# libmir/mir-optim

Measured on AMD Instinct MI355X. Metric: LM iterations/sec, higher is better.
Workload: dtype f64

## Files before the change

include/mir_optim_amd.h:

```cpp
#ifndef MIR_OPTIM_AMD_H
#define MIR_OPTIM_AMD_H

#include <stddef.h>
#include <stdint.h>

#ifdef __cplusplus
extern "C" {
#endif


typedef enum mir_least_squares_status {
    mir_ls_maxIterations = -1,
    mir_ls_furtherImprovement = 0,
    mir_ls_xConverged = 1,
    mir_ls_gConverged = 2,
    mir_ls_fConverged = 3,
    mir_ls_badBounds = -32,
    mir_ls_badGuess = -31,
    mir_ls_badMinStepQuality = -30,
    mir_ls_badGoodStepQuality = -29,
    mir_ls_badStepQuality = -28,
    mir_ls_badLambdaParams = -27,
    mir_ls_numericError = -26
} mir_least_squares_status;

typedef enum mir_box_qp_status {
    mir_box_qp_solved = 0,
    mir_box_qp_numericError = 1,
    mir_box_qp_maxIterations = 2
} mir_box_qp_status;

typedef struct mir_box_qp_settings_d { double relTolerance, absTolerance; uint32_t maxIterations; } mir_box_qp_settings_d;
typedef struct mir_box_qp_settings_s { float relTolerance, absTolerance; uint32_t maxIterations; } mir_box_qp_settings_s;

typedef struct mir_least_squares_settings_d {
    uint32_t maxIterations;
    uint32_t maxAge;
    double jacobianEpsilon;
    double absTolerance;
    double relTolerance;
    double gradTolerance;
    double maxGoodResidual;
    double maxStep;
    double maxLambda;
    double minLambda;
    double minStepQuality;
    double goodStepQuality;
    double lambdaIncrease;
    double lambdaDecrease;
    mir_box_qp_settings_d qpSettings;
} mir_least_squares_settings_d;

typedef struct mir_least_squares_settings_s {
    uint32_t maxIterations, maxAge;
    float jacobianEpsilon, absTolerance, relTolerance, gradTolerance, maxGoodResidual, maxStep,
          maxLambda, minLambda, minStepQuality, goodStepQuality, lambdaIncrease, lambdaDecrease;
    mir_box_qp_settings_s qpSettings;
} mir_least_squares_settings_s;

typedef struct mir_least_squares_result_d {
    int32_t status;
    uint32_t iterations, fCalls, gCalls;
    double residual;
    double lambda;
} mir_least_squares_result_d;
typedef struct mir_least_squares_result_s {
    int32_t status;
    uint32_t iterations, fCalls, gCalls;
    float residual, lambda;
} mir_least_squares_result_s;

typedef struct mir_slice_d { size_t length; double* ptr; } mir_slice_d;
typedef struct mir_slice_s { size_t length; float* ptr; } mir_slice_s;
typedef struct mir_slice_i { size_t length; int32_t* ptr; } mir_slice_i;

typedef void (*mir_least_squares_function_d)(void* context, size_t m, size_t n, const double* x, double* y);
typedef void (*mir_least_squares_jacobian_d)(void* context, size_t m, size_t n, const double* x, double* J);
typedef void (*mir_least_squares_function_s)(void* context, size_t m, size_t n, const float* x, float* y);
typedef void (*mir_least_squares_jacobian_s)(void* context, size_t m, size_t n, const float* x, float* J);

typedef struct mir_least_squares_task { void* context; void* function; } mir_least_squares_task;
typedef void (*mir_least_squares_task_function)(mir_least_squares_task task, uint32_t totalThreads,
                                                uint32_t threadId, uint32_t i);
typedef void (*mir_least_squares_thread_manager)(void* context, uint32_t count,
                                                 mir_least_squares_task taskContext,
                                                 mir_least_squares_task_function task);

size_t mir_least_squares_work_length(size_t m, size_t n);
size_t mir_least_squares_iwork_length(size_t m, size_t n);
size_t mir_box_qp_work_length(size_t n);
size_t mir_box_qp_iwork_length(size_t n);
size_t mir_box_qp_iwork_length_ilp64(size_t n);
size_t mir_least_squares_iwork_length_ilp64(size_t m, size_t n);
const char* mir_least_squares_status_string(mir_least_squares_status st);
void mir_least_squares_init_d(mir_least_squares_settings_d* settings);
void mir_least_squares_init_s(mir_least_squares_settings_s* settings);
void mir_least_squares_reset_d(mir_least_squares_settings_d* settings);
void mir_least_squares_reset_s(mir_least_squares_settings_s* settings);

mir_least_squares_result_d mir_optimize_least_squares_d(
    const mir_least_squares_settings_d* settings, size_t m, size_t n,
    double* x, const double* l, const double* u,
    mir_slice_d work, mir_slice_i iwork,
    void* fContext, mir_least_squares_function_d f,
    void* gContext, mir_least_squares_jacobian_d g,
    void* tmContext, mir_least_squares_thread_manager tm);

mir_least_squares_result_s mir_optimize_least_squares_s(
    const mir_least_squares_settings_s* settings, size_t m, size_t n,
    float* x, const float* l, const float* u,
    mir_slice_s work, mir_slice_i iwork,
    void* fContext, mir_least_squares_function_s f,
    void* gContext, mir_least_squares_jacobian_s g,
    void* tmContext, mir_least_squares_thread_manager tm);


typedef struct mir_lsq_comm mir_lsq_comm;
typedef struct mir_lsq_workspace mir_lsq_workspace;

typedef void (*mir_lsq_batched_function_d)(void* context, size_t m, size_t n, size_t p, const double* X, double* Y);
typedef void (*mir_lsq_batched_function_s)(void* context, size_t m, size_t n, size_t p, const float* X, float* Y);
enum {
    MIR_LSQ_DEVICE_CALLBACKS = 1u,
    MIR_LSQ_TIME_KERNELS = 2u
};

enum {
    MIR_LSQ_VARIANT_BROYDEN_REWRITE = 1u << 0,
    MIR_LSQ_VARIANT_FD_SEPARATE_FILL = 1u << 1,
    MIR_LSQ_VARIANT_NO_SPECULATION = 1u << 4,
    MIR_LSQ_VARIANT_NO_NULL_SKIP = 1u << 5,
    MIR_LSQ_VARIANT_SOLVE_BOUNDED = 1u << 6,
    MIR_LSQ_VARIANT_SOLVE_GENERIC = 1u << 10,
    MIR_LSQ_VARIANT_SOLVE_ONE_WORKGROUP = 1u << 11,
    MIR_LSQ_VARIANT_FD_HOST_COLUMNS = 1u << 13,
    MIR_LSQ_VARIANT_NO_PIPELINE = 1u << 22,
    MIR_LSQ_VARIANT_DEBUG_HELPERS_ABSENT = 1u << 12,
    MIR_LSQ_VARIANT_DEBUG_SOLVE = 1u << 7,
    MIR_LSQ_VARIANT_HOST_PROFILE = 1u << 8,
    MIR_LSQ_VARIANT_LR_CAP_SHIFT = 16
};

typedef struct mir_lsq_stats {
    uint64_t passes, accepted, rejected, step_guard_rejects;
    uint64_t jacobian_full, jacobian_broyden;
    uint64_t jtj_launches;
    uint64_t jtj_broyden_launches;
    double jtj_ms;
    double jtj_broyden_ms;
    double solve_ms;
    uint64_t solve_launches;
    double fd_ms;
    double total_ms;
    uint64_t qp_active_set_passes;
    uint64_t broyden_lr_columns;
    double jtj_fd_ms;
    uint64_t jtj_fd_launches;
    uint64_t elided_evaluations;
    uint64_t allreduce_calls[3];
    uint64_t allreduce_elems[3];
    uint64_t broyden_flushes;
    uint64_t jtj_resyncs;
    double fd_callback_ms;
    uint64_t fd_callback_calls, fd_callback_points;
    double trial_callback_ms;
    uint64_t trial_callback_calls, trial_callback_points;
    uint64_t library_launches;
    uint64_t round_launches[3];
    uint64_t rounds[3];
    double fd_host_wall_ms, fd_host_f_ms;
    uint64_t fd_host_columns;
    double host_f_ms;
    uint64_t host_f_calls;
    uint64_t fused_rounds;
    uint64_t fused_passes;
    uint64_t coop_timeouts;
} mir_lsq_stats;

typedef struct mir_lsq_trace_record {
    int32_t event;
    uint32_t iterations;
    double lambda, residual, trial_residual, dx_dot;
} mir_lsq_trace_record;
typedef struct mir_lsq_trace {
    mir_lsq_trace_record* records;
    uint64_t capacity;
    uint64_t count;
} mir_lsq_trace;

typedef struct mir_lsq_gpu_options {
    uint32_t struct_size;
    uint32_t flags;
    void* stream;
    mir_lsq_comm* comm;
    mir_lsq_workspace* workspace;
    void* fbContext;
    void* fb;
    uint32_t fd_batch;
    uint32_t variant;
    mir_lsq_stats* stats;
    mir_lsq_trace* trace;
    void* fbRowMajor;
    void* fbRowMajorDiff;
    uint32_t stats_size;
    uint32_t reserved0;
} mir_lsq_gpu_options;

mir_least_squares_result_d mir_optimize_least_squares_gpu_d(
    const mir_least_squares_settings_d* settings, size_t m, size_t n,
    double* x, const double* l, const double* u, const mir_lsq_gpu_options* options,
    void* fContext, mir_least_squares_function_d f,
    void* gContext, mir_least_squares_jacobian_d g,
    void* tmContext, mir_least_squares_thread_manager tm);
mir_least_squares_result_s mir_optimize_least_squares_gpu_s(
    const mir_least_squares_settings_s* settings, size_t m, size_t n,
    float* x, const float* l, const float* u, const mir_lsq_gpu_options* options,
    void* fContext, mir_least_squares_function_s f,
    void* gContext, mir_least_squares_jacobian_s g,
    void* tmContext, mir_least_squares_thread_manager tm);

int mir_solve_box_qp_gpu_d(const mir_box_qp_settings_d* settings, size_t n, const double* P,
                           const double* q, const double* l, const double* u, double* x,
                           int unconstrainedSolution, int* iterations);
int mir_solve_box_qp_gpu_s(const mir_box_qp_settings_s* settings, size_t n, const float* P,
                           const float* q, const float* l, const float* u, float* x,
                           int unconstrainedSolution, int* iterations);

#define MIR_LSQ_BOX_QP_UNCONSTRAINED_SOLUTION 1u
int mir_lsq_batched_box_qp_s(const mir_box_qp_settings_s* settings, size_t count, size_t n, const float* P, const float* q,
                             const float* l, const float* u, size_t bound_stride, float* x, int* status, int* iterations,
                             unsigned flags, void* stream);
int mir_lsq_batched_box_qp_d(const mir_box_qp_settings_d* settings, size_t count, size_t n, const double* P, const double* q,
                             const double* l, const double* u, size_t bound_stride, double* x, int* status, int* iterations,
                             unsigned flags, void* stream);

int mir_lsq_batched_box_qp16_s(const mir_box_qp_settings_s* settings, size_t count, size_t n, const float* P, const float* q,
                               const float* l, const float* u, size_t bound_stride, float* x, int* status, int* iterations,
                               unsigned flags, void* stream);
int mir_lsq_batched_box_qp16_d(const mir_box_qp_settings_d* settings, size_t count, size_t n, const double* P, const double* q,
                               const double* l, const double* u, size_t bound_stride, double* x, int* status, int* iterations,
                               unsigned flags, void* stream);

enum { MIR_LSQ_MODEL_EXP_DECAY = 0, MIR_LSQ_MODEL_EXP3_AFFINE = 1,
       MIR_LSQ_MODEL_EXP_DECAY_PAD8 = 2 };
enum { MIR_LSQ_BATCHED_ANALYTIC_JACOBIAN = 2 };
enum { MIR_LSQ_BATCHED_NO_LADDER = 1 };
enum { MIR_LSQ_BATCHED_DEVICE_BOUNDS = 4 };
typedef struct mir_lsq_batched_options {
    uint32_t struct_size;
    uint32_t variant;
    void* stream;
    float* basis;
    size_t basis_bytes;
    uint64_t* timing;
} mir_lsq_batched_options;

int mir_optimize_least_squares_batched_s(const mir_least_squares_settings_s* settings, size_t count, size_t m, int model,
                                         float* x, const float* lower, const float* upper,
                                         const float* t, size_t t_stride, const float* data,
                                         mir_least_squares_result_s* results, const mir_lsq_batched_options* options);

enum { MIR_LSQ_BATCHED_NEEDS_GENERAL = -100 };
int mir_lsq_batched_kernel_s(const mir_least_squares_settings_s* settings, size_t count, size_t m, int model,
                             float* x, const float* lower, const float* upper,
                             const float* t, size_t t_stride, const float* data,
                             mir_least_squares_result_s* results, const mir_lsq_batched_options* options);

int mir_optimize_least_squares_batched_d(const mir_least_squares_settings_d* settings, size_t count, size_t m, int model,
                                         double* x, const double* lower, const double* upper,
                                         const double* t, size_t t_stride, const double* data,
                                         mir_least_squares_result_d* results, const mir_lsq_batched_options* options);
int mir_lsq_batched_kernel_d(const mir_least_squares_settings_d* settings, size_t count, size_t m, int model,
                             double* x, const double* lower, const double* upper,
                             const double* t, size_t t_stride, const double* data,
                             mir_least_squares_result_d* results, const mir_lsq_batched_options* options);

enum { MIR_LSQ_BATCHED_ABSOLUTE_SIGMA = 1u };
typedef struct mir_lsq_batched_extras {
    uint32_t struct_size;
    uint32_t flags;
    const void* weights;
    size_t weight_stride;
    void* covariance;
} mir_lsq_batched_extras;
int mir_optimize_least_squares_batched_ex_s(const mir_least_squares_settings_s* settings, size_t count, size_t m, int model,
                                            float* x, const float* lower, const float* upper,
                                            const float* t, size_t t_stride, const float* data,
                                            mir_least_squares_result_s* results, const mir_lsq_batched_options* options,
                                            const mir_lsq_batched_extras* extras);
int mir_optimize_least_squares_batched_ex_d(const mir_least_squares_settings_d* settings, size_t count, size_t m, int model,
                                            double* x, const double* lower, const double* upper,
                                            const double* t, size_t t_stride, const double* data,
                                            mir_least_squares_result_d* results, const mir_lsq_batched_options* options,
                                            const mir_lsq_batched_extras* extras);
int mir_lsq_batched_kernel_ex_s(const mir_least_squares_settings_s* settings, size_t count, size_t m, int model,
                                float* x, const float* lower, const float* upper,
                                const float* t, size_t t_stride, const float* data,
                                mir_least_squares_result_s* results, const mir_lsq_batched_options* options,
                                const mir_lsq_batched_extras* extras);
int mir_lsq_batched_kernel_ex_d(const mir_least_squares_settings_d* settings, size_t count, size_t m, int model,
                                double* x, const double* lower, const double* upper,
                                const double* t, size_t t_stride, const double* data,
                                mir_least_squares_result_d* results, const mir_lsq_batched_options* options,
                                const mir_lsq_batched_extras* extras);
int mir_lsq_batched_covariance_s(const mir_least_squares_settings_s* settings, size_t count, size_t m, int model,
                                 const float* x, const float* lower, const float* upper,
                                 const float* t, size_t t_stride, const float* data,
                                 const mir_least_squares_result_s* results, const mir_lsq_batched_options* options,
                                 const mir_lsq_batched_extras* extras);
int mir_lsq_batched_covariance_d(const mir_least_squares_settings_d* settings, size_t count, size_t m, int model,
                                 const double* x, const double* lower, const double* upper,
                                 const double* t, size_t t_stride, const double* data,
                                 const mir_least_squares_result_d* results, const mir_lsq_batched_options* options,
                                 const mir_lsq_batched_extras* extras);

enum { MIR_LSQ_MODEL16_EXP_HARM16 = 16, MIR_LSQ_MODEL16_GAUSS3_AFFINE = 17 };
int mir_optimize_least_squares_batched16_d(const mir_least_squares_settings_d* settings, size_t count, size_t m, int model,
                                           double* x, const double* lower, const double* upper,
                                           const double* t, size_t t_stride, const double* data,
                                           mir_least_squares_result_d* results, const mir_lsq_batched_options* options,
                                           const mir_lsq_batched_extras* extras);
int mir_lsq_batched16_kernel_d(const mir_least_squares_settings_d* settings, size_t count, size_t m, int model,
                               double* x, const double* lower, const double* upper,
                               const double* t, size_t t_stride, const double* data,
                               mir_least_squares_result_d* results, const mir_lsq_batched_options* options,
                               const mir_lsq_batched_extras* extras);
int mir_optimize_least_squares_batched16_ex_d(const mir_least_squares_settings_d* settings, size_t count, size_t m, int model,
                                              double* x, const double* lower, const double* upper,
                                              const double* t, size_t t_stride, const double* data,
                                              mir_least_squares_result_d* results, const mir_lsq_batched_options* options,
                                              const mir_lsq_batched_extras* extras);
int mir_lsq_batched16_kernel_ex_d(const mir_least_squares_settings_d* settings, size_t count, size_t m, int model,
                                  double* x, const double* lower, const double* upper,
                                  const double* t, size_t t_stride, const double* data,
                                  mir_least_squares_result_d* results, const mir_lsq_batched_options* options,
                                  const mir_lsq_batched_extras* extras);
int mir_lsq_batched16_covariance_d(const mir_least_squares_settings_d* settings, size_t count, size_t m, int model,
                                   const double* x, const double* lower, const double* upper,
                                   const double* t, size_t t_stride, const double* data,
                                   const mir_least_squares_result_d* results, const mir_lsq_batched_options* options,
                                   const mir_lsq_batched_extras* extras);
int mir_lsq_batched16_jtj_d(size_t count, size_t m, size_t n, const double* J, const double* y, double* JJ, double* Jy, void* stream);

enum { MIR_LSQ_RESIDENT_NO_NULL_SKIP = 1u,
       MIR_LSQ_RESIDENT_UNBOUNDED = 2u,
       MIR_LSQ_RESIDENT_NO_LOOKAHEAD = 4u,
       MIR_LSQ_RESIDENT_DEBUG_DROP_WORKGROUP = 16u,
       MIR_LSQ_RESIDENT_ANALYTIC_JACOBIAN = 32u,
       MIR_LSQ_RESIDENT_NO_STAMPS = 8u           };
typedef struct mir_lsq_resident_stats {
    uint64_t rounds, passes, accepted, rejected, step_guard_rejects, jacobian_full, jacobian_broyden, qp_active_set_passes,
        elided_evaluations;
    uint64_t t_total, t_stage, t_worker, t_group, t_total_wait, t_solver, t_solve_body, t_cmd_wait;
    uint64_t t_w_eval, t_w_fd, t_w_prod;
    uint64_t t_w_mma;
    uint64_t lookahead_rejections;
    uint64_t t_look;
    uint64_t t_unpack, t_publish;
    uint32_t abort_code, grid, rows, groups;
} mir_lsq_resident_stats;
typedef struct mir_lsq_resident_options {
    uint32_t struct_size;
    uint32_t variant;
    void* stream;
    void* workspace;
    size_t workspace_bytes;
    mir_lsq_trace_record* trace_records;
    uint32_t trace_capacity;
    uint32_t max_workgroups;
    uint32_t* trace_count;
    mir_lsq_resident_stats* stats;
} mir_lsq_resident_options;

int mir_lsq_batched_posvx_s(size_t count, size_t n, const float* P, const float* rhs, float* x, int* info, void* stream);
int mir_lsq_batched_posvx_d(size_t count, size_t n, const double* P, const double* rhs, double* x, int* info, void* stream);
int mir_lsq_batched_posvx16_s(size_t count, size_t n, const float* P, const float* rhs, float* x, int* info, void* stream);
int mir_lsq_batched_posvx16_d(size_t count, size_t n, const double* P, const double* rhs, double* x, int* info, void* stream);

int mir_lsq_jtj_d(size_t m, size_t n, double* J, const double* y, const double* y_old, const double* dx,
                  int broyden, double* JJ, double* Jy, void* stream, float* kernel_ms);
int mir_lsq_jtj_s(size_t m, size_t n, float* J, const float* y, const float* y_old, const float* dx,
                  int broyden, float* JJ, float* Jy, void* stream, float* kernel_ms);
int mir_lsq_fd_jtj_d(size_t m, size_t n, const double* Yrm, const double* twh, const double* y, double* J,
                     double* JJ, double* Jy, void* stream, float* kernel_ms);
int mir_lsq_fd_diff_jtj_d(size_t m, size_t n, const double* Drm, const double* twh, const double* y, double* J,
                          double* JJ, double* Jy, void* stream, float* kernel_ms);
int mir_lsq_jtj_plan(size_t elem_size, size_t m, size_t n, int num_cu, int op, int aligned16, size_t out[10]);

enum { MIR_LSQ_COVARIANCE_ABSOLUTE_SIGMA = 1u };
int mir_lsq_covariance_gpu_d(const mir_least_squares_settings_d* settings, size_t m, size_t n,
    const double* x, const double* l, const double* u, const mir_lsq_gpu_options* options,
    void* fContext, mir_least_squares_function_d f, void* gContext, mir_least_squares_jacobian_d g,
    void* tmContext, mir_least_squares_thread_manager tm,
    uint32_t flags, double* cov, double* residual_out, int* info);
int mir_lsq_covariance_gpu_s(const mir_least_squares_settings_s* settings, size_t m, size_t n,
    const float* x, const float* l, const float* u, const mir_lsq_gpu_options* options,
    void* fContext, mir_least_squares_function_s f, void* gContext, mir_least_squares_jacobian_s g,
    void* tmContext, mir_least_squares_thread_manager tm,
    uint32_t flags, float* cov, float* residual_out, int* info);
int mir_lsq_spd_inverse_d(size_t n, const double* P, const unsigned char* fixed, double* X, int* info, void* stream);
int mir_lsq_spd_inverse_s(size_t n, const float*  P, const unsigned char* fixed, float*  X, int* info, void* stream);
size_t mir_lsq_spd_inverse_work_bytes(size_t n, size_t elem_size);
int mir_lsq_spd_inverse_work_d(size_t n, const double* P, const unsigned char* fixed, double* X, int* info, void* work,
                               size_t work_bytes, void* stream);
int mir_lsq_spd_inverse_work_s(size_t n, const float* P, const unsigned char* fixed, float* X, int* info, void* work,
                               size_t work_bytes, void* stream);

mir_lsq_workspace* mir_lsq_workspace_create(size_t m, size_t n, size_t elem_size);
void mir_lsq_workspace_destroy(mir_lsq_workspace* ws);

int mir_lsq_rccl_unique_id(void* out_128_bytes);
mir_lsq_comm* mir_lsq_comm_create_rccl(int nranks, int rank, const void* unique_id_128_bytes);
typedef void (*mir_lsq_allreduce_fn)(void* ctx, double* device_buf, size_t count, void* stream);
mir_lsq_comm* mir_lsq_comm_create_callback(int nranks, int rank, mir_lsq_allreduce_fn fn, void* ctx);
int mir_lsq_comm_create_local_group(int nranks, mir_lsq_comm** out_comms);
void mir_lsq_comm_destroy(mir_lsq_comm* comm);
int mir_lsq_comm_record(mir_lsq_comm* comm, double* host_buf, size_t capacity);
size_t mir_lsq_comm_recorded(const mir_lsq_comm* comm);
mir_lsq_comm* mir_lsq_comm_create_replay(int nranks, int rank, const double* totals_host, size_t len, mir_lsq_comm* inner);
int mir_lsq_comm_replay_rewind(mir_lsq_comm* comm);
int mir_lsq_comm_replay_set_delay(mir_lsq_comm* comm, unsigned microseconds);
int mir_lsq_comm_ranks(const mir_lsq_comm* comm);
int mir_lsq_comm_describe(const mir_lsq_comm* comm, char* buf, size_t len);
int mir_lsq_comm_allreduce_d(mir_lsq_comm* comm, double* buf, size_t count, void* stream);
int mir_lsq_comm_allreduce_s(mir_lsq_comm* comm, float* buf, size_t count, void* stream);

int mir_lsq_device_count(void);
void* mir_lsq_device_malloc(size_t bytes);
void mir_lsq_device_free(void* p);
int mir_lsq_memcpy_h2d(void* dst_device, const void* src_host, size_t bytes, void* stream);
int mir_lsq_memcpy_d2h(void* dst_host, const void* src_device, size_t bytes, void* stream);
int mir_lsq_memcpy_d2d(void* dst_device, const void* src_device, size_t bytes, void* stream);

int mir_lsq_selftest_reductions(int rounds, int mismatches[4]);
void* mir_lsq_stream_create(void);
void mir_lsq_stream_destroy(void* stream);
int mir_lsq_stream_synchronize(void* stream);
const char* mir_lsq_version(void);

enum { MIR_FIT_SPLINE_OK = 0, MIR_FIT_SPLINE_TOO_FEW_POINTS = 1, MIR_FIT_SPLINE_BAD_ARGUMENT = 2 };

int mir_fit_spline_d(const mir_least_squares_settings_d* settings, size_t npoints, const double* points, size_t nx,
                     const double* x, const double* l, const double* u, double lambda, double (*dist)(double, double),
                     double* splineY, double* splineD, mir_least_squares_result_d* result);
int mir_fit_spline_s(const mir_least_squares_settings_s* settings, size_t npoints, const float* points, size_t nx,
                     const float* x, const float* l, const float* u, float lambda, float (*dist)(float, float),
                     float* splineY, float* splineD, mir_least_squares_result_s* result);
void mir_fit_spline_residuals_d(size_t npoints, const double* points, size_t nx, const double* x, double lambda,
                                const double* splineY, size_t m, double* y);
void mir_spline_c2_derivatives_d(size_t n, const double* x, const double* y, double* d);
void mir_spline_c2_derivatives_s(size_t n, const float* x, const float* y, float* d);
void mir_spline_eval_d(size_t n, const double* x, const double* y, const double* d, double t, double* out3);
void mir_spline_eval_s(size_t n, const float* x, const float* y, const float* d, float t, float* out3);

#ifdef __cplusplus
}
#endif
#endif
```

mir_optim_amd/api.py:

```python
import ctypes as C
import enum
import os

import numpy as np

from . import build as _build

__all__ = [
    "LeastSquaresStatus", "BoxQPStatus", "LeastSquaresSettings", "LeastSquaresResult", "BoxQPSettings",
    "LeastSquaresException", "optimize", "optimizeLeastSquares", "solveBoxQP", "leastSquaresStatusString",
    "mir_least_squares_work_length", "mir_least_squares_iwork_length", "mir_box_qp_work_length",
    "mir_box_qp_iwork_length", "GpuOptions", "Stats", "lib", "workloads_lib", "device_count",
    "DeviceBuffer", "Stream", "jtj", "fd_jtj", "DEVICE_CALLBACKS", "TIME_KERNELS", "optimizeLeastSquaresBatched", "batchedPosvx", "BATCHED_NO_LADDER", "BATCHED_DEVICE_BOUNDS",
    "solveBoxQPBatched", "BOX_QP_UNCONSTRAINED_SOLUTION",
    "MODEL_EXP_DECAY", "MODEL_EXP3_AFFINE", "MODEL_EXP_DECAY_PAD8", "MODEL16_EXP_HARM16", "MODEL16_GAUSS3_AFFINE", "batched16JtJ", "optimizeLeastSquaresBatched16", "ResultS", "Trace", "TraceRecord", "Spline", "FitSplineResult", "fitSpline",
    "fit_spline_residuals", "variant_lr_cap",
    "VARIANT_BROYDEN_REWRITE", "VARIANT_FD_SEPARATE_FILL", "VARIANT_NO_SPECULATION", "VARIANT_NO_NULL_SKIP",
    "VARIANT_SOLVE_BOUNDED", "VARIANT_DEBUG_SOLVE", "VARIANT_HOST_PROFILE", "VARIANT_SOLVE_GENERIC", "VARIANT_SOLVE_ONE_WORKGROUP", "VARIANT_DEBUG_HELPERS_ABSENT", "VARIANT_FD_HOST_COLUMNS",
    "VARIANT_NO_PIPELINE", "BatchedOptions", "BatchedExtras", "BATCHED_ABSOLUTE_SIGMA",
    "covariance", "spdInverse", "COVARIANCE_ABSOLUTE_SIGMA",
]

MODEL_EXP_DECAY = 0
MODEL_EXP3_AFFINE = 1
MODEL_EXP_DECAY_PAD8 = 2
MODEL16_EXP_HARM16 = 16
MODEL16_GAUSS3_AFFINE = 17
_MODELS16 = (MODEL16_EXP_HARM16, MODEL16_GAUSS3_AFFINE)

DEVICE_CALLBACKS = 1
TIME_KERNELS = 2

VARIANT_BROYDEN_REWRITE = 1 << 0
VARIANT_FD_SEPARATE_FILL = 1 << 1
VARIANT_NO_SPECULATION = 1 << 4
VARIANT_NO_NULL_SKIP = 1 << 5
VARIANT_SOLVE_BOUNDED = 1 << 6
VARIANT_DEBUG_SOLVE = 1 << 7
VARIANT_HOST_PROFILE = 1 << 8
VARIANT_SOLVE_GENERIC = 1 << 10
VARIANT_SOLVE_ONE_WORKGROUP = 1 << 11
VARIANT_DEBUG_HELPERS_ABSENT = 1 << 12
VARIANT_FD_HOST_COLUMNS = 1 << 13
VARIANT_NO_PIPELINE = 1 << 22


def variant_lr_cap(k):
    return (int(k) & 31) << 16


class LeastSquaresStatus(enum.IntEnum):
    maxIterations = -1
    furtherImprovement = 0
    xConverged = 1
    gConverged = 2
    fConverged = 3
    badBounds = -32
    badGuess = -31
    badMinStepQuality = -30
    badGoodStepQuality = -29
    badStepQuality = -28
    badLambdaParams = -27
    numericError = -26


class BoxQPStatus(enum.IntEnum):
    solved = 0
    numericError = 1
    maxIterations = 2


class LeastSquaresException(Exception):

    def __init__(self, status, result=None):
        self.status = LeastSquaresStatus(status)
        self.result = result
        super().__init__("mir-optim Least Squares: " + leastSquaresStatusString(status))


class _QPd(C.Structure):
    _fields_ = [("relTolerance", C.c_double), ("absTolerance", C.c_double), ("maxIterations", C.c_uint32)]


class _QPs(C.Structure):
    _fields_ = [("relTolerance", C.c_float), ("absTolerance", C.c_float), ("maxIterations", C.c_uint32)]


_FIELDS = ["jacobianEpsilon", "absTolerance", "relTolerance", "gradTolerance", "maxGoodResidual", "maxStep",
           "maxLambda", "minLambda", "minStepQuality", "goodStepQuality", "lambdaIncrease", "lambdaDecrease"]


class _Sd(C.Structure):
    _fields_ = ([("maxIterations", C.c_uint32), ("maxAge", C.c_uint32)] + [(k, C.c_double) for k in _FIELDS]
                + [("qpSettings", _QPd)])


class _Ss(C.Structure):
    _fields_ = ([("maxIterations", C.c_uint32), ("maxAge", C.c_uint32)] + [(k, C.c_float) for k in _FIELDS]
                + [("qpSettings", _QPs)])


class _Rd(C.Structure):
    _fields_ = [("status", C.c_int32), ("iterations", C.c_uint32), ("fCalls", C.c_uint32), ("gCalls", C.c_uint32),
                ("residual", C.c_double), ("lambda_", C.c_double)]


class _Rs(C.Structure):
    _fields_ = [("status", C.c_int32), ("iterations", C.c_uint32), ("fCalls", C.c_uint32), ("gCalls", C.c_uint32),
                ("residual", C.c_float), ("lambda_", C.c_float)]


ResultS = _Rs


class _SliceD(C.Structure):
    _fields_ = [("length", C.c_size_t), ("ptr", C.c_void_p)]


class _Task(C.Structure):
    _fields_ = [("context", C.c_void_p), ("function", C.c_void_p)]


class Stats(C.Structure):
    _fields_ = [("passes", C.c_uint64), ("accepted", C.c_uint64), ("rejected", C.c_uint64),
                ("step_guard_rejects", C.c_uint64), ("jacobian_full", C.c_uint64), ("jacobian_broyden", C.c_uint64),
                ("jtj_launches", C.c_uint64), ("jtj_broyden_launches", C.c_uint64), ("jtj_ms", C.c_double),
                ("jtj_broyden_ms", C.c_double), ("solve_ms", C.c_double), ("solve_launches", C.c_uint64),
                ("fd_ms", C.c_double), ("total_ms", C.c_double), ("qp_active_set_passes", C.c_uint64),
                ("broyden_lr_columns", C.c_uint64),
                ("jtj_fd_ms", C.c_double), ("jtj_fd_launches", C.c_uint64),
                ("elided_evaluations", C.c_uint64),
                ("allreduce_calls", C.c_uint64 * 3), ("allreduce_elems", C.c_uint64 * 3),
                ("broyden_flushes", C.c_uint64), ("jtj_resyncs", C.c_uint64),
                ("fd_callback_ms", C.c_double), ("fd_callback_calls", C.c_uint64), ("fd_callback_points", C.c_uint64),
                ("trial_callback_ms", C.c_double), ("trial_callback_calls", C.c_uint64),
                ("trial_callback_points", C.c_uint64),
                ("library_launches", C.c_uint64), ("round_launches", C.c_uint64 * 3), ("rounds", C.c_uint64 * 3),
                ("fd_host_wall_ms", C.c_double), ("fd_host_f_ms", C.c_double), ("fd_host_columns", C.c_uint64),
                ("host_f_ms", C.c_double), ("host_f_calls", C.c_uint64),
                ("fused_rounds", C.c_uint64), ("fused_passes", C.c_uint64), ("coop_timeouts", C.c_uint64)]

    def as_dict(self):
        return {k: (list(getattr(self, k)) if isinstance(getattr(self, k), C.Array) else getattr(self, k)) for k, _ in self._fields_}


class TraceRecord(C.Structure):
    _fields_ = [("event", C.c_int32), ("iterations", C.c_uint32), ("lambda_", C.c_double), ("residual", C.c_double),
                ("trial_residual", C.c_double), ("dx_dot", C.c_double)]


class _TraceHeader(C.Structure):
    _fields_ = [("records", C.POINTER(TraceRecord)), ("capacity", C.c_uint64), ("count", C.c_uint64)]


class Trace:

    EVENTS = {0: "jacobian_full", 1: "jacobian_broyden", 2: "rejected", 3: "accepted", 4: "step_guard"}

    def __init__(self, capacity=4096):
        self._buf = (TraceRecord * capacity)()
        self.header = _TraceHeader(C.cast(self._buf, C.POINTER(TraceRecord)), capacity, 0)

    @property
    def count(self):
        return int(self.header.count)

    def records(self):
        k = min(self.count, int(self.header.capacity))
        return [(r.event, r.iterations, r.lambda_, r.residual, r.trial_residual, r.dx_dot) for r in self._buf[:k]]


class GpuOptions(C.Structure):
    _fields_ = [("struct_size", C.c_uint32), ("flags", C.c_uint32), ("stream", C.c_void_p), ("comm", C.c_void_p),
                ("workspace", C.c_void_p), ("fbContext", C.c_void_p), ("fb", C.c_void_p), ("fd_batch", C.c_uint32),
                ("variant", C.c_uint32), ("stats", C.POINTER(Stats)), ("trace", C.POINTER(_TraceHeader)),
                ("fbRowMajor", C.c_void_p), ("fbRowMajorDiff", C.c_void_p), ("stats_size", C.c_uint32),
                ("reserved0", C.c_uint32)]

    def __init__(self, **kw):
        super().__init__(**kw)
        self.struct_size = C.sizeof(GpuOptions)
        self.stats_size = C.sizeof(Stats)


class BatchedOptions(C.Structure):
    _fields_ = [("struct_size", C.c_uint32), ("variant", C.c_uint32), ("stream", C.c_void_p), ("basis", C.c_void_p),
                ("basis_bytes", C.c_size_t), ("timing", C.c_void_p)]

    def __init__(self, **kw):
        super().__init__(**kw)
        self.struct_size = C.sizeof(BatchedOptions)


class BatchedExtras(C.Structure):
    _fields_ = [("struct_size", C.c_uint32), ("flags", C.c_uint32), ("weights", C.c_void_p), ("weight_stride", C.c_size_t),
                ("covariance", C.c_void_p)]

    def __init__(self, **kw):
        super().__init__(**kw)
        self.struct_size = C.sizeof(BatchedExtras)


TASK_FN = C.CFUNCTYPE(None, _Task, C.c_uint32, C.c_uint32, C.c_uint32)
TM_FN = C.CFUNCTYPE(None, C.c_void_p, C.c_uint32, _Task, TASK_FN)
ALLREDUCE_FN = C.CFUNCTYPE(None, C.c_void_p, C.c_void_p, C.c_size_t, C.c_void_p)


def _ftype(dtype):
    ct = C.c_double if dtype == np.float64 else C.c_float
    return C.CFUNCTYPE(None, C.c_void_p, C.c_size_t, C.c_size_t, C.POINTER(ct), C.POINTER(ct))


_lib = None
_wl = None


def _load(path):
    if not os.path.exists(path):
        raise ImportError(f"{path} is missing: build it with `python -m mir_optim_amd.build` "
                          "(hipcc --offload-arch=gfx950). mir_optim_amd has no CPU fallback.")
    return C.CDLL(path, mode=C.RTLD_GLOBAL)


def lib():
    global _lib
    if _lib is None:
        L = _load(_build.SOLVER_LIB)
        sz = C.c_size_t
        for name in ("mir_least_squares_work_length", "mir_least_squares_iwork_length"):
            getattr(L, name).restype = sz
            getattr(L, name).argtypes = [sz, sz]
        for name in ("mir_box_qp_work_length", "mir_box_qp_iwork_length"):
            getattr(L, name).restype = sz
            getattr(L, name).argtypes = [sz]
        L.mir_box_qp_iwork_length_ilp64.restype = sz
        L.mir_box_qp_iwork_length_ilp64.argtypes = [sz]
        L.mir_least_squares_iwork_length_ilp64.restype = sz
        L.mir_least_squares_iwork_length_ilp64.argtypes = [sz, sz]
        L.mir_least_squares_status_string.restype = C.c_char_p
        L.mir_least_squares_status_string.argtypes = [C.c_int]
        for suf, S, R in (("d", _Sd, _Rd), ("s", _Ss, _Rs)):
            getattr(L, "mir_least_squares_init_" + suf).argtypes = [C.POINTER(S)]
            getattr(L, "mir_least_squares_reset_" + suf).argtypes = [C.POINTER(S)]
            fn = getattr(L, "mir_optimize_least_squares_" + suf)
            fn.restype = R
            fn.argtypes = [C.POINTER(S), sz, sz, C.c_void_p, C.c_void_p, C.c_void_p, _SliceD, _SliceD,
                           C.c_void_p, C.c_void_p, C.c_void_p, C.c_void_p, C.c_void_p, C.c_void_p]
            fn = getattr(L, "mir_optimize_least_squares_gpu_" + suf)
            fn.restype = R
            fn.argtypes = [C.POINTER(S), sz, sz, C.c_void_p, C.c_void_p, C.c_void_p, C.POINTER(GpuOptions),
                           C.c_void_p, C.c_void_p, C.c_void_p, C.c_void_p, C.c_void_p, C.c_void_p]
            fn = getattr(L, "mir_solve_box_qp_gpu_" + suf)
            fn.restype = C.c_int
            fn.argtypes = [C.c_void_p, sz, C.c_void_p, C.c_void_p, C.c_void_p, C.c_void_p, C.c_void_p, C.c_int,
                           C.POINTER(C.c_int)]
            fn = getattr(L, "mir_lsq_jtj_" + suf)
            fn.restype = C.c_int
            fn.argtypes = [sz, sz, C.c_void_p, C.c_void_p, C.c_void_p, C.c_void_p, C.c_int, C.c_void_p, C.c_void_p,
                           C.c_void_p, C.POINTER(C.c_float)]
            fn = getattr(L, "mir_lsq_covariance_gpu_" + suf)
            fn.restype = C.c_int
            fn.argtypes = [C.POINTER(S), sz, sz, C.c_void_p, C.c_void_p, C.c_void_p, C.POINTER(GpuOptions),
                           C.c_void_p, C.c_void_p, C.c_void_p, C.c_void_p, C.c_void_p, C.c_void_p,
                           C.c_uint32, C.c_void_p, C.c_void_p, C.POINTER(C.c_int)]
            fn = getattr(L, "mir_lsq_spd_inverse_" + suf)
            fn.restype = C.c_int
            fn.argtypes = [sz, C.c_void_p, C.c_void_p, C.c_void_p, C.c_void_p, C.c_void_p]
            fn = getattr(L, "mir_lsq_spd_inverse_work_" + suf)
            fn.restype = C.c_int
            fn.argtypes = [sz, C.c_void_p, C.c_void_p, C.c_void_p, C.c_void_p, C.c_void_p, sz, C.c_void_p]
        L.mir_lsq_spd_inverse_work_bytes.restype = sz
        L.mir_lsq_spd_inverse_work_bytes.argtypes = [sz, sz]
        L.mir_lsq_comm_create_local_group.restype = C.c_int
        L.mir_lsq_comm_create_local_group.argtypes = [C.c_int, C.POINTER(C.c_void_p)]
        L.mir_lsq_fd_diff_jtj_d.restype = C.c_int
        L.mir_lsq_fd_diff_jtj_d.argtypes = [sz, sz, C.c_void_p, C.c_void_p, C.c_void_p, C.c_void_p, C.c_void_p, C.c_void_p,
                                            C.c_void_p, C.POINTER(C.c_float)]
        L.mir_lsq_fd_jtj_d.restype = C.c_int
        L.mir_lsq_fd_jtj_d.argtypes = [sz, sz, C.c_void_p, C.c_void_p, C.c_void_p, C.c_void_p, C.c_void_p, C.c_void_p,
                                       C.c_void_p, C.c_void_p]
        L.mir_optimize_least_squares_batched_s.restype = C.c_int
        L.mir_optimize_least_squares_batched_s.argtypes = [C.POINTER(_Ss), sz, sz, C.c_int, C.c_void_p, C.c_void_p, C.c_void_p,
                                                           C.c_void_p, sz, C.c_void_p, C.c_void_p, C.POINTER(BatchedOptions)]
        L.mir_lsq_batched_kernel_s.restype = C.c_int
        L.mir_lsq_batched_kernel_s.argtypes = [C.POINTER(_Ss), sz, sz, C.c_int, C.c_void_p, C.c_void_p, C.c_void_p,
                                               C.c_void_p, sz, C.c_void_p, C.c_void_p, C.POINTER(BatchedOptions)]
        L.mir_lsq_jtj_plan.restype = C.c_int
        L.mir_lsq_jtj_plan.argtypes = [sz, sz, sz, C.c_int, C.c_int, C.c_int, C.POINTER(sz * 10)]
        L.mir_lsq_selftest_reductions.restype = C.c_int
        L.mir_lsq_selftest_reductions.argtypes = [C.c_int, C.POINTER(C.c_int * 4)]
        L.mir_lsq_batched_posvx_s.restype = C.c_int
        L.mir_lsq_batched_posvx_s.argtypes = [sz, sz, C.c_void_p, C.c_void_p, C.c_void_p, C.c_void_p, C.c_void_p]
        L.mir_optimize_least_squares_batched_d.restype = C.c_int
        L.mir_optimize_least_squares_batched_d.argtypes = [C.POINTER(_Sd), sz, sz, C.c_int, C.c_void_p, C.c_void_p, C.c_void_p,
                                                           C.c_void_p, sz, C.c_void_p, C.c_void_p, C.POINTER(BatchedOptions)]
        L.mir_lsq_batched_kernel_d.restype = C.c_int
        L.mir_lsq_batched_kernel_d.argtypes = [C.POINTER(_Sd), sz, sz, C.c_int, C.c_void_p, C.c_void_p, C.c_void_p,
                                               C.c_void_p, sz, C.c_void_p, C.c_void_p, C.POINTER(BatchedOptions)]
        L.mir_lsq_batched_posvx_d.restype = C.c_int
        L.mir_lsq_batched_posvx_d.argtypes = [sz, sz, C.c_void_p, C.c_void_p, C.c_void_p, C.c_void_p, C.c_void_p]
        for suf, S in (("s", _Ss), ("d", _Sd)):
            for name in ("mir_optimize_least_squares_batched_ex_", "mir_lsq_batched_kernel_ex_", "mir_lsq_batched_covariance_"):
                fn = getattr(L, name + suf)
                fn.restype = C.c_int
                fn.argtypes = [C.POINTER(S), sz, sz, C.c_int, C.c_void_p, C.c_void_p, C.c_void_p, C.c_void_p, sz, C.c_void_p,
                               C.c_void_p, C.POINTER(BatchedOptions), C.POINTER(BatchedExtras)]
        for name in ("mir_optimize_least_squares_batched16_d", "mir_lsq_batched16_kernel_d", "mir_optimize_least_squares_batched16_ex_d",
                     "mir_lsq_batched16_kernel_ex_d", "mir_lsq_batched16_covariance_d"):
            fn = getattr(L, name)
            fn.restype = C.c_int
            fn.argtypes = [C.POINTER(_Sd), sz, sz, C.c_int, C.c_void_p, C.c_void_p, C.c_void_p, C.c_void_p, sz, C.c_void_p,
                           C.c_void_p, C.POINTER(BatchedOptions), C.POINTER(BatchedExtras)]
        L.mir_lsq_batched16_jtj_d.restype = C.c_int
        L.mir_lsq_batched16_jtj_d.argtypes = [sz, sz, sz, C.c_void_p, C.c_void_p, C.c_void_p, C.c_void_p, C.c_void_p]
        for name in ("box_qp_s", "box_qp_d", "box_qp16_s", "box_qp16_d"):
            fn = getattr(L, "mir_lsq_batched_" + name)
            fn.restype = C.c_int
            fn.argtypes = [C.c_void_p, sz, sz, C.c_void_p, C.c_void_p, C.c_void_p, C.c_void_p, sz, C.c_void_p, C.c_void_p,
                           C.c_void_p, C.c_uint, C.c_void_p]
        for suf in ("s", "d"):
            fn = getattr(L, "mir_lsq_batched_posvx16_" + suf)
            fn.restype = C.c_int
            fn.argtypes = [sz, sz, C.c_void_p, C.c_void_p, C.c_void_p, C.c_void_p, C.c_void_p]
        L.mir_lsq_comm_describe.restype = C.c_int
        L.mir_lsq_comm_describe.argtypes = [C.c_void_p, C.c_char_p, C.c_size_t]
        L.mir_lsq_workspace_create.restype = C.c_void_p
        L.mir_lsq_workspace_create.argtypes = [sz, sz, sz]
        L.mir_lsq_workspace_destroy.argtypes = [C.c_void_p]
        L.mir_lsq_rccl_unique_id.restype = C.c_int
        L.mir_lsq_rccl_unique_id.argtypes = [C.c_void_p]
        L.mir_lsq_comm_create_rccl.restype = C.c_void_p
        L.mir_lsq_comm_create_rccl.argtypes = [C.c_int, C.c_int, C.c_void_p]
        L.mir_lsq_comm_create_callback.restype = C.c_void_p
        L.mir_lsq_comm_create_callback.argtypes = [C.c_int, C.c_int, ALLREDUCE_FN, C.c_void_p]
        L.mir_lsq_comm_destroy.argtypes = [C.c_void_p]
        L.mir_lsq_comm_record.restype = C.c_int
        L.mir_lsq_comm_record.argtypes = [C.c_void_p, C.c_void_p, sz]
        L.mir_lsq_comm_recorded.restype = sz
        L.mir_lsq_comm_recorded.argtypes = [C.c_void_p]
        L.mir_lsq_comm_create_replay.restype = C.c_void_p
        L.mir_lsq_comm_create_replay.argtypes = [C.c_int, C.c_int, C.c_void_p, sz, C.c_void_p]
        L.mir_lsq_comm_replay_rewind.restype = C.c_int
        L.mir_lsq_comm_replay_rewind.argtypes = [C.c_void_p]
        L.mir_lsq_comm_replay_set_delay.restype = C.c_int
        L.mir_lsq_comm_replay_set_delay.argtypes = [C.c_void_p, C.c_uint]
        L.mir_lsq_comm_ranks.restype = C.c_int
        L.mir_lsq_comm_ranks.argtypes = [C.c_void_p]
        for name in ("mir_lsq_comm_allreduce_d", "mir_lsq_comm_allreduce_s"):
            getattr(L, name).restype = C.c_int
            getattr(L, name).argtypes = [C.c_void_p, C.c_void_p, sz, C.c_void_p]
        L.mir_lsq_device_count.restype = C.c_int
        L.mir_lsq_device_malloc.restype = C.c_void_p
        L.mir_lsq_device_malloc.argtypes = [sz]
        L.mir_lsq_device_free.argtypes = [C.c_void_p]
        for name in ("mir_lsq_memcpy_h2d", "mir_lsq_memcpy_d2h", "mir_lsq_memcpy_d2d"):
            getattr(L, name).restype = C.c_int
            getattr(L, name).argtypes = [C.c_void_p, C.c_void_p, sz, C.c_void_p]
        L.mir_lsq_stream_create.restype = C.c_void_p
        L.mir_lsq_stream_destroy.argtypes = [C.c_void_p]
        L.mir_lsq_stream_synchronize.restype = C.c_int
        L.mir_lsq_stream_synchronize.argtypes = [C.c_void_p]
        L.mir_lsq_version.restype = C.c_char_p
        for suf, S, R, ct in (("d", _Sd, _Rd, C.c_double), ("s", _Ss, _Rs, C.c_float)):
            fn = getattr(L, "mir_fit_spline_" + suf)
            fn.restype = C.c_int
            fn.argtypes = [C.POINTER(S), sz, C.c_void_p, sz, C.c_void_p, C.c_void_p, C.c_void_p, ct, C.c_void_p,
                           C.c_void_p, C.c_void_p, C.POINTER(R)]
            getattr(L, "mir_spline_c2_derivatives_" + suf).argtypes = [sz, C.c_void_p, C.c_void_p, C.c_void_p]
            getattr(L, "mir_spline_eval_" + suf).argtypes = [sz, C.c_void_p, C.c_void_p, C.c_void_p, ct, C.c_void_p]
        L.mir_fit_spline_residuals_d.argtypes = [sz, C.c_void_p, sz, C.c_void_p, C.c_double, C.c_void_p, sz, C.c_void_p]
        _lib = L
    return _lib


def workloads_lib():
    global _wl
    if _wl is None:
        W = _load(_build.WORKLOADS_LIB)
        W.wl_uniform.argtypes = [C.c_uint64, C.c_uint64, C.c_size_t, C.c_void_p]
        W.wl_tanh_linear_generate.argtypes = [C.c_size_t, C.c_size_t, C.c_size_t, C.c_double, C.c_void_p, C.c_void_p,
                                              C.c_void_p, C.c_void_p]
        _wl = W
    return _wl


def device_count():
    return lib().mir_lsq_device_count()


def leastSquaresStatusString(st):
    return lib().mir_least_squares_status_string(int(st)).decode()


def mir_least_squares_work_length(m, n):
    return lib().mir_least_squares_work_length(m, n)


def mir_least_squares_iwork_length(m, n):
    return lib().mir_least_squares_iwork_length(m, n)


def mir_box_qp_work_length(n):
    return lib().mir_box_qp_work_length(n)


def mir_box_qp_iwork_length(n):
    return lib().mir_box_qp_iwork_length(n)


def LeastSquaresSettings(dtype=np.float64):
    s = _Sd() if dtype == np.float64 else _Ss()
    (lib().mir_least_squares_init_d if dtype == np.float64 else lib().mir_least_squares_init_s)(C.byref(s))
    return s


def BoxQPSettings(dtype=np.float64):
    return LeastSquaresSettings(dtype).qpSettings


class LeastSquaresResult:

    def __init__(self, raw):
        self.status = LeastSquaresStatus(raw.status)
        self.iterations = raw.iterations
        self.fCalls = raw.fCalls
        self.gCalls = raw.gCalls
        self.residual = raw.residual
        self.lambda_ = raw.lambda_

    def __repr__(self):
        return (f"LeastSquaresResult(status={self.status.name}, iterations={self.iterations}, fCalls={self.fCalls}, "
                f"gCalls={self.gCalls}, residual={self.residual!r}, lambda={self.lambda_!r})")


class Stream:
    def __init__(self):
        self.handle = lib().mir_lsq_stream_create()
        if not self.handle:
            raise RuntimeError("hipStreamCreate failed (no GPU?)")

    def synchronize(self):
        if lib().mir_lsq_stream_synchronize(self.handle) != 0:
            raise RuntimeError("stream synchronize failed")

    def close(self):
        if self.handle:
            lib().mir_lsq_stream_destroy(self.handle)
            self.handle = None

    def __del__(self):
        try:
            self.close()
        except Exception:
            pass


class DeviceBuffer:

    def __init__(self, array=None, nbytes=None, dtype=None, shape=None):
        if array is not None:
            array = np.ascontiguousarray(array)
            nbytes, dtype, shape = array.nbytes, array.dtype, array.shape
        self.nbytes, self.dtype, self.shape = int(nbytes), np.dtype(dtype), tuple(shape)
        self.ptr = lib().mir_lsq_device_malloc(max(self.nbytes, 8))
        if not self.ptr:
            raise MemoryError(f"hipMalloc({self.nbytes}) failed (no GPU?)")
        if array is not None:
            self.upload(array)

    def upload(self, array):
        array = np.ascontiguousarray(array, dtype=self.dtype)
        assert array.nbytes == self.nbytes
        if lib().mir_lsq_memcpy_h2d(self.ptr, array.ctypes.data, self.nbytes, None) != 0:
            raise RuntimeError("H2D copy failed")

    def upload_at(self, byte_offset, array):
        array = np.ascontiguousarray(array, dtype=self.dtype)
        assert 0 <= byte_offset and byte_offset + array.nbytes <= self.nbytes
        if lib().mir_lsq_memcpy_h2d(self.ptr + byte_offset, array.ctypes.data, array.nbytes, None) != 0:
            raise RuntimeError("H2D copy failed")

    def download(self):
        out = np.empty(self.shape, dtype=self.dtype)
        if lib().mir_lsq_memcpy_d2h(out.ctypes.data, self.ptr, self.nbytes, None) != 0:
            raise RuntimeError("D2H copy failed")
        return out

    def free(self):
        if self.ptr:
            lib().mir_lsq_device_free(self.ptr)
            self.ptr = None

    def __del__(self):
        try:
            self.free()
        except Exception:
            pass


def _as_fnptr(cb, ftype, wrap, keep):
    if cb is None:
        return C.c_void_p(None)
    if callable(cb):
        c = ftype(wrap(cb))
        keep.append(c)
        return C.cast(c, C.c_void_p)
    return C.c_void_p(int(cb))


def _wrap_callbacks(f, g, tm, dtype):
    ft = _ftype(dtype)
    keep = []
    errors = []

    def wrap_f(fn):
        def cb(_ctx, m_, n_, xp, yp):
            yv = np.ctypeslib.as_array(yp, shape=(m_,))
            try:
                xv = np.ctypeslib.as_array(xp, shape=(n_,))
                yv[:] = 0
                fn(xv, yv)
            except BaseException as e:
                errors.append(e)
                yv[:] = np.nan
        return cb

    def wrap_g(fn):
        def cb(_ctx, m_, n_, xp, Jp):
            Jv = np.ctypeslib.as_array(Jp, shape=(m_ * n_,)).reshape(m_, n_)
            try:
                xv = np.ctypeslib.as_array(xp, shape=(n_,))
                Jv[:] = 0
                fn(xv, Jv)
            except BaseException as e:
                errors.append(e)
                Jv[:] = np.nan
        return cb

    fptr = _as_fnptr(f, ft, wrap_f, keep)
    gptr = _as_fnptr(g, ft, wrap_g, keep)
    tmptr = C.c_void_p(None)
    if tm is not None:
        def tm_cb(_ctx, count, task, taskfn):
            try:
                tm(count, lambda total, tid, i: taskfn(task, total, tid, i))
            except BaseException as e:
                errors.append(e)
        tmc = TM_FN(tm_cb)
        keep.append(tmc)
        tmptr = C.cast(tmc, C.c_void_p)
    return fptr, gptr, tmptr, keep, errors


def optimizeLeastSquares(f, m, x, l=None, u=None, g=None, tm=None, settings=None, dtype=np.float64,
                         fContext=None, gContext=None, options=None, gpu_entry=None):
    L = lib()
    dbl = dtype == np.float64
    x = np.ascontiguousarray(x, dtype=dtype)
    n = x.size
    lo = np.full(n, -np.inf, dtype=dtype) if l is None else np.ascontiguousarray(l, dtype=dtype)
    up = np.full(n, np.inf, dtype=dtype) if u is None else np.ascontiguousarray(u, dtype=dtype)
    if settings is None:
        settings = LeastSquaresSettings(dtype)
    fptr, gptr, tmptr, keep, errors = _wrap_callbacks(f, g, tm, dtype)
    use_gpu_entry = gpu_entry if gpu_entry is not None else (options is not None)
    suf = "d" if dbl else "s"
    if use_gpu_entry:
        fn = getattr(L, "mir_optimize_least_squares_gpu_" + suf)
        raw = fn(C.byref(settings), m, n, x.ctypes.data, lo.ctypes.data, up.ctypes.data,
                 C.byref(options) if options is not None else None, fContext, fptr, gContext, gptr, None, tmptr)
    else:
        wl = L.mir_least_squares_work_length(m, n)
        iwl = L.mir_least_squares_iwork_length(m, n)
        iwork = np.zeros(iwl + 4, dtype=np.int32)
        work_slice = _SliceD(wl, None)
        iwork_slice = _SliceD(iwl, iwork.ctypes.data)
        fn = getattr(L, "mir_optimize_least_squares_" + suf)
        raw = fn(C.byref(settings), m, n, x.ctypes.data, lo.ctypes.data, up.ctypes.data, work_slice, iwork_slice,
                 fContext, fptr, gContext, gptr, None, tmptr)
    del keep
    if errors:
        raise errors[0]
    return LeastSquaresResult(raw), x


def optimize(f, m, x, l=None, u=None, g=None, tm=None, settings=None, dtype=np.float64, taskPool=None, **kw):
    if taskPool is not None and tm is None:
        import threading
        workers = max(1, getattr(taskPool, "_max_workers", 1))
        ids = {}
        lock = threading.Lock()

        def tm(count, task):
            def run(i):
                with lock:
                    tid = ids.setdefault(threading.get_ident(), len(ids))
                task(workers, tid % workers, i)
            list(taskPool.map(run, range(count)))
    res, xo = optimizeLeastSquares(f, m, x, l, u, g, tm, settings, dtype, **kw)
    if res.status < 0:
        raise LeastSquaresException(res.status, res)
    return res, xo


def _batched_suffix(dtype):
    if np.dtype(dtype) == np.float32:
        return "s"
    if np.dtype(dtype) == np.float64:
        return "d"
    raise ValueError(f"the batched entries exist in float32 and float64, not {np.dtype(dtype)}")


def optimizeLeastSquaresBatched(model, x, t, data, l=None, u=None, settings=None, variant=0, dtype=np.float32, weights=None,
                                covariance=False, absolute_sigma=False):
    if int(model) in _MODELS16:
        return _optimize_batched16(model, x, t, data, l, u, settings, variant, dtype, weights, covariance, absolute_sigma)
    suf = _batched_suffix(dtype)
    dtype = np.float32 if suf == "s" else np.float64
    L = lib()
    x = np.array(x, dtype=dtype, order="C")
    count, n = x.shape
    data = np.ascontiguousarray(data, dtype=dtype)
    m = data.shape[1]
    t = np.ascontiguousarray(t, dtype=dtype)
    t_stride = 0 if t.ndim == 1 else m
    lo = np.full(n, -np.inf, dtype=dtype) if l is None else np.ascontiguousarray(l, dtype=dtype)
    up = np.full(n, np.inf, dtype=dtype) if u is None else np.ascontiguousarray(u, dtype=dtype)
    if settings is None:
        settings = LeastSquaresSettings(dtype)
    raw = ((_Rs if suf == "s" else _Rd) * count)()
    if weights is None and not covariance and not absolute_sigma:
        fn = getattr(L, "mir_optimize_least_squares_batched_" + suf)
        rc = fn(C.byref(settings), count, m, int(model), x.ctypes.data, lo.ctypes.data, up.ctypes.data, t.ctypes.data, t_stride,
                data.ctypes.data, raw, C.byref(BatchedOptions(variant=variant)))
        if rc != 0:
            raise RuntimeError(f"mir_optimize_least_squares_batched_{suf} failed: {rc}")
        return [LeastSquaresResult(r) for r in raw], x
    ex = BatchedExtras(flags=BATCHED_ABSOLUTE_SIGMA if absolute_sigma else 0)
    if weights is not None:
        weights = np.ascontiguousarray(weights, dtype=dtype)
        if weights.shape not in ((m,), (count, m)):
            raise ValueError(f"weights: {m} values or {count} x {m}, not {weights.shape}")
        ex.weights = weights.ctypes.data
        ex.weight_stride = 0 if weights.ndim == 1 else m
    cov = np.empty((count, n, n), dtype=dtype) if covariance else None
    if covariance:
        ex.covariance = cov.ctypes.data
    fn = getattr(L, "mir_optimize_least_squares_batched_ex_" + suf)
    rc = fn(C.byref(settings), count, m, int(model), x.ctypes.data, lo.ctypes.data, up.ctypes.data, t.ctypes.data, t_stride,
            data.ctypes.data, raw, C.byref(BatchedOptions(variant=variant)), C.byref(ex))
    if rc != 0:
        raise RuntimeError(f"mir_optimize_least_squares_batched_ex_{suf} failed: {rc}")
    res = [LeastSquaresResult(r) for r in raw]
    return (res, x, cov) if covariance else (res, x)


def _optimize_batched16(model, x, t, data, l, u, settings, variant, dtype, weights, covariance, absolute_sigma):
    if np.dtype(dtype) != np.float64:
        raise ValueError(f"the MODEL16_* models are fitted in float64 only, not {np.dtype(dtype)}: pass dtype=np.float64")
    if weights is not None or covariance or absolute_sigma:
        raise ValueError("the MODEL16_* models take neither weights nor covariance here: call optimizeLeastSquaresBatched16")
    L = lib()
    x = np.array(x, dtype=np.float64, order="C")
    count, n = x.shape
    data = np.ascontiguousarray(data, dtype=np.float64)
    m = data.shape[1]
    t = np.ascontiguousarray(t, dtype=np.float64)
    t_stride = 0 if t.ndim == 1 else m
    lo = np.full(n, -np.inf) if l is None else np.ascontiguousarray(l, dtype=np.float64)
    up = np.full(n, np.inf) if u is None else np.ascontiguousarray(u, dtype=np.float64)
    if settings is None:
        settings = LeastSquaresSettings(np.float64)
    raw = (_Rd * count)()
    rc = L.mir_optimize_least_squares_batched16_d(C.byref(settings), count, m, int(model), x.ctypes.data, lo.ctypes.data,
                                                  up.ctypes.data, t.ctypes.data, t_stride, data.ctypes.data, raw,
                                                  C.byref(BatchedOptions(variant=variant)), None)
    if rc != 0:
        raise RuntimeError(f"mir_optimize_least_squares_batched16_d failed: {rc}")
    return [LeastSquaresResult(r) for r in raw], x


def optimizeLeastSquaresBatched16(model, x, t, data, l=None, u=None, settings=None, variant=0, weights=None, covariance=False,
                                  absolute_sigma=False):
    if int(model) not in _MODELS16:
        raise ValueError(f"optimizeLeastSquaresBatched16 takes a MODEL16_* id, not {model}")
    for name, a in (("x", x), ("t", t), ("data", data), ("weights", weights)):
        dt = getattr(a, "dtype", None)
        if dt is not None and np.issubdtype(dt, np.floating) and dt != np.float64:
            raise ValueError(f"the MODEL16_* models are fitted in float64 only: {name} is {dt}")
    if weights is None and not covariance and not absolute_sigma:
        return _optimize_batched16(model, x, t, data, l, u, settings, variant, np.float64, None, False, False)
    L = lib()
    x = np.array(x, dtype=np.float64, order="C")
    data = np.ascontiguousarray(data, dtype=np.float64)
    t = np.ascontiguousarray(t, dtype=np.float64)
    if x.ndim != 2 or data.ndim != 2 or data.shape[0] != x.shape[0]:
        raise ValueError(f"x: count x n and data: count x m, not {x.shape} and {data.shape}")
    count, n = x.shape
    m = data.shape[1]
    if t.shape not in ((m,), (count, m)):
        raise ValueError(f"t: {m} values or {count} x {m}, not {t.shape}")
    t_stride = 0 if t.ndim == 1 else m
    lo = np.full(n, -np.inf) if l is None else np.ascontiguousarray(l, dtype=np.float64)
    up = np.full(n, np.inf) if u is None else np.ascontiguousarray(u, dtype=np.float64)
    if lo.shape != (n,) or up.shape != (n,):
        raise ValueError(f"l and u: {n} values each, not {lo.shape} and {up.shape}")
    if settings is None:
        settings = LeastSquaresSettings(np.float64)
    ex = BatchedExtras(flags=BATCHED_ABSOLUTE_SIGMA if absolute_sigma else 0)
    if weights is not None:
        weights = np.ascontiguousarray(weights, dtype=np.float64)
        if weights.shape not in ((m,), (count, m)):
            raise ValueError(f"weights: {m} values or {count} x {m}, not {weights.shape}")
        ex.weights = weights.ctypes.data
        ex.weight_stride = 0 if weights.ndim == 1 else m
    cov = np.empty((count, n, n), dtype=np.float64) if covariance else None
    if covariance:
        ex.covariance = cov.ctypes.data
    raw = (_Rd * count)()
    rc = L.mir_optimize_least_squares_batched16_ex_d(C.byref(settings), count, m, int(model), x.ctypes.data, lo.ctypes.data,
                                                     up.ctypes.data, t.ctypes.data, t_stride, data.ctypes.data, raw,
                                                     C.byref(BatchedOptions(variant=variant)), C.byref(ex))
    if rc != 0:
        raise RuntimeError(f"mir_optimize_least_squares_batched16_ex_d failed: {rc}")
    res = [LeastSquaresResult(r) for r in raw]
    return (res, x, cov) if covariance else (res, x)


def batched16JtJ(J, y):
    L = lib()
    J = np.ascontiguousarray(J, dtype=np.float64)
    y = np.ascontiguousarray(y, dtype=np.float64)
    count, m, n = J.shape
    dJ, dy = DeviceBuffer(J), DeviceBuffer(y)
    dJJ = DeviceBuffer(nbytes=count * 256 * 8, dtype=np.float64, shape=(count, 16, 16))
    dJy = DeviceBuffer(nbytes=count * 16 * 8, dtype=np.float64, shape=(count, 16))
    st = Stream()
    rc = L.mir_lsq_batched16_jtj_d(count, m, n, dJ.ptr, dy.ptr, dJJ.ptr, dJy.ptr, st.handle)
    if rc != 0:
        raise RuntimeError(f"mir_lsq_batched16_jtj_d failed: {rc}")
    st.synchronize()
    JJ, Jy = dJJ.download().copy(), dJy.download().copy()
    for b in (dJ, dy, dJJ, dJy):
        b.free()
    return JJ, Jy


BATCHED_NO_LADDER = 1
BATCHED_DEVICE_BOUNDS = 4
BATCHED_ABSOLUTE_SIGMA = 1


def batchedPosvx(P, rhs, dtype=np.float32):
    suf = _batched_suffix(dtype)
    dtype = np.float32 if suf == "s" else np.float64
    L = lib()
    P = np.asarray(P, dtype=dtype)
    count, n = P.shape[0], P.shape[1]
    w, name = (8, "mir_lsq_batched_posvx_" + suf) if n <= 8 else (16, "mir_lsq_batched_posvx16_" + suf)
    Pp = np.zeros((count, w, w), dtype=dtype); Pp[:, :n, :n] = P
    bp = np.zeros((count, w), dtype=dtype); bp[:, :n] = rhs
    dP, db = DeviceBuffer(Pp), DeviceBuffer(bp)
    dx = DeviceBuffer(nbytes=count * w * np.dtype(dtype).itemsize, dtype=dtype, shape=(count, w))
    di = DeviceBuffer(nbytes=count * 4, dtype=np.int32, shape=(count,))
    st = Stream()
    rc = getattr(L, name)(count, n, dP.ptr, db.ptr, dx.ptr, di.ptr, st.handle)
    if rc != 0:
        raise RuntimeError(f"{name} failed: {rc}")
    st.synchronize()
    x, info = dx.download()[:, :n].copy(), di.download().copy()
    for b in (dP, db, dx, di):
        b.free()
    return x, info


COVARIANCE_ABSOLUTE_SIGMA = 1


def covariance(f, m, x, l=None, u=None, g=None, tm=None, settings=None, dtype=np.float64, absolute_sigma=False,
               fContext=None, gContext=None, options=None):
    L = lib()
    x = np.array(x, dtype=dtype, order="C")
    n = x.size
    lo = np.full(n, -np.inf, dtype=dtype) if l is None else np.ascontiguousarray(l, dtype=dtype)
    up = np.full(n, np.inf, dtype=dtype) if u is None else np.ascontiguousarray(u, dtype=dtype)
    if settings is None:
        settings = LeastSquaresSettings(dtype)
    fptr, gptr, tmptr, keep, errors = _wrap_callbacks(f, g, tm, dtype)
    cov = np.empty((n, n), dtype=dtype)
    res = np.zeros(1, dtype=dtype)
    info = C.c_int(0)
    fn = getattr(L, "mir_lsq_covariance_gpu_" + ("d" if dtype == np.float64 else "s"))
    rc = fn(C.byref(settings), m, n, x.ctypes.data, lo.ctypes.data, up.ctypes.data,
            C.byref(options) if options is not None else None, fContext, fptr, gContext, gptr, None, tmptr,
            COVARIANCE_ABSOLUTE_SIGMA if absolute_sigma else 0, cov.ctypes.data, res.ctypes.data, C.byref(info))
    del keep
    if errors:
        raise errors[0]
    if rc == -1:
        raise ValueError("mir_lsq_covariance_gpu: NULL argument")
    if rc != 0:
        raise LeastSquaresException(rc)
    with np.errstate(invalid="ignore"):
        stderr = np.sqrt(np.diag(cov))
    return cov, stderr, res[0], info.value


def spdInverse(P, fixed=None, dtype=np.float64):
    suf = _batched_suffix(dtype)
    dtype = np.float32 if suf == "s" else np.float64
    L = lib()
    P = np.ascontiguousarray(P, dtype=dtype)
    n = P.shape[0]
    dP = DeviceBuffer(P)
    dX = DeviceBuffer(nbytes=n * n * P.itemsize, dtype=dtype, shape=(n, n))
    di = DeviceBuffer(nbytes=4, dtype=np.int32, shape=(1,))
    df = None
    if fixed is not None:
        fx = np.ascontiguousarray(np.asarray(fixed) != 0, dtype=np.uint8)
        if fx.shape != (n,):
            raise ValueError(f"fixed: {n} flags, not {fx.shape}")
        df = DeviceBuffer(fx)
    rc = getattr(L, "mir_lsq_spd_inverse_" + suf)(n, dP.ptr, df.ptr if df is not None else None, dX.ptr, di.ptr, None)
    if rc != 0:
        raise RuntimeError(f"mir_lsq_spd_inverse_{suf} failed: {rc}")
    X, info = dX.download(), int(di.download()[0])
    for b in (dP, dX, di, df):
        if b is not None:
            b.free()
    return X, info


def solveBoxQP(P, q, l, u, x=None, settings=None, dtype=np.float64, unconstrainedSolution=False):
    L = lib()
    P = np.ascontiguousarray(P, dtype=dtype)
    n = P.shape[0]
    q = np.ascontiguousarray(q, dtype=dtype)
    l = np.ascontiguousarray(l, dtype=dtype)
    u = np.ascontiguousarray(u, dtype=dtype)
    xo = np.zeros(n, dtype=dtype) if x is None else np.ascontiguousarray(x, dtype=dtype).copy()
    if settings is None:
        settings = BoxQPSettings(dtype)
    it = C.c_int(0)
    fn = L.mir_solve_box_qp_gpu_d if dtype == np.float64 else L.mir_solve_box_qp_gpu_s
    st = fn(C.byref(settings), n, P.ctypes.data, q.ctypes.data, l.ctypes.data, u.ctypes.data, xo.ctypes.data,
            1 if unconstrainedSolution else 0, C.byref(it))
    return BoxQPStatus(st), xo, it.value


BOX_QP_UNCONSTRAINED_SOLUTION = 1


def _box_qp_batched_pack(P, q, l, u, x, dtype, unconstrainedSolution):
    return _box_qp_batched_pack_w(P, q, l, u, x, dtype, unconstrainedSolution, 8, 1)


def _box_qp_batched_pack16(P, q, l, u, x, dtype, unconstrainedSolution):
    return _box_qp_batched_pack_w(P, q, l, u, x, dtype, unconstrainedSolution, 16, 9)


def _box_qp_batched_pack_w(P, q, l, u, x, dtype, unconstrainedSolution, W, nmin):
    suf = _batched_suffix(dtype)
    dtype = np.float32 if suf == "s" else np.float64
    P = np.asarray(P, dtype=dtype)
    if P.ndim != 3 or P.shape[1] != P.shape[2]:
        raise ValueError(f"P: count x n x n, not {P.shape}")
    count, n = P.shape[0], P.shape[1]
    if not nmin <= n <= W:
        raise ValueError(f"solveBoxQPBatched: n = {n} is outside {nmin} .. {W}")
    q = np.asarray(q, dtype=dtype)
    if q.shape != (count, n):
        raise ValueError(f"q: {count} x {n}, not {q.shape}")
    l, u = np.asarray(l, dtype=dtype), np.asarray(u, dtype=dtype)
    if l.shape != u.shape or l.shape not in ((n,), (count, n)):
        raise ValueError(f"l, u: both {n} values or both {count} x {n}, not {l.shape} and {u.shape}")
    shared = l.ndim == 1
    Pp = np.zeros((count, W, W), dtype=dtype); Pp[:, :n, :n] = P
    qp = np.zeros((count, W), dtype=dtype); qp[:, :n] = q
    lp = np.zeros((W,) if shared else (count, W), dtype=dtype); lp[..., :n] = l
    up = np.zeros((W,) if shared else (count, W), dtype=dtype); up[..., :n] = u
    xp = np.zeros((count, W), dtype=dtype)
    if x is not None:
        x = np.asarray(x, dtype=dtype)
        if x.shape != (count, n):
            raise ValueError(f"x: {count} x {n}, not {x.shape}")
        xp[:, :n] = x
    elif unconstrainedSolution:
        raise ValueError("unconstrainedSolution=True needs x, the unconstrained minimisers")
    return count, n, Pp, qp, lp, up, (0 if shared else W), xp


def solveBoxQPBatched(P, q, l, u, x=None, settings=None, dtype=np.float64, unconstrainedSolution=False):
    n_in = np.shape(P)[1] if np.ndim(P) == 3 else 0
    if n_in > 16:
        raise ValueError(f"solveBoxQPBatched: n = {n_in} is above 16, the limit of the batched kernels")
    wide = n_in > 8
    pack = _box_qp_batched_pack16 if wide else _box_qp_batched_pack
    count, n, Pp, qp, lp, up, bound_stride, xp = pack(P, q, l, u, x, dtype, unconstrainedSolution)
    dtype = Pp.dtype.type
    suf = "s" if dtype == np.float32 else "d"
    if settings is None:
        settings = BoxQPSettings(dtype)
    if count == 0:
        return np.zeros(0, dtype=np.int32), np.zeros((0, n), dtype=dtype), np.zeros(0, dtype=np.int32)
    L = lib()
    bufs = [DeviceBuffer(a) for a in (Pp, qp, lp, up, xp)]
    dst = DeviceBuffer(nbytes=count * 4, dtype=np.int32, shape=(count,))
    dit = DeviceBuffer(nbytes=count * 4, dtype=np.int32, shape=(count,))
    st = Stream()
    name = ("mir_lsq_batched_box_qp16_" if wide else "mir_lsq_batched_box_qp_") + suf
    rc = getattr(L, name)(C.addressof(settings), count, n, bufs[0].ptr, bufs[1].ptr, bufs[2].ptr, bufs[3].ptr, bound_stride,
                          bufs[4].ptr, dst.ptr, dit.ptr, BOX_QP_UNCONSTRAINED_SOLUTION if unconstrainedSolution else 0, st.handle)
    if rc != 0:
        raise RuntimeError(f"{name} failed: {rc}")
    st.synchronize()
    out = dst.download().copy(), bufs[4].download()[:, :n].copy(), dit.download().copy()
    for b in bufs + [dst, dit]:
        b.free()
    return out


def jtj(J, y, y_old=None, dx=None, dtype=np.float64):
    L = lib()
    J = np.ascontiguousarray(J, dtype=dtype)
    m, n = J.shape
    dJ = DeviceBuffer(J)
    dy = DeviceBuffer(np.ascontiguousarray(y, dtype=dtype))
    broyden = dx is not None
    dyo = DeviceBuffer(np.ascontiguousarray(y_old if broyden else y, dtype=dtype))
    ddx = DeviceBuffer(np.ascontiguousarray(dx if broyden else np.zeros(n), dtype=dtype))
    dJJ = DeviceBuffer(nbytes=n * n * J.itemsize, dtype=dtype, shape=(n, n))
    dJy = DeviceBuffer(nbytes=n * J.itemsize, dtype=dtype, shape=(n,))
    ms = C.c_float(0)
    fn = L.mir_lsq_jtj_d if dtype == np.float64 else L.mir_lsq_jtj_s
    rc = fn(m, n, dJ.ptr, dy.ptr, dyo.ptr, ddx.ptr, 1 if broyden else 0, dJJ.ptr, dJy.ptr, None, C.byref(ms))
    if rc != 0:
        raise RuntimeError(f"mir_lsq_jtj failed: {rc}")
    out = dJJ.download(), dJy.download(), dJ.download(), ms.value
    for b in (dJ, dy, dyo, ddx, dJJ, dJy):
        b.free()
    return out


JTJ_OPS = ("plain", "rewrite", "fd", "fd_diff")
JTJ_FAMILIES = ("none", "stream", "fdp", "pc32", "ring8", "fdp8", "wide")


def jtj_plan(elem_size, m, n, num_cu, op, aligned=True):
    out = (C.c_size_t * 10)()
    rc = lib().mir_lsq_jtj_plan(elem_size, m, n, num_cu, JTJ_OPS.index(op), int(bool(aligned)), C.byref(out))
    if rc != 0:
        raise ValueError(f"mir_lsq_jtj_plan: {rc}")
    d = dict(zip(("family", "ncb", "flat", "grid", "jobs", "lds", "slabs", "slab_len", "reduce_ncb", "workspace_slab_elems"), map(int, out)))
    d["family"] = JTJ_FAMILIES[d["family"]]
    return d


def fd_jtj(Yrm, twh, y, diff=False):
    L = lib()
    Yrm = np.ascontiguousarray(Yrm, dtype=np.float64)
    m, n2 = Yrm.shape
    n = n2 if diff else n2 // 2
    dY = DeviceBuffer(Yrm)
    dt = DeviceBuffer(np.ascontiguousarray(twh, dtype=np.float64))
    dy = DeviceBuffer(np.ascontiguousarray(y, dtype=np.float64))
    dJ = DeviceBuffer(nbytes=m * n * 8, dtype=np.float64, shape=(m, n))
    dJJ = DeviceBuffer(nbytes=n * n * 8, dtype=np.float64, shape=(n, n))
    dJy = DeviceBuffer(nbytes=n * 8, dtype=np.float64, shape=(n,))
    ms = C.c_float(0)
    rc = (L.mir_lsq_fd_diff_jtj_d if diff else L.mir_lsq_fd_jtj_d)(m, n, dY.ptr, dt.ptr, dy.ptr, dJ.ptr, dJJ.ptr, dJy.ptr, None, C.byref(ms))
    if rc != 0:
        raise RuntimeError(f"mir_lsq_fd_jtj_d failed: {rc}")
    out = dJ.download(), dJJ.download(), dJy.download(), ms.value
    for b in (dY, dt, dy, dJ, dJJ, dJy):
        b.free()
    return out



class Spline:

    def __init__(self, x, values, dtype=np.float64):
        self.dtype = dtype
        self.x = np.ascontiguousarray(x, dtype=dtype)
        self.values = np.ascontiguousarray(values, dtype=dtype)
        self.derivatives = np.zeros_like(self.values)
        suf = "d" if dtype == np.float64 else "s"
        getattr(lib(), "mir_spline_c2_derivatives_" + suf)(self.x.size, self.x.ctypes.data, self.values.ctypes.data,
                                                         self.derivatives.ctypes.data)
        self._eval = getattr(lib(), "mir_spline_eval_" + suf)

    def withTwoDerivatives(self, t):
        out = np.zeros(3, dtype=self.dtype)
        self._eval(self.x.size, self.x.ctypes.data, self.values.ctypes.data, self.derivatives.ctypes.data, t, out.ctypes.data)
        return out

    def __call__(self, t):
        if np.ndim(t) == 0:
            return self.withTwoDerivatives(float(t))[0]
        return np.array([self.withTwoDerivatives(float(v))[0] for v in np.asarray(t).ravel()]).reshape(np.shape(t))


class FitSplineResult:

    def __init__(self, leastSquaresResult, spline):
        self.leastSquaresResult = leastSquaresResult
        self.spline = spline


def fit_spline_residuals(points, x, lambda_, splineY):
    points = np.ascontiguousarray(points, dtype=np.float64)
    x = np.ascontiguousarray(x, dtype=np.float64)
    v = np.ascontiguousarray(splineY, dtype=np.float64)
    m = points.shape[0] + (1 if lambda_ == 0 else 0)
    y = np.zeros(m)
    lib().mir_fit_spline_residuals_d(points.shape[0], points.ctypes.data, x.size, x.ctypes.data, lambda_, v.ctypes.data, m,
                                     y.ctypes.data)
    return y


def fitSpline(settings, points, x, l, u, lambda_=0.0, dtype=np.float64):
    L = lib()
    points = np.ascontiguousarray(points, dtype=dtype)
    x = np.ascontiguousarray(x, dtype=dtype)
    lo = np.ascontiguousarray(l, dtype=dtype)
    up = np.ascontiguousarray(u, dtype=dtype)
    if not lambda_ >= 0:
        raise ValueError("fitSpline: lambda has to be non-negative")
    y = np.zeros(x.size, dtype=dtype)
    d = np.zeros(x.size, dtype=dtype)
    dbl = dtype == np.float64
    raw = (_Rd if dbl else _Rs)()
    fn = L.mir_fit_spline_d if dbl else L.mir_fit_spline_s
    rc = fn(C.byref(settings) if settings is not None else None, points.shape[0], points.ctypes.data, x.size,
            x.ctypes.data, lo.ctypes.data, up.ctypes.data, lambda_, None, y.ctypes.data, d.ctypes.data, C.byref(raw))
    if rc == 1:
        raise Exception("fitSpline: points.length has to be greater or equal x.length when lambda is 0.0")
    if rc != 0:
        raise ValueError("fitSpline: bad argument")
    res = LeastSquaresResult(raw)
    if res.status < 0:
        raise LeastSquaresException(int(res.status), res)
    return FitSplineResult(res, Spline(x, y, dtype))
```

mir_optim_amd/csrc/broyden_launch.h:

```cpp
#pragma once

#include "common.h"
#include "solve_types.h"

namespace mirlsq {

template <typename T>
struct LrArgs {
    const T* J;
    T* U;
    const T* D;
    const T* dx;
    const T* dx_dot;
    const T* y;
    const T* y_old;
    T* partials;
    size_t m;
    int n;
    int k;
    const ChainRec<T>* spec_rec;
    T absTolerance, relTolerance;
};

constexpr int kLrMaxBlocks = 1024;
inline int lr_blocks(size_t m, int num_cu)
{
    const size_t G = (m + 3) / 4;
    size_t want = (G + 4 * 8 - 1) / (4 * 8);
    size_t cap = (size_t)num_cu * 4;
    if (cap > (size_t)kLrMaxBlocks) cap = kLrMaxBlocks;
    if (want > cap) want = cap;
    return (int)(want ? want : 1);
}

template <typename T> hipError_t lr_sweep(const LrArgs<T>& a, int nblk, hipStream_t s);
template <typename T> hipError_t lr_reduce(const T* partials, int nblk, int n, T* out, hipStream_t s);
template <typename T> hipError_t lr_finish(const T* lr, T* D, const T* dx, int k, int n, T* JJ, T* Jy, LmState<T>* st, hipStream_t s);
template <typename T> hipError_t lr_sumsq(const T* v, size_t m, int count, size_t vstride, T* partials, int pstride, int nblk, hipStream_t s);
template <typename T> hipError_t lr_sumsq_final(const T* partials, int pstride, int nblk, int count, T* out, hipStream_t s);
template <typename T> hipError_t lr_flush(T* J, const T* U, const T* D, int k, size_t m, int n, int num_cu, hipStream_t s);

}
```

mir_optim_amd/csrc/broyden_lr.h:

```cpp
#pragma once

#include "broyden_launch.h"
#include "common.h"
#include "solve_types.h"

namespace mirlsq {


template <typename T> struct LrPair;
template <> struct LrPair<double> { using type = double2; };
template <> struct LrPair<float> { using type = float2; };



template <typename T>
__device__ __forceinline__ bool lr_spec_go(const ChainRec<T>& r, T absTolerance, T relTolerance)
{
    const T dxn = dsqrt(r.new_dx_dot);
    return r.qp_status == 0 && !(r.flags & (kFlagDxNaN | kFlagXNaN | kFlagStepTooLong | kFlagNullStep | kFlagGradSmall))
        && (dxn > absTolerance && r.trial_xnorm > dxn * relTolerance);
}

template <typename T>
__device__ __forceinline__ T lr_wave_sumsq(const T* __restrict__ y, size_t m, size_t gb, size_t ge, int q)
{
    T yy = 0;
    for (size_t g0 = gb; g0 < ge; g0 += 8) {
        T v[8];
#pragma unroll
        for (int e = 0; e < 8; ++e) {
            const size_t row = 4 * (g0 + e) + q;
            v[e] = (g0 + e < ge && row < m) ? y[row] : T(0);
        }
#pragma unroll
        for (int e = 0; e < 8; ++e)
            if (g0 + e < ge) yy = dfma(v[e], v[e], yy);
    }
    yy += wave_shfl_xor(yy, 16);
    yy += wave_shfl_xor(yy, 32);
    return yy;
}

template <typename T, int NCP, bool VEC>
__global__ __launch_bounds__(256, (NCP <= 4 ? 4 : 1)) void k_broyden_lr(const LrArgs<T> a)
{
    using P2 = typename LrPair<T>::type;
    __shared__ T red[4][lr_len(kLrMaxN)];
    __shared__ T coef[kLrMax];
    const int lane = threadIdx.x & 63, wave = threadIdx.x >> 6;
    const int q = lane >> 4, p = lane & 15;
    const int n = a.n, k = a.k;
    const size_t m = a.m;
    const size_t G = (m + 3) / 4;
    const size_t nw = (size_t)gridDim.x * 4, wid = (size_t)blockIdx.x * 4 + wave;
    const size_t per = (G + nw - 1) / nw;
    const size_t gb = wid * per;
    const size_t ge = gb + per < G ? gb + per : G;
    if (a.spec_rec && !lr_spec_go(a.spec_rec[0], a.absTolerance, a.relTolerance)) {
        const T yy = lr_wave_sumsq(a.y, m, gb, ge, q);
        if (q == 0 && p == 0) red[wave][0] = yy;
        __syncthreads();
        const int len = lr_len(n);
        T* out = a.partials + (size_t)blockIdx.x * len;
        for (int e = threadIdx.x; e < len; e += blockDim.x) out[e] = e == lr_yy(n) ? (red[0][0] + red[1][0]) + (red[2][0] + red[3][0]) : T(0);
        return;
    }

    for (int l = wave; l < k; l += 4) {
        T s = 0;
        for (int j = lane; j < n; j += kWave) s += a.D[(size_t)l * n + j] * a.dx[j];
        s = wave_sum(s);
        if (lane == 0) coef[l] = s;
    }
    T d0[NCP], d1[NCP];
    int coff[NCP];
    bool ok0[NCP], ok1[NCP];
#pragma unroll
    for (int c = 0; c < NCP; ++c) {
        const int col = 32 * c + 2 * p;
        ok0[c] = col < n;
        ok1[c] = col + 1 < n;
        coff[c] = ok0[c] ? col : 0;
        const T t0 = a.dx[ok0[c] ? col : 0], t1 = a.dx[ok1[c] ? col + 1 : 0];
        d0[c] = ok0[c] ? t0 : T(0);
        d1[c] = ok1[c] ? t1 : T(0);
    }
    __syncthreads();
    const bool own = p < k;
    const T cp = own ? coef[p] : T(0);
    const T* __restrict__ Up = a.U + (size_t)(own ? p : 0) * m;
    T* __restrict__ Uk = a.U + (size_t)k * m;
    const T nd = -(T(1) / *a.dx_dot);

    T va0[NCP], va1[NCP], ga0[NCP], ga1[NCP];
#pragma unroll
    for (int c = 0; c < NCP; ++c) { va0[c] = 0; va1[c] = 0; ga0[c] = 0; ga1[c] = 0; }
    T wl = 0, hl = 0, uu = 0, uy = 0, yy = 0;

    constexpr int UNR = NCP == 1 ? 4 : (NCP == 2 ? 2 : 1);
    for (size_t g0 = gb; g0 < ge; g0 += UNR) {
        T v0[UNR][NCP], v1[UNR][NCP], ynv[UNR], yov[UNR], ulv[UNR];
#pragma unroll
        for (int e = 0; e < UNR; ++e) {
            const size_t g = g0 + e < ge ? g0 + e : ge - 1;
            const size_t row = 4 * g + q;
            const size_t rr = row < m ? row : m - 1;
            const T* __restrict__ rp = a.J + rr * (size_t)n;
#pragma unroll
            for (int c = 0; c < NCP; ++c) {
                if constexpr (VEC) {
                    typedef T lr_v2 __attribute__((ext_vector_type(2)));
                    const lr_v2 t = __builtin_nontemporal_load(reinterpret_cast<const lr_v2*>(rp + coff[c]));
                    v0[e][c] = t.x;
                    v1[e][c] = t.y;
                } else {
                    v0[e][c] = rp[coff[c]];
                    v1[e][c] = rp[ok1[c] ? coff[c] + 1 : 0];
                }
            }
            ynv[e] = a.y[rr];
            yov[e] = a.y_old[rr];
            ulv[e] = own ? Up[rr] : T(0);
        }
#pragma unroll
        for (int e = 0; e < UNR; ++e) {
            if (g0 + e < ge) {
                const size_t row = 4 * (g0 + e) + q;
                const bool rok = row < m;
                T yn = ynv[e];
                const T yo = yov[e], ul = ulv[e];
                T s = ul * cp;
#pragma unroll
                for (int c = 0; c < NCP; ++c) s += v0[e][c] * d0[c] + v1[e][c] * d1[c];
                s = sum16(s);
                T u = nd * ((yo - yn) + s);
                if (!rok) { u = 0; yn = 0; }
                if (rok && p == 0) Uk[row] = u;
#pragma unroll
                for (int c = 0; c < NCP; ++c) {
                    va0[c] += v0[e][c] * u;
                    va1[c] += v1[e][c] * u;
                    ga0[c] += v0[e][c] * yn;
                    ga1[c] += v1[e][c] * yn;
                }
                wl += ul * u;
                hl += ul * yn;
                uu += u * u;
                uy += u * yn;
                yy = dfma(yn, yn, yy);
            }
        }
    }

    auto qsum = [](T v) { v += wave_shfl_xor(v, 16); v += wave_shfl_xor(v, 32); return v; };
#pragma unroll
    for (int c = 0; c < NCP; ++c) { va0[c] = qsum(va0[c]); va1[c] = qsum(va1[c]); ga0[c] = qsum(ga0[c]); ga1[c] = qsum(ga1[c]); }
    wl = qsum(wl); hl = qsum(hl); uu = qsum(uu); uy = qsum(uy); yy = qsum(yy);
    if (q == 0) {
#pragma unroll
        for (int c = 0; c < NCP; ++c) {
            if (ok0[c]) { red[wave][coff[c]] = va0[c]; red[wave][n + coff[c]] = ga0[c]; }
            if (ok1[c]) { red[wave][coff[c] + 1] = va1[c]; red[wave][n + coff[c] + 1] = ga1[c]; }
        }
        red[wave][2 * n + p] = wl;
        red[wave][2 * n + kLrMax + p] = hl;
        if (p == 0) { red[wave][2 * n + 2 * kLrMax] = uu; red[wave][2 * n + 2 * kLrMax + 1] = uy; red[wave][lr_yy(n)] = yy; }
    }
    __syncthreads();
    const int len = lr_len(n);
    T* out = a.partials + (size_t)blockIdx.x * len;
    for (int e = threadIdx.x; e < len; e += blockDim.x) out[e] = (red[0][e] + red[1][e]) + (red[2][e] + red[3][e]);
}

template <typename T>
__global__ __launch_bounds__(32 * kReduceRanges) void k_lr_reduce(const T* __restrict__ partials, int nparts, int len, T* __restrict__ out)
{
    __shared__ T part[kReduceRanges][33];
    const int es = threadIdx.x & 31, sp = threadIdx.x >> 5;
    const int e = blockIdx.x * 32 + es;
    T s = 0;
    if (e < len) {
        const int per = (nparts + kReduceRanges - 1) / kReduceRanges;
        const int b0 = sp * per, b1 = (b0 + per < nparts) ? b0 + per : nparts;
#pragma unroll 8
        for (int b = b0; b < b1; ++b) s += partials[(size_t)b * len + e];
    }
    part[sp][es] = s;
    __syncthreads();
    if (sp == 0 && e < len) {
        T tot = part[0][es];
#pragma unroll
        for (int r = 1; r < kReduceRanges; ++r) tot += part[r][es];
        out[e] = tot;
    }
}

template <typename T>
__device__ inline T lr_reduce_scalar(const T* __restrict__ partials, int nparts, T* part )
{
    if ((int)threadIdx.x < kReduceRanges) {
        const int per = (nparts + kReduceRanges - 1) / kReduceRanges;
        const int b0 = (int)threadIdx.x * per, b1 = (b0 + per < nparts) ? b0 + per : nparts;
        T s = 0;
#pragma unroll 8
        for (int b = b0; b < b1; ++b) s += partials[b];
        part[threadIdx.x] = s;
    }
    __syncthreads();
    T tot = part[0];
#pragma unroll
    for (int r = 1; r < kReduceRanges; ++r) tot += part[r];
    __syncthreads();
    return tot;
}

template <typename T>
__global__ __launch_bounds__(256) void k_lr_sumsq(const T* __restrict__ v0, size_t m, size_t vstride, T* __restrict__ partials0, int pstride)
{
    __shared__ T red[4];
    const int lane = threadIdx.x & 63, wave = threadIdx.x >> 6;
    const T* __restrict__ v = v0 + (size_t)blockIdx.y * vstride;
    const size_t G = (m + 3) / 4;
    const size_t nw = (size_t)gridDim.x * 4, wid = (size_t)blockIdx.x * 4 + wave;
    const size_t per = (G + nw - 1) / nw;
    const size_t gb = wid * per;
    const size_t ge = gb + per < G ? gb + per : G;
    const T yy = lr_wave_sumsq(v, m, gb, ge, lane >> 4);
    if (lane == 0) red[wave] = yy;
    __syncthreads();
    if (threadIdx.x == 0) partials0[(size_t)blockIdx.y * pstride + blockIdx.x] = (red[0] + red[1]) + (red[2] + red[3]);
}
template <typename T>
__global__ __launch_bounds__(256) void k_lr_sumsq_final(const T* __restrict__ partials0, int pstride, int nparts, T* __restrict__ out)
{
    __shared__ T part[kReduceRanges];
    const T tot = lr_reduce_scalar(partials0 + (size_t)blockIdx.x * pstride, nparts, part);
    if (threadIdx.x == 0) out[blockIdx.x] = tot;
}

template <typename T>
__global__ __launch_bounds__(256) void k_lr_finish(const T* __restrict__ lr, T* __restrict__ D, const T* __restrict__ dx,
                                                   int k, int n, T* __restrict__ JJ, T* __restrict__ Jy, LmState<T>* st)
{
    __shared__ T v[kLrMaxN];
    __shared__ T red[4];
    const T* __restrict__ w = lr + 2 * n;
    const T* __restrict__ h = w + kLrMax;
    const T uu = lr[2 * n + 2 * kLrMax], uy = lr[2 * n + 2 * kLrMax + 1];
    const int i = blockIdx.x;
    if (i < n) {
        for (int j = threadIdx.x; j < n; j += blockDim.x) {
            T s = lr[j];
            for (int l = 0; l < k; ++l) s = dfma(D[(size_t)l * n + j], w[l], s);
            v[j] = s;
        }
        __syncthreads();
        for (int j = threadIdx.x; j < n; j += blockDim.x) {
            const int r = i >= j ? i : j, c = i >= j ? j : i;
            JJ[(size_t)i * n + j] += lr_jj_term(v[r], v[c], dx[r], dx[c], uu);
        }
        return;
    }
    T mx = 0;
    for (int j = threadIdx.x; j < n; j += blockDim.x) {
        T s = lr[n + j];
        for (int l = 0; l < k; ++l) s = dfma(D[(size_t)l * n + j], h[l], s);
        s = dfma(dx[j], uy, s);
        Jy[j] = s;
        const T av = dabs(s);
        if (av > mx) mx = av;
        D[(size_t)k * n + j] = dx[j];
    }
    mx = wave_max(mx);
    if ((threadIdx.x & 63) == 0) red[threadIdx.x >> 6] = mx;
    __syncthreads();
    if (threadIdx.x == 0) {
        T r = red[0];
        for (int wv = 1; wv < (int)(blockDim.x >> 6); ++wv) r = red[wv] > r ? red[wv] : r;
        st->jy_inf = r;
    }
}

template <typename T, int NCP, bool VEC>
__global__ __launch_bounds__(256) void k_lr_flush(T* J, const T* __restrict__ U, const T* __restrict__ D,
                                                  int k, size_t m, int n)
{
    using P2 = typename LrPair<T>::type;
    extern __shared__ unsigned char lr_smem[];
    T* Ds = reinterpret_cast<T*>(lr_smem);
    for (int e = threadIdx.x; e < k * n; e += blockDim.x) Ds[e] = D[e];
    __syncthreads();
    const int lane = threadIdx.x & 63;
    const int q = lane >> 4, p = lane & 15;
    int coff[NCP];
    bool ok0[NCP], ok1[NCP];
#pragma unroll
    for (int c = 0; c < NCP; ++c) {
        const int col = 32 * c + 2 * p;
        ok0[c] = col < n;
        ok1[c] = col + 1 < n;
        coff[c] = ok0[c] ? col : 0;
    }
    const size_t G = (m + 3) / 4;
    const size_t wave_id = ((size_t)blockIdx.x * blockDim.x + threadIdx.x) >> 6;
    const size_t nwaves = ((size_t)gridDim.x * blockDim.x) >> 6;
    for (size_t g = wave_id; g < G; g += nwaves) {
        const size_t row = 4 * g + q;
        const bool rok = row < m;
        const size_t rr = rok ? row : m - 1;
        T* rp = J + rr * (size_t)n;
        const T* sp = rp;
        T v0[NCP], v1[NCP];
#pragma unroll
        for (int c = 0; c < NCP; ++c) {
            if constexpr (VEC) {
                typedef T lr_v2 __attribute__((ext_vector_type(2)));
                const lr_v2 t = __builtin_nontemporal_load(reinterpret_cast<const lr_v2*>(sp + coff[c]));
                v0[c] = t.x;
                v1[c] = t.y;
            } else {
                v0[c] = sp[coff[c]];
                v1[c] = sp[ok1[c] ? coff[c] + 1 : 0];
            }
        }
        for (int l = 0; l < k; ++l) {
            const T ul = U[(size_t)l * m + rr];
#pragma unroll
            for (int c = 0; c < NCP; ++c) {
                v0[c] += ul * Ds[l * n + coff[c]];
                v1[c] += ul * Ds[l * n + (ok1[c] ? coff[c] + 1 : 0)];
            }
        }
        if (rok) {
#pragma unroll
            for (int c = 0; c < NCP; ++c) {
                if constexpr (VEC) {
                    if (ok0[c]) {
                        typedef T lr_v2 __attribute__((ext_vector_type(2)));
                        lr_v2 t; t.x = v0[c]; t.y = v1[c];
                        __builtin_nontemporal_store(t, reinterpret_cast<lr_v2*>(rp + coff[c]));
                    }
                } else {
                    if (ok0[c]) rp[coff[c]] = v0[c];
                    if (ok1[c]) rp[coff[c] + 1] = v1[c];
                }
            }
        }
    }
}

}
```

mir_optim_amd/csrc/launch_broyden.hip:

```cpp
#include <hip/hip_runtime.h>

#include "broyden_launch.h"
#include "launch_util.h"
#include "broyden_lr.h"

namespace mirlsq {

namespace {
template <typename T, int NCP>
hipError_t lr_sweep_ncp(const LrArgs<T>& a, int nblk, bool vec, hipStream_t s)
{
    if (vec) MIRLSQ_LAUNCH((k_broyden_lr<T, NCP, true>), dim3(nblk), dim3(256), 0, s, a);
    else MIRLSQ_LAUNCH((k_broyden_lr<T, NCP, false>), dim3(nblk), dim3(256), 0, s, a);
    return hipGetLastError();
}
}
template <typename T>
hipError_t lr_sweep(const LrArgs<T>& a, int nblk, hipStream_t s)
{
    if (a.n > kLrMaxN || a.k < 0 || a.k >= kLrMax) return hipErrorInvalidValue;
    const bool vec = (a.n % 2 == 0) && (reinterpret_cast<uintptr_t>(a.J) % (2 * sizeof(T)) == 0);
    const int ncp = (a.n + 31) / 32;
    if (ncp <= 1) return lr_sweep_ncp<T, 1>(a, nblk, vec, s);
    if (ncp <= 2) return lr_sweep_ncp<T, 2>(a, nblk, vec, s);
    if (ncp <= 4) return lr_sweep_ncp<T, 4>(a, nblk, vec, s);
    if (ncp <= 8) return lr_sweep_ncp<T, 8>(a, nblk, vec, s);
    return lr_sweep_ncp<T, 16>(a, nblk, vec, s);
}

namespace {
template <typename T, int NCP>
hipError_t lr_flush_ncp(T* J, const T* U, const T* D, int k, size_t m, int n, int nblk, bool vec, hipStream_t s)
{
    const size_t lds = (size_t)k * n * sizeof(T);
    if (vec) MIRLSQ_LAUNCH((k_lr_flush<T, NCP, true>), dim3(nblk), dim3(256), lds, s, J, U, D, k, m, n);
    else MIRLSQ_LAUNCH((k_lr_flush<T, NCP, false>), dim3(nblk), dim3(256), lds, s, J, U, D, k, m, n);
    return hipGetLastError();
}
}
template <typename T>
hipError_t lr_flush(T* J, const T* U, const T* D, int k, size_t m, int n, int num_cu, hipStream_t s)
{
    if (k <= 0) return hipSuccess;
    if (n > kLrMaxN || k > kLrMax) return hipErrorInvalidValue;
    const size_t G = (m + 3) / 4;
    size_t blocks = (G + 3) / 4;
    if (blocks > (size_t)num_cu * 8) blocks = (size_t)num_cu * 8;
    if (blocks < 1) blocks = 1;
    const bool vec = (n % 2 == 0) && (reinterpret_cast<uintptr_t>(J) % (2 * sizeof(T)) == 0);
    const int ncp = (n + 31) / 32;
    if (ncp <= 1) return lr_flush_ncp<T, 1>(J, U, D, k, m, n, (int)blocks, vec, s);
    if (ncp <= 2) return lr_flush_ncp<T, 2>(J, U, D, k, m, n, (int)blocks, vec, s);
    if (ncp <= 4) return lr_flush_ncp<T, 4>(J, U, D, k, m, n, (int)blocks, vec, s);
    if (ncp <= 8) return lr_flush_ncp<T, 8>(J, U, D, k, m, n, (int)blocks, vec, s);
    return lr_flush_ncp<T, 16>(J, U, D, k, m, n, (int)blocks, vec, s);
}

template <typename T>
hipError_t lr_reduce(const T* partials, int nblk, int n, T* out, hipStream_t s)
{
    const int len = lr_len(n);
    MIRLSQ_LAUNCH(k_lr_reduce<T>, dim3((len + 31) / 32), dim3(32 * kReduceRanges), 0, s, partials, nblk, len, out);
    return hipGetLastError();
}

template <typename T>
hipError_t lr_finish(const T* lr, T* D, const T* dx, int k, int n, T* JJ, T* Jy, LmState<T>* st, hipStream_t s)
{
    MIRLSQ_LAUNCH(k_lr_finish<T>, dim3(n + 1), dim3(256), 0, s, lr, D, dx, k, n, JJ, Jy, st);
    return hipGetLastError();
}

template <typename T>
hipError_t lr_sumsq(const T* v, size_t m, int count, size_t vstride, T* partials, int pstride, int nblk, hipStream_t s)
{
    if (count < 1 || nblk < 1 || nblk > pstride) return hipErrorInvalidValue;
    MIRLSQ_LAUNCH(k_lr_sumsq<T>, dim3(nblk, count), dim3(256), 0, s, v, m, vstride, partials, pstride);
    return hipGetLastError();
}
template <typename T>
hipError_t lr_sumsq_final(const T* partials, int pstride, int nblk, int count, T* out, hipStream_t s)
{
    MIRLSQ_LAUNCH(k_lr_sumsq_final<T>, dim3(count), dim3(256), 0, s, partials, pstride, nblk, out);
    return hipGetLastError();
}

#define MIRLSQ_INSTANTIATE(T)                                                                                             \
    template hipError_t lr_sweep<T>(const LrArgs<T>&, int, hipStream_t);                                                  \
    template hipError_t lr_reduce<T>(const T*, int, int, T*, hipStream_t);                                                \
    template hipError_t lr_finish<T>(const T*, T*, const T*, int, int, T*, T*, LmState<T>*, hipStream_t);                 \
    template hipError_t lr_sumsq<T>(const T*, size_t, int, size_t, T*, int, int, hipStream_t);                            \
    template hipError_t lr_sumsq_final<T>(const T*, int, int, int, T*, hipStream_t);                                      \
    template hipError_t lr_flush<T>(T*, const T*, const T*, int, size_t, int, int, hipStream_t);
MIRLSQ_INSTANTIATE(double)
MIRLSQ_INSTANTIATE(float)
#undef MIRLSQ_INSTANTIATE

}

MIRLSQ_DEFINE_PRELOAD(broyden)
```

mir_optim_amd/csrc/solver_jacobian.hip:

```cpp
#include "driver.h"
#include "launch_util.h"
#include "misc_kernels.h"

namespace mirlsq {

template <typename T>
bool Solver<T>::broyden_lowrank(const T* y_dev, const T* yold_dev)
{
    T* U = static_cast<T*>(ws->ulr);
    if (lr_k >= lr_cap) {
        const uint64_t launches_before = launches_now();
        struct Excl { Solver* s; uint64_t l0; ~Excl() { s->launches_excluded += s->launches_now() - l0; } } excl{this, launches_before};
        if (!ok(lr_flush<T>(B.J, U, B.lrD, lr_k, m, (int)n, ws->num_cu, stream), "broyden flush")) return false;
        lr_k = 0;
        if (stats) stats->broyden_flushes++;
        if (!plain_products(yold_dev)) return false;
        if (stats) stats->jtj_resyncs++;
    }
    LrArgs<T> a{};
    a.J = B.J; a.U = U; a.D = B.lrD; a.dx = B.dx_acc; a.dx_dot = &B.st->dx_dot; a.y = y_dev; a.y_old = yold_dev;
    a.partials = B.lrpart; a.m = m; a.n = (int)n; a.k = lr_k;
    const int nblk = lr_blocks(m, ws->num_cu), len = lr_len((int)n);
    ev_begin(1);
    if (!ok(lr_sweep<T>(a, nblk, stream), "broyden sweep")) return false;
    ev_end();
    if (!ok(lr_reduce<T>(B.lrpart, nblk, (int)n, B.lrvec, stream), "broyden reduce")) return false;
    if (comm && !allreduce(B.lrvec, (size_t)len, 1)) return false;
    if (!ok(lr_finish<T>(B.lrvec, B.lrD, B.dx_acc, lr_k, (int)n, B.JJ, B.Jy, B.st, stream), "broyden finish")) return false;
    if (stats) stats->broyden_lr_columns += (uint64_t)lr_k;
    ++lr_k;
    return true;
}

template <typename T>
bool Solver<T>::plain_products(const T* y_vec)
{
    JtjArgs<T> a{};
    a.J = B.J; a.Jout = B.J; a.y = y_vec; a.y_old = y_vec; a.dx = B.dx_acc; a.dx_dot = &B.st->dx_dot;
    a.slabs = B.slabs; a.m = m; a.n = (int)n;
    const bool direct = unpack_in_reduce(JtjOp::plain);
    ev_begin(0);
    if (!ok(jtj_run<T>(plan, JtjOp::plain, a, B.packed, stream, direct ? unpack_target() : JtjUnpack<T>{}), "jtj kernel")) return false;
    ev_end();
    return finish_products(direct);
}

template <typename T>
bool Solver<T>::finish_products(bool direct)
{
    if (direct) return ok(hipGetLastError(), "jtj reduce");
    if (comm && !allreduce(B.packed, (size_t)n * (n + 1) / 2 + n, 0)) return false;
    return ok(jtj_unpack<T>(B.packed, (int)n, B.JJ, B.Jy, B.st, stream), "unpack");
}

template <typename T>
bool Solver<T>::jacobian_products(bool broyden, const T* y_dev, const T* yold_dev)
{
    if (broyden && lowrank) return broyden_lowrank(y_dev, yold_dev);
    if (!broyden) lr_k = 0;
    JtjArgs<T> a{};
    a.J = B.J; a.Jout = B.J; a.y = y_dev; a.y_old = yold_dev; a.dx = B.dx_acc; a.dx_dot = &B.st->dx_dot;
    a.slabs = B.slabs; a.m = m; a.n = (int)n;
    if (!broyden && fd_fused) {
        const JtjOp op = fd_fused == 2 ? JtjOp::fd_diff : JtjOp::fd;
        fd_fused = 0;
        a.J = static_cast<const T*>(ws->ypanel); a.twh = B.twh;
        const bool direct = unpack_in_reduce(op);
        ev_begin(3);
        if (!ok(jtj_run<T>(plan, op, a, B.packed, stream, direct ? unpack_target() : JtjUnpack<T>{}), "fd + jtj kernel")) return false;
        ev_end();
        return finish_products(direct);
    }
    const JtjOp op = broyden ? JtjOp::rewrite : JtjOp::plain;
    const bool direct = unpack_in_reduce(op);
    ev_begin(broyden ? 1 : 0);
    if (!ok(jtj_run<T>(plan, op, a, B.packed, stream, direct ? unpack_target() : JtjUnpack<T>{}), "jtj kernel")) return false;
    ev_end();
    return finish_products(direct);
}

template <typename T>
bool Solver<T>::fd_device()
{
    MIRLSQ_LAUNCH(k_fd_points<T>, dim3(n), dim3(64), 0, stream, B.x, B.lower, B.upper, sd.jacobianEpsilon, (int)n, B.X, B.twh);
    for (uint32_t j = 0; j < n; ++j) {
        const T save = xh[j];
        T xmh = save - S->jacobianEpsilon, xph = save + S->jacobianEpsilon;
        xmh = std::fmax(xmh, lh[j]);
        xph = std::fmin(xph, uh[j]);
        twh_h[j] = xph - xmh;
    }
    size_t pb = n;
    size_t cap = (size_t)64 << 30;
    if (ws->ypanel_bytes < 2 * pb * m * sizeof(T)) {
        size_t free_b = 0, total_b = 0;
        if (hipMemGetInfo(&free_b, &total_b) == hipSuccess) {
            const size_t have = ws->ypanel_bytes + free_b;
            if (have / 2 < cap) cap = have / 2;
        }
        if (cap < ((size_t)1 << 30)) cap = (size_t)1 << 30;
    }
    if (2 * pb * m * sizeof(T) > cap) {
        pb = cap / (2 * m * sizeof(T));
        if (pb >= 64) pb -= pb % 64;
    }
    if (pb < 1) pb = 1;
    if (fb && fd_batch && fd_batch / 2 < pb) pb = fd_batch / 2 ? fd_batch / 2 : 1;
    const bool no_fuse = (variant & MIR_LSQ_VARIANT_FD_SEPARATE_FILL) != 0;
    const bool use_diff = fbd && plan.fd_diff.kernel != JtjKernel::none && pb == n && !no_fuse;
    const size_t need = (use_diff ? 1 : 2) * pb * m * sizeof(T);
    if (ws->ypanel_bytes < need) {
        if (ws->ypanel) (void)hipFree(ws->ypanel);
        ws->ypanel = nullptr; ws->ypanel_bytes = 0;
        if (!ok(hipMalloc(&ws->ypanel, need), "hipMalloc(FD panel)")) return false;
        ws->ypanel_bytes = need;
    }
    T* Y = static_cast<T*>(ws->ypanel);
    if (use_diff) {
        ev_begin(4);
        fbd(fbctx, m, n, 2 * (size_t)n, B.X, Y);
        ev_end();
        if (stats) { stats->fd_callback_points += 2 * (uint64_t)n; stats->fd_callback_calls++; }
        fd_fused = 2;
        ret.fCalls += n;
        return ok(hipGetLastError(), "fd batched callback");
    }
    if (fbr && plan.fd.kernel != JtjKernel::none && pb == n && !no_fuse) {
        ev_begin(4);
        fbr(fbctx, m, n, 2 * (size_t)n, B.X, Y);
        ev_end();
        if (stats) { stats->fd_callback_points += 2 * (uint64_t)n; stats->fd_callback_calls++; }
        fd_fused = 1;
        ret.fCalls += n;
        return ok(hipGetLastError(), "fd batched callback");
    }
    for (size_t j0 = 0; j0 < n; j0 += pb) {
        const size_t pc = (j0 + pb <= n) ? pb : n - j0;
        ev_begin(4);
        if (fb) {
            fb(fbctx, m, n, 2 * pc, B.X + 2 * j0 * n, Y);
            if (stats) stats->fd_callback_points += 2 * (uint64_t)pc;
        } else {
            for (size_t c = 0; c < pc; ++c) {
                if (twh_h[j0 + c] == 0) continue;
                f(fctx, m, n, B.X + (2 * (j0 + c)) * n, Y + (2 * c) * m);
                f(fctx, m, n, B.X + (2 * (j0 + c) + 1) * n, Y + (2 * c + 1) * m);
                if (stats) stats->fd_callback_points += 2;
            }
        }
        ev_end();
        if (stats) stats->fd_callback_calls++;
        dim3 grid((unsigned)((m + 63) / 64), (unsigned)((pc + 31) / 32));
        MIRLSQ_LAUNCH(k_fd_fill<T>, grid, dim3(256), 0, stream, Y, m, B.twh, B.J, m, (int)n, (int)j0, (int)pc);
    }
    ret.fCalls += n;
    return ok(hipGetLastError(), "fd fill");
}

template <typename T>
void Solver<T>::fd_task_trampoline(mir_least_squares_task task, uint32_t totalThreads, uint32_t threadId, uint32_t j)
{
    static_cast<Solver<T>*>(task.context)->fd_task(totalThreads, threadId, j);
}
template <typename T>
void Solver<T>::fd_task(uint32_t totalThreads, uint32_t threadId, uint32_t j)
{
    const uint32_t idx = totalThreads >= n ? j : threadId;
    if (idx >= n || j >= n) { fd_failed = true; return; }
    ++fd_tasks_run;
    if (hipSetDevice(device) != hipSuccess) { fd_failed = true; return; }
    Slot* s;
    {
        std::lock_guard<std::mutex> lk(fd_mutex);
        s = &slots[idx];
        if (!s->p) {
            s->p = static_cast<T*>(std::malloc(n * sizeof(T)));
            if (!s->p) { fd_failed = true; return; }
        }
        if (!fd_panel_mode && !s->yp) {
            if (hipHostMalloc((void**)&s->yp, m * sizeof(T), hipHostMallocDefault) != hipSuccess
                || hipHostMalloc((void**)&s->ym, m * sizeof(T), hipHostMallocDefault) != hipSuccess) {
                fd_failed = true;
                return;
            }
        }
        if (slot_count[idx]++ == 0) std::memcpy(s->p, xh, n * sizeof(T));
    }
    T* p = s->p;
    const T save = p[j];
    T xmh = save - S->jacobianEpsilon, xph = save + S->jacobianEpsilon;
    xmh = std::fmax(xmh, lh[j]);
    xph = std::fmin(xph, uh[j]);
    const T twh = xph - xmh;
    if (fd_panel_mode) {
        if (twh != 0) {
            T* hp = static_cast<T*>(ws->pinned_panel) + (size_t)(2 * j) * m;
            const auto t0 = std::chrono::steady_clock::now();
            p[j] = xph;
            f(fctx, m, n, p, hp);
            p[j] = xmh;
            f(fctx, m, n, p, hp + m);
            p[j] = save;
            fd_f_ns += (uint64_t)std::chrono::duration_cast<std::chrono::nanoseconds>(std::chrono::steady_clock::now() - t0).count();
            const int k = (int)(idx % mir_lsq_workspace::kCopyStreams);
            fd_streams_used |= 1u << k;
            if (hipMemcpyAsync(static_cast<T*>(ws->ypanel) + (size_t)(2 * j) * m, hp, 2 * m * sizeof(T), hipMemcpyHostToDevice,
                               ws->copy_stream[k]) != hipSuccess)
                fd_failed = true;
        }
        return;
    }
    if (twh != 0) {
        p[j] = xph;
        f(fctx, m, n, p, s->yp);
        p[j] = xmh;
        f(fctx, m, n, p, s->ym);
        p[j] = save;
    }
    std::lock_guard<std::mutex> lk(fd_mutex);
    if (twh != 0) {
        if (hipMemcpyAsync(mB, s->yp, m * sizeof(T), hipMemcpyHostToDevice, stream) != hipSuccess
            || hipMemcpyAsync(fr, s->ym, m * sizeof(T), hipMemcpyHostToDevice, stream) != hipSuccess) {
            fd_failed = true;
            return;
        }
    }
    hipLaunchKernelGGL(k_fd_fill_col<T>, dim3((unsigned)((m + 255) / 256)), dim3(256), 0, stream, mB, fr, twh, B.J, m, (int)n, (int)j);
    worker_launches.fetch_add(1, std::memory_order_relaxed);
    if (hipStreamSynchronize(stream) != hipSuccess) fd_failed = true;
}
template <typename T>
bool Solver<T>::fd_host_prepare_panel()
{
    if (variant & MIR_LSQ_VARIANT_FD_HOST_COLUMNS) return false;
    const size_t need = 2 * (size_t)n * m * sizeof(T);
    if (need > ((size_t)16 << 30)) return false;
    if (ws->ypanel_bytes < need) {
        size_t free_b = 0, total_b = 0;
        if (hipMemGetInfo(&free_b, &total_b) != hipSuccess) return false;
        size_t cap = (ws->ypanel_bytes + free_b) / 2;
        if (cap > ((size_t)64 << 30)) cap = (size_t)64 << 30;
        if (need > cap) return false;
        if (ws->ypanel) (void)hipFree(ws->ypanel);
        ws->ypanel = nullptr; ws->ypanel_bytes = 0;
        if (hipMalloc(&ws->ypanel, need) != hipSuccess) return false;
        ws->ypanel_bytes = need;
    }
    if (ws->pinned_panel_bytes < need) {
        if (ws->pinned_panel) (void)hipHostFree(ws->pinned_panel);
        ws->pinned_panel = nullptr; ws->pinned_panel_bytes = 0;
        if (hipHostMalloc(&ws->pinned_panel, need, hipHostMallocDefault) != hipSuccess) return false;
        ws->pinned_panel_bytes = need;
    }
    for (int k = 0; k < mir_lsq_workspace::kCopyStreams; ++k) {
        if (!ws->copy_stream[k] && hipStreamCreateWithFlags(&ws->copy_stream[k], hipStreamNonBlocking) != hipSuccess) return false;
        if (!ws->copy_event[k] && hipEventCreateWithFlags(&ws->copy_event[k], hipEventDisableTiming) != hipSuccess) return false;
    }
    return true;
}
template <typename T>
bool Solver<T>::fd_host()
{
    slots.resize(n);
    slot_count.assign(n, 0);
    fd_panel_mode = fd_host_prepare_panel();
    fd_streams_used = 0;
    fd_tasks_run = 0;
    if (fd_panel_mode) {
        MIRLSQ_LAUNCH(k_fd_points<T>, dim3(n), dim3(64), 0, stream, B.x, B.lower, B.upper, sd.jacobianEpsilon, (int)n, B.X, B.twh);
    }
    mir_least_squares_task task{this, nullptr};
    const auto t0 = std::chrono::steady_clock::now();
    if (tm) tm(tmctx, n, task, &fd_task_trampoline);
    else for (uint32_t j = 0; j < n; ++j) fd_task(1, 0, j);
    uint32_t calls = 0;
    for (uint32_t k = 0; k < n; ++k) calls += (uint32_t)slot_count[k];
    ret.fCalls += calls;
    if (stats) {
        stats->fd_host_wall_ms += std::chrono::duration<double, std::milli>(std::chrono::steady_clock::now() - t0).count();
        stats->fd_host_f_ms += (double)fd_f_ns.exchange(0) * 1e-6;
        stats->fd_host_columns += n;
    }
    const bool incomplete = fd_tasks_run.load() != n;
    if (incomplete)
        std::fprintf(stderr, "[mir_optim_amd] thread manager ran %u of %u finite-difference tasks\n", fd_tasks_run.load(), n);
    if (incomplete || fd_failed) {
        if (fd_panel_mode)
            for (int k = 0; k < mir_lsq_workspace::kCopyStreams; ++k)
                if (fd_streams_used.load() & (1u << k)) (void)hipStreamSynchronize(ws->copy_stream[k]);
        return false;
    }
    if (fd_panel_mode) {
        const uint32_t used = fd_streams_used.load();
        for (int k = 0; k < mir_lsq_workspace::kCopyStreams; ++k) {
            if (!(used & (1u << k))) continue;
            if (!ok(hipEventRecord(ws->copy_event[k], ws->copy_stream[k]), "copy event")
                || !ok(hipStreamWaitEvent(stream, ws->copy_event[k], 0), "wait for the panel copies")) return false;
        }
        dim3 grid((unsigned)((m + 63) / 64), (unsigned)((n + 31) / 32));
        MIRLSQ_LAUNCH(k_fd_fill<T>, grid, dim3(256), 0, stream, static_cast<const T*>(ws->ypanel), m, B.twh, B.J, m, (int)n, 0, (int)n);
        return ok(hipGetLastError(), "fd fill");
    }
    return true;
}

template <typename T>
bool Solver<T>::analytic_jacobian()
{
    if (device_cb) {
        g(gctx, m, n, B.x, B.J);
    } else {
        if (!ws->pinned_J && !ok(hipHostMalloc(&ws->pinned_J, m * n * sizeof(T), hipHostMallocDefault), "hipHostMalloc(J)")) return false;
        T* Jh = static_cast<T*>(ws->pinned_J);
        g(gctx, m, n, xh, Jh);
        if (!ok(hipMemcpyAsync(B.J, Jh, m * n * sizeof(T), hipMemcpyHostToDevice, stream), "H2D J")
            || !ok(hipStreamSynchronize(stream), "sync")) return false;
    }
    ret.gCalls += 1;
    return true;
}

#define MIRLSQ_INSTANTIATE(T)                                                                       \
    template bool Solver<T>::broyden_lowrank(const T*, const T*);                                   \
    template bool Solver<T>::plain_products(const T*);                                              \
    template bool Solver<T>::finish_products(bool);                                                 \
    template bool Solver<T>::jacobian_products(bool, const T*, const T*);                           \
    template bool Solver<T>::fd_device();                                                           \
    template void Solver<T>::fd_task_trampoline(mir_least_squares_task, uint32_t, uint32_t, uint32_t); \
    template void Solver<T>::fd_task(uint32_t, uint32_t, uint32_t);                                 \
    template bool Solver<T>::fd_host_prepare_panel();                                               \
    template bool Solver<T>::fd_host();                                                             \
    template bool Solver<T>::analytic_jacobian();
MIRLSQ_INSTANTIATE(double)
MIRLSQ_INSTANTIATE(float)
#undef MIRLSQ_INSTANTIATE

}

MIRLSQ_DEFINE_PRELOAD(jacobian)
```

mir_optim_amd/csrc/solver_loop.hip:

```cpp
#include "driver.h"
#include "launch_util.h"
#include "misc_kernels.h"

namespace mirlsq {

template <typename T>
void Solver<T>::ev_begin(int kind)
{
    if (!time_kernels) return;
    HpScope hp(this, 0);
    EventPair p{};
    p.kind = spec_enqueue ? kind + 100 : kind;
    if (ws->event_pool.size() < 2 * (events.size() + 1)) {
        hipEvent_t ea, eb;
        (void)hipEventCreate(&ea);
        (void)hipEventCreate(&eb);
        ws->event_pool.push_back(ea);
        ws->event_pool.push_back(eb);
    }
    p.a = ws->event_pool[2 * events.size()];
    p.b = ws->event_pool[2 * events.size() + 1];
    (void)hipEventRecord(p.a, stream);
    events.push_back(p);
}
template <typename T>
void Solver<T>::ev_end()
{
    if (!time_kernels) return;
    HpScope hp(this, 0);
    (void)hipEventRecord(events.back().b, stream);
}

template <typename T>
bool Solver<T>::setup()
{
    if (!ws) {
        ws = workspace_create<T>(m, n);
        own_ws = true;
        if (!ws) return false;
    } else if (ws->m != m || ws->n != n || ws->elem != sizeof(T)) {
        std::fprintf(stderr, "[mir_optim_amd] workspace shape mismatch\n");
        ws = nullptr;
        return false;
    }
    if (hipGetDevice(&caller_device) != hipSuccess) caller_device = ws->device;
    if (caller_device != ws->device && !ok(hipSetDevice(ws->device), "hipSetDevice")) return false;
    plan = jtj_plan<T>(m, (int)n, ws->num_cu);
    B = carve<T>(ws->dev, m, n, ws->num_cu);
    device = ws->device;
    for (int k = 0; k < 2; ++k) {
        st_slot[k] = reinterpret_cast<LmState<T>*>(ws->pinned) + k;
        st_slot_d[k] = reinterpret_cast<LmState<T>*>(ws->pinned_dev) + k;
        x_slot[k] = reinterpret_cast<T*>(static_cast<char*>(ws->pinned) + 2 * sizeof(LmState<T>)) + (size_t)k * n;
        x_slot_d[k] = reinterpret_cast<T*>(static_cast<char*>(ws->pinned_dev) + 2 * sizeof(LmState<T>)) + (size_t)k * n;
        st_slot[k]->seq = 0;
    }
    st_h = st_slot[0];
    trial_h = reinterpret_cast<T*>(static_cast<char*>(ws->pinned) + 2 * sizeof(LmState<T>)) + 2 * (size_t)n;
    if (!stream) {
        if (!ok(hipStreamCreate(&stream), "hipStreamCreate")) return false;
        own_stream = true;
    }
    sd = lm_settings_dev(S);
    dbg_solve = (variant & MIR_LSQ_VARIANT_DEBUG_SOLVE) != 0;
    no_speculation = (variant & MIR_LSQ_VARIANT_NO_SPECULATION) != 0;
    lowrank = (variant & MIR_LSQ_VARIANT_BROYDEN_REWRITE) == 0;
    no_null_skip = (variant & MIR_LSQ_VARIANT_NO_NULL_SKIP) != 0;
    host_profile = (variant & MIR_LSQ_VARIANT_HOST_PROFILE) != 0;
    {
        const int v = (int)((variant >> MIR_LSQ_VARIANT_LR_CAP_SHIFT) & 31u);
        if (v >= 1 && v <= kLrMax) lr_cap = v;
    }
    y = B.y;
    mB = B.mB;
    fr = B.ytmp;
    big_solve = n > (uint32_t)kSolveMaxN || (variant & MIR_LSQ_VARIANT_SOLVE_GENERIC) != 0;
    if (n > (uint32_t)kLrMaxN) lowrank = false;
    fused = device_cb && lowrank && !big_solve && !trace && !(variant & MIR_LSQ_VARIANT_NO_PIPELINE);
    twh_h.resize(n);
    char* stage = static_cast<char*>(ws->pinned) + align_up(2 * sizeof(LmState<T>) + (3 * (size_t)n + 8) * sizeof(T), 256);
    const size_t ol = (size_t)(reinterpret_cast<char*>(B.lower) - reinterpret_cast<char*>(B.x));
    const size_t ou = (size_t)(reinterpret_cast<char*>(B.upper) - reinterpret_cast<char*>(B.x));
    std::memcpy(stage, xh, n * sizeof(T));
    std::memcpy(stage + ol, lh, n * sizeof(T));
    std::memcpy(stage + ou, uh, n * sizeof(T));
    return ok(hipMemcpyAsync(B.x, stage, ou + n * sizeof(T), hipMemcpyHostToDevice, stream), "H2D x, l, u");
}

template <typename T>
void Solver<T>::teardown()
{
    if (stream) (void)hipStreamSynchronize(stream);
    if (host_profile) std::fprintf(stderr, "[host profile] J %p  FD panel %p  y %p\n", (void*)B.J, ws ? ws->ypanel : nullptr, (void*)B.y);
    if (host_profile)
        std::fprintf(stderr, "[host profile] events %.3f ms  all-reduce calls %.3f  trial callbacks %.3f  readback+sync %.3f  solve launch %.3f  "
                             "longest single call %.3f\n", hp_ms[0], hp_ms[1], hp_ms[2], hp_ms[3], hp_ms[4], hp_ms[5]);
    if (stats) {
        for (auto& e : events) {
            if (e.kind < 0 || e.kind >= 100) continue;
            float ms = 0;
            (void)hipEventElapsedTime(&ms, e.a, e.b);
            if (e.kind == 0) { stats->jtj_ms += ms; stats->jtj_launches++; }
            else if (e.kind == 1) { stats->jtj_ms += ms; stats->jtj_launches++; stats->jtj_broyden_ms += ms; stats->jtj_broyden_launches++; }
            else if (e.kind == 2) { stats->solve_ms += ms; stats->solve_launches++; }
            else if (e.kind == 3) { stats->jtj_ms += ms; stats->jtj_launches++; stats->jtj_fd_ms += ms; stats->jtj_fd_launches++; }
            else if (e.kind == 4) stats->fd_callback_ms += ms;
            else if (e.kind == 5) stats->trial_callback_ms += ms;
        }
    }
    events.clear();
    for (auto& s : slots) {
        if (s.p) std::free(s.p);
        if (s.yp) (void)hipHostFree(s.yp);
        if (s.ym) (void)hipHostFree(s.ym);
    }
    slots.clear();
    if (own_stream && stream) (void)hipStreamDestroy(stream);
    if (ws && caller_device >= 0 && caller_device != ws->device) (void)hipSetDevice(caller_device);
    if (own_ws && ws) workspace_destroy(ws);
}

template <typename T>
bool Solver<T>::eval_f(const T* x_dev, const T* x_host, T* y_dev)
{
    if (device_cb) {
        f(fctx, m, n, x_dev, y_dev);
        return true;
    }
    if (!ws->pinned_y && !ok(hipHostMalloc(&ws->pinned_y, m * sizeof(T), hipHostMallocDefault), "hipHostMalloc(y)")) return false;
    T* yh = static_cast<T*>(ws->pinned_y);
    const auto t0 = std::chrono::steady_clock::now();
    f(fctx, m, n, x_host, yh);
    if (stats) { stats->host_f_ms += std::chrono::duration<double, std::milli>(std::chrono::steady_clock::now() - t0).count(); stats->host_f_calls++; }
    return ok(hipMemcpyAsync(y_dev, yh, m * sizeof(T), hipMemcpyHostToDevice, stream), "H2D y")
        && ok(hipStreamSynchronize(stream), "sync");
}

template <typename T>
int Solver<T>::sumsq_blocks() const
{
    int nb = (int)((m + 4095) / 4096);
    if (nb > kPartials) nb = kPartials;
    return nb < 1 ? 1 : nb;
}
template <typename T>
bool Solver<T>::sumsq(const T* v, int slot)
{
    const int nb = sumsq_blocks();
    MIRLSQ_LAUNCH(k_sumsq_partial<T>, dim3(nb), dim3(256), 0, stream, v, m, B.partials, (size_t)0, kPartials);
    MIRLSQ_LAUNCH(k_sumsq_final<T>, dim3(1), dim3(256), 0, stream, B.partials, nb, B.sum + slot, kPartials);
    if (comm && !allreduce(B.sum + slot, 1, 2)) return false;
    return ok(hipGetLastError(), "sumsq");
}

template <typename T>
bool Solver<T>::trial_sums(const T* v, int count, size_t vstride)
{
    static_assert(kPartials >= kLrMaxBlocks, "one partial per workgroup of the sweep's grid");
    const int nb = lr_blocks(m, ws->num_cu);
    if (!ok(lr_sumsq<T>(v, m, count, vstride, B.partials, kPartials, nb, stream), "trial sums")) return false;
    if (!comm) { sums_pending = nb; return true; }
    if (!ok(lr_sumsq_final<T>(B.partials, kPartials, nb, count, B.sum + 1, stream), "trial sums, stage 2")) return false;
    return allreduce(B.sum + 1, (size_t)count, 2);
}

template <typename T>
bool Solver<T>::allreduce(T* buf, size_t count, int kind)
{
    HpScope hp(this, 1);
    if (stats && !spec_enqueue) { stats->allreduce_calls[kind]++; stats->allreduce_elems[kind] += count; }
    return comm_allreduce<T>(comm, buf, count, stream) == 0;
}

template <typename T>
void Solver<T>::trace_emit(int event, uint32_t iterations, T lambda, T residual, T trial_residual, T dx_dot)
{
    if (!trace) return;
    if (trace->count < trace->capacity && trace->records) {
        mir_lsq_trace_record& r = trace->records[trace->count];
        r.event = event; r.iterations = iterations; r.lambda = (double)lambda; r.residual = (double)residual;
        r.trial_residual = (double)trial_residual; r.dx_dot = (double)dx_dot;
    }
    trace->count++;
}
template <typename T>
bool Solver<T>::trace_round(int ks, T residual_before, uint32_t iterations_before)
{
    ChainRec<T> rec[kChainMax];
    T sums[kChainMax];
    if (!ok(hipMemcpyAsync(rec, B.rec, (size_t)ks * sizeof(ChainRec<T>), hipMemcpyDeviceToHost, stream), "D2H rec")
        || !ok(hipMemcpyAsync(sums, B.sum + 1, (size_t)ks * sizeof(T), hipMemcpyDeviceToHost, stream), "D2H sums")
        || !ok(hipStreamSynchronize(stream), "sync"))
        return false;
    const int dec = st_h->decision;
    if (dec == kDecideGradSmall || dec == kDecideNumericError) return true;
    for (uint32_t k = 0; k < st_h->consumed && k < (uint32_t)ks; ++k) {
        if (rec[k].flags & kFlagStepTooLong)
            trace_emit(4, iterations_before, rec[k].lambda, residual_before, 0, rec[k].new_dx_dot);
        else if ((int)k != st_h->accepted_k)
            trace_emit(2, iterations_before, rec[k].lambda, residual_before, sums[k], rec[k].new_dx_dot);
        else
            trace_emit(3, iterations_before + 1, rec[k].lambda, sums[k], sums[k], rec[k].new_dx_dot);
    }
    return true;
}

template <typename T>
bool Solver<T>::wait_state(uint32_t expect)
{
    HpScope hp(this, 3);
    st_h = st_slot[expect & 1];
    x_h = x_slot[expect & 1];
    volatile uint32_t* sq = &st_h->seq;
    constexpr double kWaitBoundSeconds = 600.0;
    std::chrono::steady_clock::time_point t_wait{};
    for (uint64_t spins = 0;; ++spins) {
        if (*sq == expect) break;
        if ((spins & 0xfff) == 0xfff) {
            const hipError_t q = hipStreamQuery(stream);
            if (q == hipSuccess) {
                if (*sq == expect) break;
                std::fprintf(stderr, "[mir_optim_amd] decision point %u was not published\n", expect);
                return false;
            }
            if (q != hipErrorNotReady) return ok(q, "stream query");
            const auto now = std::chrono::steady_clock::now();
            if (t_wait == std::chrono::steady_clock::time_point{}) t_wait = now;
            else if (std::chrono::duration<double>(now - t_wait).count() > kWaitBoundSeconds) {
                std::fprintf(stderr, "[mir_optim_amd] decision point %u: no progress for %.0f s, giving up\n", expect, kWaitBoundSeconds);
                return false;
            }
        }
        if (spins < 20000) cpu_relax(); else std::this_thread::yield();
    }
    std::atomic_thread_fence(std::memory_order_acquire);
    return true;
}

template <typename T>
bool Solver<T>::read_state(const T* vec_dev)
{
    HpScope hp(this, 3);
    if (!ok(hipMemcpyAsync(st_h, B.st, sizeof(LmState<T>), hipMemcpyDeviceToHost, stream), "D2H state")) return false;
    if (vec_dev && !ok(hipMemcpyAsync(trial_h, vec_dev, n * sizeof(T), hipMemcpyDeviceToHost, stream), "D2H vec")) return false;
    return ok(hipStreamSynchronize(stream), "sync");
}

template <typename T>
void Solver<T>::print_solve_dbg(bool fused_round)
{
    long long h[32];
    if (hipMemcpy(h, B.sc[0].dbg, sizeof h, hipMemcpyDeviceToHost) != hipSuccess) return;
    if (fused_round)
        std::fprintf(stderr, "[solve dbg] fused round head (10ns ticks): decision + publication %lld (loads landed %lld, decided + point copied %lld, fence + sequence number %lld)  n x n side of the Broyden pass %lld\n", h[27] - h[26], h[29] - h[26], h[30] - h[29], h[31] - h[30], h[28] - h[27]);
    std::fprintf(stderr, "[solve dbg] (10ns ticks) build %lld  copy/equil %lld  scale %lld  potrf %lld  potrs %lld  refine %lld  epilogue %lld  total %lld  shader MHz %.0f  [matvec1 %lld berr %lld]\n",
                 h[1] - h[0], h[2] - h[1], h[3] - h[2], h[4] - h[3], h[5] - h[4], h[6] - h[5], h[8] - h[7], h[8] - h[0], (double)(h[10] - h[9]) / (double)(h[8] - h[0]) * 100.0, h[11] - h[5], h[12] - h[11]);
    if (n <= 128)
        std::fprintf(stderr, "[solve dbg] load (10ns ticks): kernel entry -> loads landed %lld (of which inside posvx %lld)  reduction + LDS commit %lld  rest of the phase %lld\n",
                     h[24] - h[0], h[24] - h[2], h[25] - h[24], h[3] - h[25]);
    if (n <= 128)
        std::fprintf(stderr, "[solve dbg] refinement (10ns ticks): residual 1 %lld  berr 1 %lld  potrs 2 %lld  residual 2 %lld  rest %lld  (correction applied: %lld)\n",
                     h[11] - h[5], h[12] - h[11], h[13] - h[12], h[14] - h[13], h[6] - h[14], h[15]);
    if (n <= 128)
        std::fprintf(stderr, "[solve dbg] lds_potrf, wave 0 (shader cycles, summed over the panels): diagonal update + factor %lld  wait %lld  rows below %lld  wait %lld\n", h[20], h[21], h[22], h[23]);
    if (n > 128)
        std::fprintf(stderr, "[solve dbg] potrf_panel steps (10ns ticks, summed over the panels): earlier panels on MFMA %lld (of which publishing / waiting for the helpers' look-ahead jobs %lld)  diagonal rows %lld  other rows + store %lld\n", h[16], h[19], h[17], h[18]);
}

template <typename T>
LmSolveArgs<T> Solver<T>::solve_args(int ks, const T* lam, bool check_grad, bool lambda_from_state)
{
    LmSolveArgs<T> a{};
    a.JJ = B.JJ; a.Jy = B.Jy; a.x = B.x; a.lower = B.lower; a.upper = B.upper;
    a.dx = B.dx; a.trial = B.trial; a.st = B.st; a.rec = B.rec; a.set = sd; a.n = (int)n;
    for (int k = 0; k < kChainMax; ++k) { a.sc[k] = B.sc[k]; a.lam[k] = (lam && k < ks) ? lam[k] : T(0); }
    a.f_in_lds = solve_nb((int)n, (int)sizeof(T)) > 0;
    a.check_grad = check_grad ? 1 : 0;
    a.lambda_from_state = lambda_from_state ? 1 : 0;
    if (!dbg_solve) a.sc[0].dbg = nullptr;
    a.coop_w = (big_solve && n > (uint32_t)kSolveMaxN && !(variant & MIR_LSQ_VARIANT_SOLVE_ONE_WORKGROUP) && !coop_disabled) ? coop_peers((int)n) : 1;
    if (a.coop_w > ws->num_cu / 2) a.coop_w = ws->num_cu / 2 >= 2 ? ws->num_cu / 2 : 1;
    a.coop_epoch = a.coop_w > 1 ? ++ws->solve_epoch : 0;
    a.coop_absent = (variant & MIR_LSQ_VARIANT_DEBUG_HELPERS_ABSENT) ? 1 : 0;
    return a;
}
template <typename T>
bool Solver<T>::enqueue_solve(int ks, const T* lam, bool check_grad, bool lambda_from_state)
{
    const LmSolveArgs<T> a = solve_args(ks, lam, check_grad, lambda_from_state);
    ev_begin(2);
    {
        HpScope hp(this, 4);
        if (!ok(launch_lm_solve<T>(a, ks, has_bounds, big_solve, stream), "solve launch")) return false;
    }
    ev_end();
    return true;
}

template <typename T>
DecideArgs<T> Solver<T>::decide_args(int ks, bool check_grad, bool lambda_from_state)
{
    DecideArgs<T> d{};
    d.sums = B.sum + 1; d.rec = B.rec; d.st = B.st; d.set = sd; d.x = B.x; d.trial = B.trial; d.dx_chain = B.dx;
    d.dx_acc = B.dx_acc; d.n = (int)n; d.ks = ks; d.check_grad = check_grad ? 1 : 0;
    d.lambda_from_state = lambda_from_state ? 1 : 0;
    ++seq;
    d.host_st = st_slot_d[seq & 1]; d.host_x = x_slot_d[seq & 1]; d.seq = seq;
    d.maxIterations = S->maxIterations;
    d.partials = B.partials; d.nparts = sums_pending; d.pstride = kPartials;
    sums_pending = 0;
    return d;
}
template <typename T>
bool Solver<T>::enqueue_decide(int ks, bool check_grad, bool lambda_from_state, const T* sum_v)
{
    if (sum_v && !trial_sums(sum_v, ks, m)) return false;
    const DecideArgs<T> d = decide_args(ks, check_grad, lambda_from_state);
    MIRLSQ_LAUNCH(k_decide_chain<T>, dim3(1), dim3(kSolveThreads), 0, stream, d);
    return ok(hipGetLastError(), "decide kernel");
}

template <typename T>
bool Solver<T>::enqueue_fused_tail(const T* ytr, bool check_grad, bool lambda_from_state)
{
    spec_events_from = events.size();
    if (stats) stats->fused_rounds++;
    LrArgs<T> a{};
    a.J = B.J; a.U = static_cast<T*>(ws->ulr); a.D = B.lrD; a.dx = B.dx; a.dx_dot = &B.rec[0].new_dx_dot; a.y = ytr; a.y_old = y;
    a.partials = B.lrpart; a.m = m; a.n = (int)n; a.k = lr_k;
    a.spec_rec = B.rec; a.absTolerance = sd.absTolerance; a.relTolerance = sd.relTolerance;
    const int nblk = lr_blocks(m, ws->num_cu), len = lr_len((int)n);
    spec_enqueue = true;
    ev_begin(1);
    const bool swept = ok(lr_sweep<T>(a, nblk, stream), "broyden sweep");
    ev_end();
    spec_enqueue = false;
    if (!swept || !ok(lr_reduce<T>(B.lrpart, nblk, (int)n, B.lrvec, stream), "broyden reduce")) return false;
    if (comm && !allreduce(B.lrvec, (size_t)len, 1)) return false;
    LmSolveArgs<T> sa = solve_args(1, nullptr, true, false);
    sa.lambda_from_device = 1;
    sa.fused = 1;
    sa.dec = decide_args(1, check_grad, lambda_from_state);
    sa.dec.sums = B.lrvec + lr_yy((int)n);
    sa.dec.spec_static = 1;
    sa.fin_lr = B.lrvec; sa.fin_D = B.lrD; sa.fin_JJ = B.JJ; sa.fin_Jy = B.Jy; sa.fin_k = lr_k;
    spec_enqueue = true;
    ev_begin(2);
    bool good;
    {
        HpScope hp(this, 4);
        good = ok(launch_lm_solve<T>(sa, 1, has_bounds, false, stream), "fused round launch");
    }
    ev_end();
    spec_enqueue = false;
    return good;
}
template <typename T>
void Solver<T>::commit_spec_round()
{
    for (size_t i = spec_events_from; i < events.size(); ++i) if (events[i].kind >= 100) events[i].kind -= 100;
    if (stats) {
        stats->jacobian_broyden++;
        stats->fused_passes++;
        stats->broyden_lr_columns += (uint64_t)lr_k;
    }
    ++lr_k;
}
template <typename T>
void Solver<T>::drop_spec_round()
{
    for (size_t i = spec_events_from; i < events.size(); ++i) if (events[i].kind >= 100) events[i].kind = -1;
}

template <typename T>
typename Solver<T>::Result Solver<T>::run()
{
    ret.status = mir_ls_numericError; ret.iterations = 0; ret.fCalls = 0; ret.gCalls = 0;
    ret.residual = Lim<T>::inf(); ret.lambda = 0;
    const auto t_start = std::chrono::steady_clock::now();
    launches_mark = launches_now();

    {
        bool finite = true;
        for (uint32_t i = 0; i < n; ++i) if (!(-Lim<T>::inf() < xh[i] && xh[i] < Lim<T>::inf())) finite = false;
        if (m == 0 || n == 0 || !finite) { ret.status = mir_ls_badGuess; return ret; }
        for (uint32_t i = 0; i < n; ++i) if (!(lh[i] <= xh[i]) || !(xh[i] <= uh[i])) { ret.status = mir_ls_badBounds; return ret; }
        if (const int bad = bad_settings(S)) { ret.status = bad; return ret; }
    }
    if (!device_available()) return ret;
    if (!setup()) { teardown(); return ret; }
    has_bounds = (variant & MIR_LSQ_VARIANT_SOLVE_BOUNDED) != 0;
    for (uint32_t i = 0; i < n; ++i)
        if (lh[i] > -Lim<T>::inf() || uh[i] < Lim<T>::inf()) has_bounds = true;

    const uint32_t maxAge = S->maxAge ? S->maxAge : (g ? 3 : 2 * n);

    bool fail = false;
    do {
        if (!eval_f(B.x, xh, y)) { fail = true; break; }
        ++ret.fCalls;
        ++seq;
        if (!sumsq(y, 0)) { fail = true; break; }
        MIRLSQ_LAUNCH(k_init_state<T>, dim3(1), dim3(1), 0, stream, B.sum, B.st, st_slot_d[seq & 1], seq);
        if (!ok(hipGetLastError(), "init state") || !wait_state(seq)) { fail = true; break; }
    } while (false);
    if (fail) { teardown(); ret.status = mir_ls_numericError; return ret; }

    ret.residual = st_h->residual;
    bool fConverged = LM_F_CONVERGED(ret.residual, sd);
    bool needJacobian = true;
    bool last_rejected = false;
    bool spec_live = false;
    bool spec_predict = true;
    const bool speculate = device_cb && !no_speculation;
    uint32_t age = maxAge;
    ret.lambda = 0;
    T mu = 1;
    ret.status = mir_ls_maxIterations;

    do {
        close_round();
        if (stats) stats->passes++;
        if (fConverged) { ret.status = mir_ls_fConverged; break; }
        if (!LM_LAMBDA_IN_RANGE(ret.lambda, sd)) { ret.status = mir_ls_furtherImprovement; break; }
        if (mu > kSuspiciousMu && age) {
            needJacobian = true;
            age = maxAge;
            mu = 1;
            MIRLSQ_LAUNCH(k_reset_mu<T>, dim3(1), dim3(1), 0, stream, B.st);
        }
        {
            bool nan = false;
            for (uint32_t i = 0; i < n; ++i) if (!(xh[i] <= xh[i])) nan = true;
            if (nan) { ret.status = mir_ls_numericError; break; }
        }
        bool newJacobian = false;
        int ks = 1;
        bool lambda_from_state = false, skip_eval = false;
        T* ytr = fr;
        bool solve_enqueued = false;
        if (spec_live) {
            spec_live = false;
            if (!needJacobian || !(age < maxAge) || lr_k >= lr_cap) {
                std::fprintf(stderr, "[mir_optim_amd] internal error: the pass run ahead by the fused round is not the next pass\n");
                fail = true;
                break;
            }
            needJacobian = false;
            newJacobian = true;
            last_rejected = false;
            age++;
            commit_spec_round();
            solve_enqueued = true;
        }
        round_kind = solve_enqueued ? 1 : 2;
        if (needJacobian) {
            needJacobian = false;
            newJacobian = true;
            last_rejected = false;
            round_kind = age < maxAge ? 1 : 0;
            if (age < maxAge) {
                age++;
                if (stats) stats->jacobian_broyden++;
                if (!jacobian_products(true, y, mB)) { fail = true; break; }
                trace_emit(1, ret.iterations, ret.lambda, ret.residual, 0, st_h->dx_dot);
            } else {
                age = 0;
                if (stats) stats->jacobian_full++;
                const auto t0 = std::chrono::steady_clock::now();
                bool okj;
                if (g) okj = analytic_jacobian();
                else okj = device_cb ? fd_device() : fd_host();
                if (!okj) { fail = true; break; }
                if (stats && !device_cb)
                    stats->fd_ms += std::chrono::duration<double, std::milli>(std::chrono::steady_clock::now() - t0).count();
                if (!jacobian_products(false, y, mB)) { fail = true; break; }
                trace_emit(0, ret.iterations, ret.lambda, ret.residual, 0, st_h->dx_dot);
            }
        }

        lambda_from_state = !solve_enqueued && !LM_LAMBDA_SET(ret.lambda, sd);
        T lam[kChainMax];
        lam[0] = ret.lambda;
        if (speculate && !newJacobian && !lambda_from_state && last_rejected) {
            T l2 = ret.lambda, m2 = mu;
            while (ks < kChainMax) {
                LM_REJECT(l2, m2, sd);
                if (!LM_LAMBDA_IN_RANGE(l2, sd)) break;
                if (m2 > kSuspiciousMu && age) break;
                lam[ks++] = l2;
            }
        }
        if (!solve_enqueued && !enqueue_solve(ks, lam, newJacobian, lambda_from_state)) { fail = true; break; }
        if (dbg_solve && !solve_enqueued) print_solve_dbg(false);

        if (device_cb && tail_null && last_rejected && !newJacobian && !no_null_skip) {
            HpScope hp(this, 3);
            ChainRec<T> rr[kChainMax];
            if (!ok(hipMemcpyAsync(rr, B.rec, (size_t)ks * sizeof(ChainRec<T>), hipMemcpyDeviceToHost, stream), "D2H rec")
                || !ok(hipStreamSynchronize(stream), "sync")) { fail = true; break; }
            skip_eval = true;
            for (int k = 0; k < ks; ++k) if (!(rr[k].flags & kFlagNullStep)) skip_eval = false;
            if (skip_eval && stats) stats->elided_evaluations += (uint64_t)ks;
        }

        if (ks > 1) ytr = static_cast<T*>(ws->ytrial);
        if (skip_eval) {
        } else if (device_cb) {
            HpScope hp(this, 2);
            ev_begin(5);
            if (ks > 1 && fb) fb(fbctx, m, n, (size_t)ks, B.trial, ytr);
            else for (int k = 0; k < ks; ++k) f(fctx, m, n, B.trial + (size_t)k * n, ytr + (size_t)k * m);
            ev_end();
            if (stats) { stats->trial_callback_points += (uint64_t)ks; stats->trial_callback_calls++; }
        } else {
            ChainRec<T> r0;
            if (!ok(hipMemcpyAsync(&r0, B.rec, sizeof r0, hipMemcpyDeviceToHost, stream), "D2H rec") || !read_state(B.trial)) { fail = true; break; }
            const bool null_step = (r0.flags & kFlagNullStep) && !no_null_skip;
            if (null_step && stats) stats->elided_evaluations++;
            const bool no_f = (newJacobian && (r0.flags & kFlagGradSmall)) || r0.qp_status != 0
                || (r0.flags & (kFlagDxNaN | kFlagStepTooLong)) || null_step;
            if (!no_f && !eval_f(B.trial, trial_h, ytr)) { fail = true; break; }
        }

        const bool fuse = fused && spec_predict && ks == 1 && !skip_eval && age < maxAge && lr_k < lr_cap;
        if (fuse ? !enqueue_fused_tail(ytr, newJacobian, lambda_from_state)
                 : !enqueue_decide(ks, newJacobian, lambda_from_state, skip_eval ? nullptr : ytr)) { fail = true; break; }
        const uint32_t round_seq = seq;
        if (!wait_state(round_seq)) { fail = true; break; }
        if (fuse) {
            if (st_h->spec_ok) spec_live = true; else drop_spec_round();
            if (dbg_solve && spec_live) print_solve_dbg(true);
        }
        if (ks == 1 && newJacobian) spec_predict = st_h->decision == kDecideAccept;

        if (trace && !trace_round(ks, ret.residual, ret.iterations)) { fail = true; break; }
        if (st_h->coop_rescued) {
            if (stats) stats->coop_timeouts += st_h->coop_rescued;
            coop_disabled = true;
        }
        const int dec = st_h->decision;
        tail_null = st_h->null_tail != 0;
        ret.fCalls += st_h->fcalls;
        if (stats) {
            if (st_h->consumed > 1) stats->passes += st_h->consumed - 1;
            stats->rejected += st_h->rejects;
            stats->step_guard_rejects += st_h->guards;
            stats->qp_active_set_passes += st_h->qp_active;
        }
        if (dec == kDecideGradSmall) {
            if (age == 0) { ret.status = mir_ls_gConverged; break; }
            age = maxAge;
            continue;
        }
        ret.lambda = st_h->lambda;
        mu = st_h->mu;
        if (dec == kDecideNumericError) { ret.status = mir_ls_numericError; break; }
        if (dec == kDecideReject) { last_rejected = true; continue; }
        last_rejected = false;

        needJacobian = true;
        ret.iterations = st_h->iterations;
        for (uint32_t i = 0; i < n; ++i) xh[i] = x_h[i];
        if (ytr != fr) {
            if (!ok(hipMemcpyAsync(fr, ytr + (size_t)st_h->accepted_k * m, m * sizeof(T), hipMemcpyDeviceToDevice, stream), "D2D y")) { fail = true; break; }
        }
        { T* t = mB; mB = y; y = fr; fr = t; }
        ret.residual = st_h->residual;
        fConverged = LM_F_CONVERGED(ret.residual, sd);
        if (stats) stats->accepted++;

        if (dec == kDecideAcceptNoPrediction) { ret.status = mir_ls_furtherImprovement; break; }

        const T dxn = std::sqrt(st_h->dx_dot);
        if (!LM_X_MOVING(dxn, st_h->trial_xnorm, sd)) {
            if (age == 0) { ret.status = mir_ls_xConverged; break; }
            age = maxAge;
            continue;
        }
    } while (ret.iterations < S->maxIterations);

    close_round();
    if (fail) ret.status = mir_ls_numericError;
    if (stats) stats->total_ms += std::chrono::duration<double, std::milli>(std::chrono::steady_clock::now() - t_start).count();
    teardown();
    return ret;
}

template <typename T>
void Solver<T>::apply_options(const mir_lsq_gpu_options* opt)
{
    Solver<T>& s = *this;
    if (!opt) return;
    s.device_cb = (opt->flags & MIR_LSQ_DEVICE_CALLBACKS) != 0;
    s.time_kernels = (opt->flags & MIR_LSQ_TIME_KERNELS) != 0 && opt->stats;
    s.stream = static_cast<hipStream_t>(opt->stream);
    s.comm = opt->comm;
    s.ws = opt->workspace;
    s.fbctx = opt->fbContext;
    s.fb = s.device_cb ? reinterpret_cast<typename Abi<T>::FB>(opt->fb) : nullptr;
    s.fd_batch = opt->fd_batch;
    s.variant = opt->variant;
    if (opt->stats) {
        size_t bytes = opt->struct_size >= offsetof(mir_lsq_gpu_options, fbRowMajorDiff) + sizeof(void*)
            ? offsetof(mir_lsq_stats, trial_callback_points) + sizeof(uint64_t)
            : (opt->struct_size >= offsetof(mir_lsq_gpu_options, fbRowMajor) + sizeof(void*)
                   ? offsetof(mir_lsq_stats, jtj_fd_launches) + sizeof(uint64_t)
                   : offsetof(mir_lsq_stats, qp_active_set_passes) + sizeof(uint64_t));
        if (opt->struct_size >= offsetof(mir_lsq_gpu_options, stats_size) + sizeof(uint32_t) && opt->stats_size)
            bytes = opt->stats_size;
        if (bytes > sizeof(mir_lsq_stats)) bytes = sizeof(mir_lsq_stats);
        s.stats_user = opt->stats;
        s.stats_bytes = bytes;
        std::memcpy(&s.stats_local, opt->stats, bytes);
        s.stats = &s.stats_local;
    }
    if (opt->struct_size >= offsetof(mir_lsq_gpu_options, trace) + sizeof(void*)) s.trace = opt->trace;
    if (opt->struct_size >= offsetof(mir_lsq_gpu_options, fbRowMajor) + sizeof(void*) && s.device_cb)
        s.fbr = reinterpret_cast<typename Abi<T>::FB>(opt->fbRowMajor);
    if (opt->struct_size >= offsetof(mir_lsq_gpu_options, fbRowMajorDiff) + sizeof(void*) && s.device_cb)
        s.fbd = reinterpret_cast<typename Abi<T>::FB>(opt->fbRowMajorDiff);
}

template <typename T>
typename Abi<T>::Result solve_entry(const typename Abi<T>::Settings* settings, size_t m, size_t n, T* x, const T* l,
                                    const T* u, const mir_lsq_gpu_options* opt, void* fctx, typename Abi<T>::F f,
                                    void* gctx, typename Abi<T>::G g, void* tmctx, mir_least_squares_thread_manager tm)
{
    Solver<T> s{};
    s.S = settings; s.m = m; s.n = (uint32_t)n; s.xh = x; s.lh = l; s.uh = u;
    s.fctx = fctx; s.f = f; s.gctx = gctx; s.g = g; s.tmctx = tmctx; s.tm = tm;
    s.apply_options(opt);
    if (s.trace) s.trace->count = 0;
    const typename Abi<T>::Result r = s.run();
    if (s.stats_user) std::memcpy(s.stats_user, &s.stats_local, s.stats_bytes);
    return r;
}

#define MIRLSQ_INSTANTIATE(T)                                                                                                   \
    template struct Solver<T>;                                                                                                  \
    template Abi<T>::Result solve_entry<T>(const Abi<T>::Settings*, size_t, size_t, T*, const T*, const T*, const mir_lsq_gpu_options*, \
                                           void*, Abi<T>::F, void*, Abi<T>::G, void*, mir_least_squares_thread_manager);
MIRLSQ_INSTANTIATE(double)
MIRLSQ_INSTANTIATE(float)
#undef MIRLSQ_INSTANTIATE

}

MIRLSQ_DEFINE_PRELOAD(loop)
```

mir_optim_amd/csrc/unit_entries.hip:

```cpp
#include "driver.h"
#include "misc_kernels.h"

using namespace mirlsq;

namespace {
__global__ __launch_bounds__(256) void k_selftest_reductions(int rounds, uint32_t seed, int* out)
{
#pragma clang fp contract(off)
    uint32_t sr = seed ^ (0x9E3779B9u * (blockIdx.x * blockDim.x + threadIdx.x + 1));
    auto rnd = [&]() { sr ^= sr << 13; sr ^= sr >> 17; sr ^= sr << 5; return sr; };
    int bad[4] = {0, 0, 0, 0};
    for (int it = 0; it < rounds; ++it) {
        const float f = (float)(int32_t)rnd() * (1.0f / 65536.0f) * ((it & 7) == 0 ? 1e-20f : 1.0f);
        const double d = ((double)(int32_t)rnd() + (double)rnd() * 2.3283064365386963e-10) * ((it & 3) == 0 ? 1e-200 : 1.0);
        auto ref_sum = [](auto v) {
            v += __shfl_xor(v, 8, kWave); v += __shfl_xor(v, 4, kWave); v += __shfl_xor(v, 2, kWave); v += __shfl_xor(v, 1, kWave);
            v += __shfl_xor(v, 16, kWave); v += __shfl_xor(v, 32, kWave);
            return v;
        };
        auto ref_max = [](auto v) {
            for (int m : {8, 4, 2, 1, 16, 32}) { const auto o = __shfl_xor(v, m, kWave); v = o > v ? o : v; }
            return v;
        };
        const float sf = wave_sum(f), rf = ref_sum(f);
        const double sd = wave_sum(d), rdd = ref_sum(d);
        bad[0] += __float_as_uint(sf) != __float_as_uint(rf);
        bad[1] += __double_as_longlong(sd) != __double_as_longlong(rdd);
        bad[2] += __float_as_uint(wave_max(f)) != __float_as_uint(ref_max(f));
        bad[3] += __double_as_longlong(wave_max(d)) != __double_as_longlong(ref_max(d));
    }
    for (int k = 0; k < 4; ++k) if (bad[k]) atomicAdd(out + k, bad[k]);
}

template <typename T, typename QS>
int box_qp_entry(const QS* settings, size_t n_, const T* P, const T* q, const T* l, const T* u, T* x,
                 int unconstrainedSolution, int* iterations)
{
    if (iterations) *iterations = 0;
    if (n_ == 0) return mir_box_qp_solved;
    if (!device_available()) return mir_box_qp_numericError;
    const int n = (int)n_;
    size_t off = 0;
    auto take = [&](size_t bytes) { size_t o = off; off = align_up(off + bytes, 256); return o; };
    const size_t oP = take(sizeof(T) * n * n), oq = take(sizeof(T) * n), ol = take(sizeof(T) * n), ou = take(sizeof(T) * n),
                 ox = take(sizeof(T) * n), oPm = take(sizeof(T) * n * n), oA = take(sizeof(T) * n * n),
                 oF = take(sizeof(T) * n * (n | 1)), ov = take(sizeof(T) * 12 * n), oi = take(sizeof(int32_t) * 2 * n),
                 oo = take(sizeof(int) * 4);
    char* base = nullptr;
    if (hipMalloc((void**)&base, off) != hipSuccess) return mir_box_qp_numericError;
    BoxQpArgs<T> a{};
    a.P = (T*)(base + oP); a.q = (T*)(base + oq); a.l = (T*)(base + ol); a.u = (T*)(base + ou); a.x = (T*)(base + ox);
    a.sc.Pm = (T*)(base + oPm); a.sc.A = (T*)(base + oA); a.sc.Fg = (T*)(base + oF); a.sc.vec = (T*)(base + ov);
    a.sc.ivec = (int32_t*)(base + oi); a.out = (int*)(base + oo); a.sc.dbg = nullptr;
    a.relTol = settings->relTolerance; a.absTol = settings->absTolerance; a.maxIterations = settings->maxIterations;
    a.unconstrained = unconstrainedSolution; a.n = n;
    a.f_in_lds = solve_nb(n, (int)sizeof(T)) > 0;
    int out[2] = {mir_box_qp_numericError, 0};
    bool good = hipMemcpy((void*)a.P, P, sizeof(T) * n * n, hipMemcpyHostToDevice) == hipSuccess
        && hipMemcpy((void*)a.q, q, sizeof(T) * n, hipMemcpyHostToDevice) == hipSuccess
        && hipMemcpy((void*)a.l, l, sizeof(T) * n, hipMemcpyHostToDevice) == hipSuccess
        && hipMemcpy((void*)a.u, u, sizeof(T) * n, hipMemcpyHostToDevice) == hipSuccess
        && hipMemcpy((void*)a.x, x, sizeof(T) * n, hipMemcpyHostToDevice) == hipSuccess;
    if (good) good = launch_box_qp<T>(a, nullptr) == hipSuccess;
    if (good) {
        good = hipGetLastError() == hipSuccess && hipDeviceSynchronize() == hipSuccess
            && hipMemcpy(out, a.out, sizeof(out), hipMemcpyDeviceToHost) == hipSuccess
            && hipMemcpy(x, a.x, sizeof(T) * n, hipMemcpyDeviceToHost) == hipSuccess;
    }
    (void)hipFree(base);
    if (!good) return mir_box_qp_numericError;
    if (iterations) *iterations = out[1];
    return out[0];
}

template <typename T>
int jtj_entry(size_t m, size_t n, T* J, const T* y, const T* y_old, const T* dx, int broyden, T* JJ, T* Jy,
              void* stream_, float* kernel_ms)
{
    if (!device_available()) return -1;
    if (n == 0 || m == 0) return -2;
    hipStream_t stream = static_cast<hipStream_t>(stream_);
    const JtjPlan plan = jtj_plan<T>(m, (int)n, query_num_cu());
    const size_t packed_len = n * (n + 1) / 2 + n + 8;
    T *slabs = nullptr, *packed = nullptr, *dxdot = nullptr;
    LmState<T>* st = nullptr;
    const size_t slab_count = jtj_slab_elems(plan);
    if (hipMalloc((void**)&slabs, sizeof(T) * slab_count) != hipSuccess) return -3;
    if (hipMalloc((void**)&packed, sizeof(T) * packed_len) != hipSuccess) { (void)hipFree(slabs); return -3; }
    if (hipMalloc((void**)&st, sizeof(LmState<T>) + sizeof(T) * 8) != hipSuccess) { (void)hipFree(slabs); (void)hipFree(packed); return -3; }
    dxdot = reinterpret_cast<T*>(st + 1);
    int rc = 0;
    if (broyden) {
        hipLaunchKernelGGL(k_sumsq_partial<T>, dim3(1), dim3(256), 0, stream, dx, n, packed);
        hipLaunchKernelGGL(k_sumsq_final<T>, dim3(1), dim3(256), 0, stream, packed, 1, dxdot);
    }
    JtjArgs<T> a{};
    a.J = J; a.Jout = J; a.y = y; a.y_old = y_old; a.dx = dx; a.dx_dot = dxdot; a.slabs = slabs; a.m = m; a.n = (int)n;
    hipEvent_t e0, e1;
    (void)hipEventCreate(&e0); (void)hipEventCreate(&e1);
    (void)hipEventRecord(e0, stream);
    if (jtj_run<T>(plan, broyden ? JtjOp::rewrite : JtjOp::plain, a, packed, stream) != hipSuccess) rc = -4;
    (void)hipEventRecord(e1, stream);
    (void)jtj_unpack<T>(packed, (int)n, JJ, Jy, st, stream);
    if (hipStreamSynchronize(stream) != hipSuccess) rc = -5;
    if (kernel_ms) { float ms = 0; (void)hipEventElapsedTime(&ms, e0, e1); *kernel_ms = ms; }
    (void)hipEventDestroy(e0); (void)hipEventDestroy(e1);
    (void)hipFree(slabs); (void)hipFree(packed); (void)hipFree(st);
    return rc;
}
int fd_jtj_entry(size_t m, size_t n, const double* Yrm, const double* twh, const double* y, double* J,
                 double* JJ, double* Jy, void* stream_, float* kernel_ms, bool diff)
{
    if (!device_available()) return -1;
    if (n == 0 || m == 0) return -2;
    hipStream_t stream = static_cast<hipStream_t>(stream_);
    const JtjPlan plan = jtj_plan<double>(m, (int)n, query_num_cu());
    const JtjOp op = diff ? JtjOp::fd_diff : JtjOp::fd;
    if (plan.of(op).kernel == JtjKernel::none) return -6;
    const size_t packed_len = n * (n + 1) / 2 + n + 8;
    double *slabs = nullptr, *packed = nullptr;
    LmState<double>* st = nullptr;
    const size_t slab_count = jtj_slab_elems(plan);
    if (hipMalloc((void**)&slabs, sizeof(double) * slab_count) != hipSuccess) return -3;
    if (hipMalloc((void**)&packed, sizeof(double) * packed_len) != hipSuccess) { (void)hipFree(slabs); return -3; }
    if (hipMalloc((void**)&st, sizeof(LmState<double>)) != hipSuccess) { (void)hipFree(slabs); (void)hipFree(packed); return -3; }
    int rc = 0;
    JtjArgs<double> a{};
    a.J = Yrm; a.Jout = J; a.y = y; a.y_old = y; a.dx = nullptr; a.dx_dot = nullptr; a.slabs = slabs; a.m = m; a.n = (int)n;
    a.twh = twh;
    hipEvent_t e0, e1;
    (void)hipEventCreate(&e0); (void)hipEventCreate(&e1);
    (void)hipEventRecord(e0, stream);
    if (jtj_run<double>(plan, op, a, packed, stream) != hipSuccess) rc = -4;
    (void)hipEventRecord(e1, stream);
    (void)jtj_unpack<double>(packed, (int)n, JJ, Jy, st, stream);
    if (hipStreamSynchronize(stream) != hipSuccess) rc = -5;
    if (kernel_ms) { float ms = 0; (void)hipEventElapsedTime(&ms, e0, e1); *kernel_ms = ms; }
    (void)hipEventDestroy(e0); (void)hipEventDestroy(e1);
    (void)hipFree(slabs); (void)hipFree(packed); (void)hipFree(st);
    return rc;
}
}

extern "C" {

int mir_solve_box_qp_gpu_d(const mir_box_qp_settings_d* settings, size_t n, const double* P, const double* q,
                           const double* l, const double* u, double* x, int unconstrainedSolution, int* iterations)
{
    return box_qp_entry<double>(settings, n, P, q, l, u, x, unconstrainedSolution, iterations);
}
int mir_solve_box_qp_gpu_s(const mir_box_qp_settings_s* settings, size_t n, const float* P, const float* q,
                           const float* l, const float* u, float* x, int unconstrainedSolution, int* iterations)
{
    return box_qp_entry<float>(settings, n, P, q, l, u, x, unconstrainedSolution, iterations);
}

int mir_lsq_jtj_d(size_t m, size_t n, double* J, const double* y, const double* y_old, const double* dx, int broyden,
                  double* JJ, double* Jy, void* stream, float* kernel_ms)
{
    return jtj_entry<double>(m, n, J, y, y_old, dx, broyden, JJ, Jy, stream, kernel_ms);
}
int mir_lsq_fd_jtj_d(size_t m, size_t n, const double* Yrm, const double* twh, const double* y, double* J,
                     double* JJ, double* Jy, void* stream_, float* kernel_ms)
{
    return fd_jtj_entry(m, n, Yrm, twh, y, J, JJ, Jy, stream_, kernel_ms, false);
}
int mir_lsq_fd_diff_jtj_d(size_t m, size_t n, const double* Drm, const double* twh, const double* y, double* J,
                          double* JJ, double* Jy, void* stream_, float* kernel_ms)
{
    return fd_jtj_entry(m, n, Drm, twh, y, J, JJ, Jy, stream_, kernel_ms, true);
}
int mir_lsq_jtj_plan(size_t elem_size, size_t m, size_t n, int num_cu, int op, int aligned16, size_t out[10])
{
    if ((elem_size != 4 && elem_size != 8) || m == 0 || n == 0 || n > (size_t)1 << 20 || num_cu < 1 || op < 0 || op > 3 || !out) return -1;
    const JtjPlan p = elem_size == 8 ? jtj_plan<double>(m, (int)n, num_cu) : jtj_plan<float>(m, (int)n, num_cu);
    const JtjLaunch l = jtj_resolve(p, (JtjOp)op, aligned16 != 0);
    const bool wide = l.kernel == JtjKernel::wide;
    const size_t v[10] = {(size_t)l.kernel, (size_t)l.ncb, (size_t)l.flat, (size_t)l.nblk, (size_t)l.njobs, l.lds,
                          (size_t)l.nblk * l.njobs, (size_t)l.slab_len, wide ? 0 : (size_t)l.ncb, jtj_slab_elems(p)};
    for (int i = 0; i < 10; ++i) out[i] = v[i];
    return 0;
}
int mir_lsq_jtj_s(size_t m, size_t n, float* J, const float* y, const float* y_old, const float* dx, int broyden,
                  float* JJ, float* Jy, void* stream, float* kernel_ms)
{
    return jtj_entry<float>(m, n, J, y, y_old, dx, broyden, JJ, Jy, stream, kernel_ms);
}
int mir_lsq_selftest_reductions(int rounds, int mismatches[4])
{
    if (!mismatches || rounds <= 0) return -1;
    if (!device_available()) return -2;
    int* d = nullptr;
    if (hipMalloc((void**)&d, 4 * sizeof(int)) != hipSuccess) return -3;
    bool ok = hipMemset(d, 0, 4 * sizeof(int)) == hipSuccess;
    if (ok) {
        hipLaunchKernelGGL(k_selftest_reductions, dim3(2048), dim3(256), 0, nullptr, rounds, 12345u, d);
        ok = hipGetLastError() == hipSuccess && hipDeviceSynchronize() == hipSuccess
          && hipMemcpy(mismatches, d, 4 * sizeof(int), hipMemcpyDeviceToHost) == hipSuccess;
    }
    (void)hipFree(d);
    return ok ? 0 : -4;
}

}
```

mir_optim_amd/csrc/workloads.hip:

```cpp
#include "workloads_device.h"
#include "workloads_gemm.h"

namespace {

template <typename T> struct Pair;
template <> struct Pair<double> { using type = double2; };
template <> struct Pair<float> { using type = float2; };

template <typename T, int NCP, int MODE, bool VEC>
__global__ __launch_bounds__(256) void k_tanh_linear(const T* __restrict__ A, const T* __restrict__ b,
                                                     const T* __restrict__ x, T* __restrict__ out, size_t m, int n)
{
    using P2 = typename Pair<T>::type;
    const int lane = threadIdx.x & 63;
    const int q = lane >> 4, p = lane & 15;
    T x0[NCP], x1[NCP];
    int coff[NCP];
    bool ok0[NCP], ok1[NCP];
#pragma unroll
    for (int c = 0; c < NCP; ++c) {
        const int col = 32 * c + 2 * p;
        ok0[c] = col < n;
        ok1[c] = col + 1 < n;
        coff[c] = ok0[c] ? col : 0;
        const T t0 = x[ok0[c] ? col : 0], t1 = x[ok1[c] ? col + 1 : 0];
        x0[c] = ok0[c] ? t0 : T(0);
        x1[c] = ok1[c] ? t1 : T(0);
    }
    const size_t G = (m + 3) / 4;
    const size_t wave_id = ((size_t)blockIdx.x * blockDim.x + threadIdx.x) >> 6;
    const size_t nwaves = ((size_t)gridDim.x * blockDim.x) >> 6;
    const size_t per = (G + nwaves - 1) / nwaves;
    const size_t gb = wave_id * per < G ? wave_id * per : G;
    const size_t ge = gb + per < G ? gb + per : G;
    constexpr int kAhead = (VEC && MODE == 0) ? 3 : 0, kRing = kAhead + 1;
    T v0[kRing][NCP], v1[kRing][NCP], bv[kRing];
    auto load = [&](size_t g, auto B) {
        constexpr int buf = decltype(B)::value;
        const size_t gc = g < ge ? g : (ge > gb ? ge - 1 : gb);
        const size_t row = 4 * gc + q;
        const T* rp = A + (row < m ? row : m - 1) * (size_t)n;
        if constexpr (MODE == 0) bv[buf] = b[row < m ? row : m - 1];
#pragma unroll
        for (int c = 0; c < NCP; ++c) {
            if constexpr (VEC) {
                typedef T wl_v2 __attribute__((ext_vector_type(2)));
                const wl_v2 t = __builtin_nontemporal_load(reinterpret_cast<const wl_v2*>(rp + coff[c]));
                v0[buf][c] = t.x;
                v1[buf][c] = t.y;
            } else {
                v0[buf][c] = rp[coff[c]];
                v1[buf][c] = rp[ok1[c] ? coff[c] + 1 : 0];
            }
        }
    };
    auto use = [&](size_t g, auto B) {
        constexpr int buf = decltype(B)::value;
        const size_t row = 4 * g + q;
        const bool rok = row < m;
        T s = 0;
#pragma unroll
        for (int c = 0; c < NCP; ++c) s += v0[buf][c] * x0[c] + v1[buf][c] * x1[c];
        s = sum16(s);
        const T t = dtanh(s);
        if constexpr (MODE == 0) {
            if (rok && p == 0) out[row] = t - bv[buf];
        } else {
            const T d = 1 - t * t;
            T* op = out + (rok ? row : m - 1) * (size_t)n;
#pragma unroll
            for (int c = 0; c < NCP; ++c) {
                if (rok && ok0[c]) op[coff[c]] = d * v0[buf][c];
                if (rok && ok1[c]) op[coff[c] + 1] = d * v1[buf][c];
            }
        }
    };
    if (gb >= ge) return;
    wl_static_for<kAhead>([&](auto U) { load(gb + decltype(U)::value, U); });
    for (size_t g0 = gb; g0 < ge; g0 += kRing) {
        wl_static_for<kRing>([&](auto U) {
            constexpr int u0 = decltype(U)::value;
            load(g0 + u0 + kAhead, std::integral_constant<int, (u0 + kAhead) % kRing>{});
            if (g0 + u0 < ge) use(g0 + u0, U);
        });
    }
}

template <typename T, int MODE>
__global__ __launch_bounds__(256) void k_tanh_linear_rows(const T* __restrict__ A, const T* __restrict__ b,
                                                          const T* __restrict__ x, T* __restrict__ out, size_t m, int n)
{
    const int lane = threadIdx.x & 63;
    const size_t wave_id = ((size_t)blockIdx.x * blockDim.x + threadIdx.x) >> 6;
    const size_t nwaves = ((size_t)gridDim.x * blockDim.x) >> 6;
    for (size_t row = wave_id; row < m; row += nwaves) {
        const T* rp = A + row * (size_t)n;
        T s = 0;
        for (int c = lane; c < n; c += 64) s += rp[c] * x[c];
        s = sum16(s);
        s += __shfl_xor(s, 16, 64);
        s += __shfl_xor(s, 32, 64);
        const T t = dtanh(s);
        if constexpr (MODE == 0) {
            if (lane == 0) out[row] = t - b[row];
        } else {
            const T d = 1 - t * t;
            T* op = out + row * (size_t)n;
            for (int c = lane; c < n; c += 64) op[c] = d * rp[c];
        }
    }
}

template <typename T, int NCP, int MODE>
void launch_tanh_linear_ncp(const T* A, const T* b, const T* x, T* out, size_t m, int n, dim3 grid, hipStream_t s)
{
    const bool vec = (n % 2 == 0) && (reinterpret_cast<uintptr_t>(A) % (2 * sizeof(T)) == 0);
    if (vec) hipLaunchKernelGGL((k_tanh_linear<T, NCP, MODE, true>), grid, dim3(256), 0, s, A, b, x, out, m, n);
    else hipLaunchKernelGGL((k_tanh_linear<T, NCP, MODE, false>), grid, dim3(256), 0, s, A, b, x, out, m, n);
}

template <typename T, int MODE>
void launch_tanh_linear(const T* A, const T* b, const T* x, T* out, size_t m, int n, hipStream_t s)
{
    const size_t G = (m + 3) / 4;
    size_t blocks = (G + 3) / 4;
    if (blocks > 256 * 4) blocks = 256 * 4;
    if (blocks < 1) blocks = 1;
    const int ncp = (n + 31) / 32;
    dim3 grid((unsigned)blocks);
    if (ncp > 8) {
        hipLaunchKernelGGL((k_tanh_linear_rows<T, MODE>), grid, dim3(256), 0, s, A, b, x, out, m, n);
        return;
    }
    if (ncp <= 1) launch_tanh_linear_ncp<T, 1, MODE>(A, b, x, out, m, n, grid, s);
    else if (ncp <= 2) launch_tanh_linear_ncp<T, 2, MODE>(A, b, x, out, m, n, grid, s);
    else if (ncp <= 4) launch_tanh_linear_ncp<T, 4, MODE>(A, b, x, out, m, n, grid, s);
    else launch_tanh_linear_ncp<T, 8, MODE>(A, b, x, out, m, n, grid, s);
}

constexpr int kGaussMax = 16;
template <typename T> __device__ inline T gauss_g(T w) { return T(-1) / (2 * w * w); }
template <typename T, int KC>
__device__ inline T gauss_row(T ti, const T (&a)[KC], const T (&c)[KC], const T (&g)[KC], int K, T base)
{
    T s = base;
#pragma unroll
    for (int k = 0; k < KC; ++k)
        if (k < K) { const T d = ti - c[k]; s = fma(a[k], dexp((d * d) * g[k]), s); }
    return s;
}
template <typename T> __device__ inline T gauss_row_any(T ti, const T* x, int K)
{
    T s = x[3 * K];
    for (int k = 0; k < K; ++k) { const T d = ti - x[K + k]; s = fma(x[k], dexp((d * d) * gauss_g(x[2 * K + k])), s); }
    return s;
}

template <typename T>
__global__ __launch_bounds__(256) void k_gauss_sum(const T* __restrict__ t, const T* __restrict__ data,
                                                   const T* __restrict__ x, T* __restrict__ y, size_t m, int n)
{
    const int K = (n - 1) / 3;
    if (K <= kGaussMax) {
        T a[kGaussMax], c[kGaussMax], g[kGaussMax];
#pragma unroll
        for (int k = 0; k < kGaussMax; ++k) { a[k] = k < K ? x[k] : T(0); c[k] = k < K ? x[K + k] : T(0); g[k] = k < K ? gauss_g(x[2 * K + k]) : T(0); }
        const T base = x[3 * K];
        for (size_t i = (size_t)blockIdx.x * blockDim.x + threadIdx.x; i < m; i += (size_t)gridDim.x * blockDim.x)
            y[i] = gauss_row<T, kGaussMax>(t[i], a, c, g, K, base) - data[i];
    } else {
        for (size_t i = (size_t)blockIdx.x * blockDim.x + threadIdx.x; i < m; i += (size_t)gridDim.x * blockDim.x)
            y[i] = gauss_row_any(t[i], x, K) - data[i];
    }
}

template <typename T, bool RM, bool FIXED>
__global__ __launch_bounds__(256) void k_gauss_sum_batched(const T* __restrict__ t, const T* __restrict__ data,
                                                           const T* __restrict__ X, T* __restrict__ Y, size_t m, int n, int P)
{
    const int K = (n - 1) / 3;
    const size_t total = m * (size_t)P;
    const size_t gid = (size_t)blockIdx.x * blockDim.x + threadIdx.x, stride = (size_t)gridDim.x * blockDim.x;
    if constexpr (FIXED) {
        static_assert(RM, "a fixed point per thread is the row-major walk");
        const int k = (int)(gid % (size_t)P);
        const T* x = X + (size_t)k * n;
        T a[kGaussMax], c[kGaussMax], g[kGaussMax];
#pragma unroll
        for (int q = 0; q < kGaussMax; ++q) { a[q] = q < K ? x[q] : T(0); c[q] = q < K ? x[K + q] : T(0); g[q] = q < K ? gauss_g(x[2 * K + q]) : T(0); }
        const T base = x[3 * K];
        const size_t rstep = stride / (size_t)P;
        size_t i = gid / (size_t)P;
        for (size_t e = gid; e < total; e += stride, i += rstep) Y[e] = gauss_row<T, kGaussMax>(t[i], a, c, g, K, base) - data[i];
    } else {
        for (size_t e = gid; e < total; e += stride) {
            const size_t i = RM ? e / P : e % m;
            const int k = (int)(RM ? e % P : e / m);
            Y[e] = gauss_row_any(t[i], X + (size_t)k * n, K) - data[i];
        }
    }
}

template <typename T>
__global__ __launch_bounds__(256) void k_exp_decay(const T* __restrict__ t, const T* __restrict__ data,
                                                   const T* __restrict__ x, T* __restrict__ y, size_t m, int kind)
{
    for (size_t i = (size_t)blockIdx.x * blockDim.x + threadIdx.x; i < m; i += (size_t)gridDim.x * blockDim.x) {
        if (kind == 0) y[i] = x[0] * dexp(-t[i] * x[1]) - data[i];
        else y[i] = x[0] * dexp(-t[i] / x[1]) + x[2] - data[i];
    }
}



template <int NCP, int NP>
__global__ __launch_bounds__(256) void k_tanh_linear_multi(const double* __restrict__ A, const double* __restrict__ b,
                                                           const double* __restrict__ X, double* __restrict__ Y,
                                                           size_t m, int n, int P)
{
    const int lane = threadIdx.x & 63;
    const int q = lane >> 4, p = lane & 15;
    double x0[NP][NCP], x1[NP][NCP];
    int coff[NCP];
#pragma unroll
    for (int c = 0; c < NCP; ++c) {
        const int col = 32 * c + 2 * p;
        const bool ok = col < n;
        coff[c] = ok ? col : 0;
#pragma unroll
        for (int k = 0; k < NP; ++k) {
            const double2 t = *reinterpret_cast<const double2*>(X + (size_t)(k < P ? k : 0) * n + coff[c]);
            x0[k][c] = (ok && k < P) ? t.x : 0.0;
            x1[k][c] = (ok && k < P) ? t.y : 0.0;
        }
    }
    const size_t G = (m + 3) / 4;
    const size_t wave_id = ((size_t)blockIdx.x * blockDim.x + threadIdx.x) >> 6;
    const size_t nwaves = ((size_t)gridDim.x * blockDim.x) >> 6;
    for (size_t g = wave_id; g < G; g += nwaves) {
        const size_t row = 4 * g + q;
        const bool rok = row < m;
        const double* rp = A + (rok ? row : m - 1) * (size_t)n;
        double2 v[NCP];
#pragma unroll
        for (int c = 0; c < NCP; ++c) {
            typedef double wl_d2 __attribute__((ext_vector_type(2)));
            const wl_d2 t = __builtin_nontemporal_load(reinterpret_cast<const wl_d2*>(rp + coff[c]));
            v[c] = make_double2(t.x, t.y);
        }
        const double bv = b[rok ? row : m - 1];
#pragma unroll
        for (int k = 0; k < NP; ++k) {
            if (k < P) {
                double s = 0;
#pragma unroll
                for (int c = 0; c < NCP; ++c) s += v[c].x * x0[k][c] + v[c].y * x1[k][c];
                s = sum16(s);
                if (rok && p == 0) Y[(size_t)k * m + row] = dtanh(s) - bv;
            }
        }
    }
}

bool launch_tanh_linear_multi(const double* A, const double* b, const double* X, double* Y, size_t m, int n, int P, hipStream_t s)
{
    if (P > 8 || n > 128 || n % 2 != 0) return false;
    if (reinterpret_cast<uintptr_t>(A) % 16 != 0 || reinterpret_cast<uintptr_t>(X) % 16 != 0) return false;
    const size_t G = (m + 3) / 4;
    size_t blocks = (G + 3) / 4;
    if (blocks > 256 * 8) blocks = 256 * 8;
    if (blocks < 1) blocks = 1;
    const int ncp = (n + 31) / 32;
    dim3 grid((unsigned)blocks), blk(256);
    if (ncp <= 1) hipLaunchKernelGGL((k_tanh_linear_multi<1, 8>), grid, blk, 0, s, A, b, X, Y, m, n, P);
    else if (ncp <= 2) hipLaunchKernelGGL((k_tanh_linear_multi<2, 8>), grid, blk, 0, s, A, b, X, Y, m, n, P);
    else hipLaunchKernelGGL((k_tanh_linear_multi<4, 8>), grid, blk, 0, s, A, b, X, Y, m, n, P);
    return true;
}

inline unsigned blocks_for(size_t m)
{
    size_t b = (m + 255) / 256;
    if (b > 256 * 8) b = 256 * 8;
    return (unsigned)(b ? b : 1);
}

inline uint64_t splitmix64_mix(uint64_t z)
{
    z += 0x9E3779B97F4A7C15ull;
    z = (z ^ (z >> 30)) * 0xBF58476D1CE4E5B9ull;
    z = (z ^ (z >> 27)) * 0x94D049BB133111EBull;
    return z ^ (z >> 31);
}

}

__global__ __launch_bounds__(256) void k_busy(long long ticks)
{
    extern __shared__ unsigned char busy_smem[];
    const long long t0 = wall_clock64();
    if (threadIdx.x == 0) busy_smem[0] = 1;
    while (wall_clock64() - t0 < ticks) __builtin_amdgcn_s_sleep(32);
}

extern "C" {

struct wl_tanh_linear_ctx { const void* A; const void* b; void* stream; int read_a_once;  };
struct wl_curve_ctx { const void* t; const void* data; void* stream; int kind; };

void wl_tanh_linear_f_d(void* vctx, size_t m, size_t n, const double* x, double* y)
{
    auto* c = static_cast<wl_tanh_linear_ctx*>(vctx);
    launch_tanh_linear<double, 0>((const double*)c->A, (const double*)c->b, x, y, m, (int)n, (hipStream_t)c->stream);
}
void wl_tanh_linear_g_d(void* vctx, size_t m, size_t n, const double* x, double* J)
{
    auto* c = static_cast<wl_tanh_linear_ctx*>(vctx);
    launch_tanh_linear<double, 1>((const double*)c->A, (const double*)c->b, x, J, m, (int)n, (hipStream_t)c->stream);
}
void wl_tanh_linear_fb_d(void* vctx, size_t m, size_t n, size_t p, const double* X, double* Y)
{
    auto* c = static_cast<wl_tanh_linear_ctx*>(vctx);
    if (p <= 8 && launch_tanh_linear_multi((const double*)c->A, (const double*)c->b, X, Y, m, (int)n, (int)p, (hipStream_t)c->stream)) return;
    if (launch_tanh_linear_batched((const double*)c->A, (const double*)c->b, X, Y, m, (int)n, (int)p, (hipStream_t)c->stream)) return;
    for (size_t k = 0; k < p; ++k)
        launch_tanh_linear<double, 0>((const double*)c->A, (const double*)c->b, X + k * n, Y + k * m, m, (int)n, (hipStream_t)c->stream);
}
void wl_tanh_linear_fbr_d(void* vctx, size_t m, size_t n, size_t p, const double* X, double* Y)
{
    auto* c = static_cast<wl_tanh_linear_ctx*>(vctx);
    launch_tanh_linear_batched_rm((const double*)c->A, (const double*)c->b, X, Y, m, (int)n, (int)p, (hipStream_t)c->stream);
}
void wl_tanh_linear_fbd_d(void* vctx, size_t m, size_t n, size_t p, const double* X, double* D)
{
    auto* c = static_cast<wl_tanh_linear_ctx*>(vctx);
    launch_tanh_linear_batched_diff((const double*)c->A, (const double*)c->b, X, D, m, (int)n, (int)p, (hipStream_t)c->stream, c->read_a_once);
}
void wl_tanh_linear_fbd_dense_d(void* vctx, size_t m, size_t n, size_t p, const double* X, double* D)
{
    auto* c = static_cast<wl_tanh_linear_ctx*>(vctx);
    launch_tanh_linear_batched_diff((const double*)c->A, (const double*)c->b, X, D, m, (int)n, (int)p, (hipStream_t)c->stream, c->read_a_once,
                                    true);
}
void wl_tanh_linear_f_s(void* vctx, size_t m, size_t n, const float* x, float* y)
{
    auto* c = static_cast<wl_tanh_linear_ctx*>(vctx);
    launch_tanh_linear<float, 0>((const float*)c->A, (const float*)c->b, x, y, m, (int)n, (hipStream_t)c->stream);
}
void wl_tanh_linear_g_s(void* vctx, size_t m, size_t n, const float* x, float* J)
{
    auto* c = static_cast<wl_tanh_linear_ctx*>(vctx);
    launch_tanh_linear<float, 1>((const float*)c->A, (const float*)c->b, x, J, m, (int)n, (hipStream_t)c->stream);
}

struct wl_tanh_linear_host_ctx { const double* A; const double* b; };
void wl_tanh_linear_f_host_d(void* vctx, size_t m, size_t n, const double* x, double* y)
{
    auto* c = static_cast<wl_tanh_linear_host_ctx*>(vctx);
#pragma omp parallel for schedule(static)
    for (ptrdiff_t i = 0; i < (ptrdiff_t)m; ++i) {
        const double* a = c->A + (size_t)i * n;
        double s = 0;
        for (size_t j = 0; j < n; ++j) s += a[j] * x[j];
        y[i] = std::tanh(s) - c->b[i];
    }
}

void wl_tanh_linear_f_host_serial_d(void* vctx, size_t m, size_t n, const double* x, double* y)
{
    auto* c = static_cast<wl_tanh_linear_host_ctx*>(vctx);
    for (size_t i = 0; i < m; ++i) {
        const double* a = c->A + i * n;
        double s = 0;
        for (size_t j = 0; j < n; ++j) s += a[j] * x[j];
        y[i] = std::tanh(s) - c->b[i];
    }
}

struct wl_task { void* context; void* fn; };
typedef void (*wl_task_fn)(wl_task, uint32_t, uint32_t, uint32_t);
void wl_omp_thread_manager(void* ctx, uint32_t count, wl_task task, wl_task_fn fn)
{
    const int want = ctx ? *static_cast<const int*>(ctx) : 0;
#pragma omp parallel num_threads(want > 0 ? want : omp_get_max_threads())
    {
        const uint32_t total = (uint32_t)omp_get_num_threads(), tid = (uint32_t)omp_get_thread_num();
#pragma omp for schedule(dynamic, 1)
        for (ptrdiff_t i = 0; i < (ptrdiff_t)count; ++i) fn(task, total, tid, (uint32_t)i);
    }
}

void wl_gauss_sum_f_d(void* vctx, size_t m, size_t n, const double* x, double* y)
{
    auto* c = static_cast<wl_curve_ctx*>(vctx);
    hipLaunchKernelGGL(k_gauss_sum<double>, dim3(blocks_for(m)), dim3(256), 0, (hipStream_t)c->stream,
                       (const double*)c->t, (const double*)c->data, x, y, m, (int)n);
}
void wl_gauss_sum_f_s(void* vctx, size_t m, size_t n, const float* x, float* y)
{
    auto* c = static_cast<wl_curve_ctx*>(vctx);
    hipLaunchKernelGGL(k_gauss_sum<float>, dim3(blocks_for(m)), dim3(256), 0, (hipStream_t)c->stream,
                       (const float*)c->t, (const float*)c->data, x, y, m, (int)n);
}
void wl_gauss_sum_fb_d(void* vctx, size_t m, size_t n, size_t p, const double* X, double* Y)
{
    auto* c = static_cast<wl_curve_ctx*>(vctx);
    hipLaunchKernelGGL((k_gauss_sum_batched<double, false, false>), dim3(blocks_for(m * p)), dim3(256), 0, (hipStream_t)c->stream,
                       (const double*)c->t, (const double*)c->data, X, Y, m, (int)n, (int)p);
}
void wl_gauss_sum_fbr_d(void* vctx, size_t m, size_t n, size_t p, const double* X, double* Y)
{
    auto* c = static_cast<wl_curve_ctx*>(vctx);
    const unsigned nb = blocks_for(m * p);
    if ((n - 1) / 3 <= (size_t)kGaussMax && p > 0 && ((size_t)nb * 256) % p == 0)
        hipLaunchKernelGGL((k_gauss_sum_batched<double, true, true>), dim3(nb), dim3(256), 0, (hipStream_t)c->stream,
                           (const double*)c->t, (const double*)c->data, X, Y, m, (int)n, (int)p);
    else
        hipLaunchKernelGGL((k_gauss_sum_batched<double, true, false>), dim3(nb), dim3(256), 0, (hipStream_t)c->stream,
                           (const double*)c->t, (const double*)c->data, X, Y, m, (int)n, (int)p);
}
void wl_exp_decay_f_d(void* vctx, size_t m, size_t n, const double* x, double* y)
{
    (void)n;
    auto* c = static_cast<wl_curve_ctx*>(vctx);
    hipLaunchKernelGGL(k_exp_decay<double>, dim3(blocks_for(m)), dim3(256), 0, (hipStream_t)c->stream,
                       (const double*)c->t, (const double*)c->data, x, y, m, c->kind);
}
void wl_exp_decay_f_s(void* vctx, size_t m, size_t n, const float* x, float* y)
{
    (void)n;
    auto* c = static_cast<wl_curve_ctx*>(vctx);
    hipLaunchKernelGGL(k_exp_decay<float>, dim3(blocks_for(m)), dim3(256), 0, (hipStream_t)c->stream,
                       (const float*)c->t, (const float*)c->data, x, y, m, c->kind);
}

void wl_busy(void* stream, unsigned blocks, unsigned lds_bytes, unsigned microseconds)
{
    hipLaunchKernelGGL(k_busy, dim3(blocks), dim3(256), lds_bytes, (hipStream_t)stream, (long long)microseconds * 100);
}

void wl_uniform(uint64_t seed, uint64_t offset, size_t count, double* out)
{
    for (size_t k = 0; k < count; ++k) out[k] = (double)(splitmix64_mix(seed + offset + (uint64_t)k) >> 11) * 0x1p-53;
}

void wl_tanh_linear_generate(size_t m, size_t n, size_t row_offset, double noise, double* A, double* b,
                             double* xstar, double* x0)
{
    const double sc = std::sqrt(3.0 / (double)n);
    for (size_t j = 0; j < n; ++j) {
        xstar[j] = 2 * ((double)(splitmix64_mix(11 + j) >> 11) * 0x1p-53) - 1;
        x0[j] = xstar[j] + 0.1 * (2 * ((double)(splitmix64_mix(13 + j) >> 11) * 0x1p-53) - 1);
    }
#pragma omp parallel for schedule(static)
    for (ptrdiff_t i = 0; i < (ptrdiff_t)m; ++i) {
        const uint64_t gi = (uint64_t)row_offset + (uint64_t)i;
        double* a = A + (size_t)i * n;
        double s = 0;
        for (size_t j = 0; j < n; ++j) {
            a[j] = (2 * ((double)(splitmix64_mix(10 + gi * n + j) >> 11) * 0x1p-53) - 1) * sc;
            s += a[j] * xstar[j];
        }
        b[i] = std::tanh(s) + noise * (2 * ((double)(splitmix64_mix(12 + gi) >> 11) * 0x1p-53) - 1);
    }
}

}
```

Before: 1167.

## Add ring-buffered software-pipelined row sweeps for Broyden LR and tanh-linear kernels

Adds a RING-buffered software-pipelined variant of the low-rank Broyden sweep kernel. It prefetches J rows several groups ahead and loads the y/y_old/U side vectors in 16-group pieces shared via shuffles. It is selected only through a new SWEEP_RING variant flag. The tanh-linear workload kernels gain a contiguous-range 'pieces' path with double-buffered nontemporal loads, which turns on by default when each wave has enough row groups. A standalone lr_sweep test/timing entry point is also added. The aim is to hide global load latency, with the cost of higher register use and a lower occupancy bound (2 WGs) on the ring path.

```diff
diff --git a/include/mir_optim_amd.h b/include/mir_optim_amd.h
--- a/include/mir_optim_amd.h
+++ b/include/mir_optim_amd.h
@@ -135,6 +135,8 @@
     MIR_LSQ_VARIANT_SOLVE_ONE_WORKGROUP = 1u << 11,
     MIR_LSQ_VARIANT_FD_HOST_COLUMNS = 1u << 13,
     MIR_LSQ_VARIANT_NO_PIPELINE = 1u << 22,
+    MIR_LSQ_VARIANT_SWEEP_PLAIN = 1u << 23,
+    MIR_LSQ_VARIANT_SWEEP_RING = 1u << 24,
     MIR_LSQ_VARIANT_DEBUG_HELPERS_ABSENT = 1u << 12,
     MIR_LSQ_VARIANT_DEBUG_SOLVE = 1u << 7,
     MIR_LSQ_VARIANT_HOST_PROFILE = 1u << 8,
@@ -386,6 +388,8 @@
 int mir_lsq_fd_diff_jtj_d(size_t m, size_t n, const double* Drm, const double* twh, const double* y, double* J,
                           double* JJ, double* Jy, void* stream, float* kernel_ms);
 int mir_lsq_jtj_plan(size_t elem_size, size_t m, size_t n, int num_cu, int op, int aligned16, size_t out[10]);
+int mir_lsq_lr_sweep_d(size_t m, size_t n, int k, const double* J, double* U, const double* D, const double* dx, const double* y,
+                       const double* y_old, int spec, int path, int reps, double* partials, double* reduced, int* nblk, float* kernel_ms);
 
 enum { MIR_LSQ_COVARIANCE_ABSOLUTE_SIGMA = 1u };
 int mir_lsq_covariance_gpu_d(const mir_least_squares_settings_d* settings, size_t m, size_t n,
diff --git a/mir_optim_amd/api.py b/mir_optim_amd/api.py
--- a/mir_optim_amd/api.py
+++ b/mir_optim_amd/api.py
@@ -17,7 +17,7 @@
     "fit_spline_residuals", "variant_lr_cap",
     "VARIANT_BROYDEN_REWRITE", "VARIANT_FD_SEPARATE_FILL", "VARIANT_NO_SPECULATION", "VARIANT_NO_NULL_SKIP",
     "VARIANT_SOLVE_BOUNDED", "VARIANT_DEBUG_SOLVE", "VARIANT_HOST_PROFILE", "VARIANT_SOLVE_GENERIC", "VARIANT_SOLVE_ONE_WORKGROUP", "VARIANT_DEBUG_HELPERS_ABSENT", "VARIANT_FD_HOST_COLUMNS",
-    "VARIANT_NO_PIPELINE", "BatchedOptions", "BatchedExtras", "BATCHED_ABSOLUTE_SIGMA",
+    "VARIANT_NO_PIPELINE", "VARIANT_SWEEP_PLAIN", "VARIANT_SWEEP_RING", "lr_sweep", "BatchedOptions", "BatchedExtras", "BATCHED_ABSOLUTE_SIGMA",
     "covariance", "spdInverse", "COVARIANCE_ABSOLUTE_SIGMA",
 ]
 
@@ -43,6 +43,8 @@
 VARIANT_DEBUG_HELPERS_ABSENT = 1 << 12
 VARIANT_FD_HOST_COLUMNS = 1 << 13
 VARIANT_NO_PIPELINE = 1 << 22
+VARIANT_SWEEP_PLAIN = 1 << 23
+VARIANT_SWEEP_RING = 1 << 24
 
 
 def variant_lr_cap(k):
@@ -276,6 +278,9 @@
         L.mir_lsq_fd_diff_jtj_d.restype = C.c_int
         L.mir_lsq_fd_diff_jtj_d.argtypes = [sz, sz, C.c_void_p, C.c_void_p, C.c_void_p, C.c_void_p, C.c_void_p, C.c_void_p,
                                             C.c_void_p, C.POINTER(C.c_float)]
+        L.mir_lsq_lr_sweep_d.restype = C.c_int
+        L.mir_lsq_lr_sweep_d.argtypes = [sz, sz, C.c_int] + [C.c_void_p] * 6 + [C.c_int] * 3 + [C.c_void_p, C.c_void_p,
+                                                                                                 C.POINTER(C.c_int), C.POINTER(C.c_float)]
         L.mir_lsq_fd_jtj_d.restype = C.c_int
         L.mir_lsq_fd_jtj_d.argtypes = [sz, sz, C.c_void_p, C.c_void_p, C.c_void_p, C.c_void_p, C.c_void_p, C.c_void_p,
                                        C.c_void_p, C.c_void_p]
@@ -942,6 +947,28 @@
     return out
 
 
+LR_MAX = 16
+LR_BLOCKS_MAX = 1024
+
+
+def lr_sweep(J, U, D, dx, y, y_old, k, spec=0, path=0, reps=1):
+    J = np.ascontiguousarray(J, dtype=np.float64)
+    m, n = J.shape
+    U = np.array(U, dtype=np.float64, order="C")
+    D = np.ascontiguousarray(D, dtype=np.float64)
+    dx, y, y_old = (np.ascontiguousarray(v, dtype=np.float64) for v in (dx, y, y_old))
+    assert U.shape == (LR_MAX, m) and D.shape == (LR_MAX, n) and dx.shape == (n,) and y.shape == (m,) and y_old.shape == (m,)
+    ln = 2 * n + 2 * LR_MAX + 3
+    partials = np.zeros((LR_BLOCKS_MAX, ln))
+    reduced = np.zeros(ln)
+    nblk, ms = C.c_int(0), C.c_float(0)
+    rc = lib().mir_lsq_lr_sweep_d(m, n, int(k), J.ctypes.data, U.ctypes.data, D.ctypes.data, dx.ctypes.data, y.ctypes.data, y_old.ctypes.data,
+                                  int(spec), int(path), int(reps), partials.ctypes.data, reduced.ctypes.data, C.byref(nblk), C.byref(ms))
+    if rc != 0:
+        raise RuntimeError(f"mir_lsq_lr_sweep_d failed: {rc}")
+    return partials.reshape(-1)[:nblk.value * ln].reshape(nblk.value, ln).copy(), reduced, U, ms.value
+
+
 JTJ_OPS = ("plain", "rewrite", "fd", "fd_diff")
 JTJ_FAMILIES = ("none", "stream", "fdp", "pc32", "ring8", "fdp8", "wide")
 
diff --git a/mir_optim_amd/csrc/broyden_launch.h b/mir_optim_amd/csrc/broyden_launch.h
--- a/mir_optim_amd/csrc/broyden_launch.h
+++ b/mir_optim_amd/csrc/broyden_launch.h
@@ -20,6 +20,7 @@
     int k;
     const ChainRec<T>* spec_rec;
     T absTolerance, relTolerance;
+    int path;
 };
 
 constexpr int kLrMaxBlocks = 1024;
diff --git a/mir_optim_amd/csrc/broyden_lr.h b/mir_optim_amd/csrc/broyden_lr.h
--- a/mir_optim_amd/csrc/broyden_lr.h
+++ b/mir_optim_amd/csrc/broyden_lr.h
@@ -41,8 +41,8 @@
     return yy;
 }
 
-template <typename T, int NCP, bool VEC>
-__global__ __launch_bounds__(256, (NCP <= 4 ? 4 : 1)) void k_broyden_lr(const LrArgs<T> a)
+template <typename T, int NCP, bool VEC, int RING = 0, int WGS = (NCP <= 4 ? 4 : 1)>
+__global__ __launch_bounds__(256, WGS) void k_broyden_lr(const LrArgs<T> a)
 {
     using P2 = typename LrPair<T>::type;
     __shared__ T red[4][lr_len(kLrMaxN)];
@@ -98,6 +98,89 @@
     T wl = 0, hl = 0, uu = 0, uy = 0, yy = 0;
 
     constexpr int UNR = NCP == 1 ? 4 : (NCP == 2 ? 2 : 1);
+    if constexpr (RING > 0) {
+        static_assert(VEC && 16 % RING == 0, "the ring walks 16-group pieces of the side vectors");
+        typedef T lr_v2 __attribute__((ext_vector_type(2)));
+        auto sweep = [&](auto KBc) {
+            constexpr int KB = decltype(KBc)::value;
+            T v0[RING][NCP], v1[RING][NCP], ulr[RING];
+            auto load = [&](size_t g, auto B) {
+                constexpr int buf = decltype(B)::value;
+                const size_t gc = g < ge ? g : ge - 1;
+                const size_t row = 4 * gc + q;
+                const size_t rr = row < m ? row : m - 1;
+                const T* __restrict__ rp = a.J + rr * (size_t)n;
+#pragma unroll
+                for (int c = 0; c < NCP; ++c) {
+                    const lr_v2 t = __builtin_nontemporal_load(reinterpret_cast<const lr_v2*>(rp + coff[c]));
+                    v0[buf][c] = t.x;
+                    v1[buf][c] = t.y;
+                }
+                if constexpr (KB == 2) ulr[buf] = own ? Up[rr] : T(0);
+            };
+            auto side = [&](size_t c0, T& ys, T& os, T& ua, T& ub) {
+                const size_t row = 4 * c0 + lane;
+                const size_t rr = row < m ? row : m - 1;
+                ys = a.y[rr];
+                os = a.y_old[rr];
+                if constexpr (KB == 1) { ua = a.U[rr]; ub = k > 1 ? a.U[m + rr] : T(0); }
+            };
+            T yc = 0, oc = 0, uac = 0, ubc = 0, yx = 0, ox = 0, uax = 0, ubx = 0;
+            static_for<RING - 1>([&](auto B) { load(gb + decltype(B)::value, B); });
+            side(gb, yc, oc, uac, ubc);
+            for (size_t c0 = gb; c0 < ge; c0 += 16) {
+                side(c0 + 16, yx, ox, uax, ubx);
+                T ust = 0;
+                static_for<16>([&](auto E) {
+                    constexpr int e = decltype(E)::value;
+                    load(c0 + e + RING - 1, IntC<(e + RING - 1) % RING>{});
+                    if (c0 + e < ge) {
+                        constexpr int buf = e % RING;
+                        const size_t row = 4 * (c0 + e) + q;
+                        const bool rok = row < m;
+                        T yn = __shfl(yc, 4 * e + q, kWave);
+                        const T yo = __shfl(oc, 4 * e + q, kWave);
+                        T ul = 0;
+                        if constexpr (KB == 1) {
+                            const T ta = __shfl(uac, 4 * e + q, kWave), tb = __shfl(ubc, 4 * e + q, kWave);
+                            ul = p == 0 ? ta : (p == 1 ? tb : T(0));
+                        }
+                        if constexpr (KB == 2) ul = ulr[buf];
+                        T s = ul * cp;
+#pragma unroll
+                        for (int c = 0; c < NCP; ++c) s += v0[buf][c] * d0[c] + v1[buf][c] * d1[c];
+                        s = sum16(s);
+                        T u = nd * ((yo - yn) + s);
+                        if (!rok) { u = 0; yn = 0; }
+                        const T ug = __shfl(u, 16 * (lane & 3), kWave);
+                        if ((lane >> 2) == e) ust = ug;
+#pragma unroll
+                        for (int c = 0; c < NCP; ++c) {
+                            va0[c] += v0[buf][c] * u;
+                            va1[c] += v1[buf][c] * u;
+                            ga0[c] += v0[buf][c] * yn;
+                            ga1[c] += v1[buf][c] * yn;
+                        }
+                        wl += ul * u;
+                        hl += ul * yn;
+                        uu += u * u;
+                        uy += u * yn;
+                        yy = dfma(yn, yn, yy);
+                    }
+                });
+                {
+                    const size_t row = 4 * c0 + lane;
+                    if (c0 + (size_t)(lane >> 2) < ge && row < m) Uk[row] = ust;
+                }
+                yc = yx; oc = ox; uac = uax; ubc = ubx;
+            }
+        };
+        if (gb < ge) {
+            if (k == 0) sweep(IntC<0>{});
+            else if (k <= 2) sweep(IntC<1>{});
+            else sweep(IntC<2>{});
+        }
+    } else
     for (size_t g0 = gb; g0 < ge; g0 += UNR) {
         T v0[UNR][NCP], v1[UNR][NCP], ynv[UNR], yov[UNR], ulv[UNR];
 #pragma unroll
diff --git a/mir_optim_amd/csrc/launch_broyden.hip b/mir_optim_amd/csrc/launch_broyden.hip
--- a/mir_optim_amd/csrc/launch_broyden.hip
+++ b/mir_optim_amd/csrc/launch_broyden.hip
@@ -23,7 +23,15 @@
     const int ncp = (a.n + 31) / 32;
     if (ncp <= 1) return lr_sweep_ncp<T, 1>(a, nblk, vec, s);
     if (ncp <= 2) return lr_sweep_ncp<T, 2>(a, nblk, vec, s);
-    if (ncp <= 4) return lr_sweep_ncp<T, 4>(a, nblk, vec, s);
+    if (ncp <= 4) {
+        if constexpr (sizeof(T) == 8) {
+            if (vec && a.path == 2) {
+                MIRLSQ_LAUNCH((k_broyden_lr<T, 4, true, 4, 2>), dim3(nblk), dim3(256), 0, s, a);
+                return hipGetLastError();
+            }
+        }
+        return lr_sweep_ncp<T, 4>(a, nblk, vec, s);
+    }
     if (ncp <= 8) return lr_sweep_ncp<T, 8>(a, nblk, vec, s);
     return lr_sweep_ncp<T, 16>(a, nblk, vec, s);
 }
diff --git a/mir_optim_amd/csrc/solver_jacobian.hip b/mir_optim_amd/csrc/solver_jacobian.hip
--- a/mir_optim_amd/csrc/solver_jacobian.hip
+++ b/mir_optim_amd/csrc/solver_jacobian.hip
@@ -19,7 +19,7 @@
     }
     LrArgs<T> a{};
     a.J = B.J; a.U = U; a.D = B.lrD; a.dx = B.dx_acc; a.dx_dot = &B.st->dx_dot; a.y = y_dev; a.y_old = yold_dev;
-    a.partials = B.lrpart; a.m = m; a.n = (int)n; a.k = lr_k;
+    a.partials = B.lrpart; a.m = m; a.n = (int)n; a.k = lr_k; a.path = (variant & MIR_LSQ_VARIANT_SWEEP_PLAIN) ? 1 : ((variant & MIR_LSQ_VARIANT_SWEEP_RING) ? 2 : 0);
     const int nblk = lr_blocks(m, ws->num_cu), len = lr_len((int)n);
     ev_begin(1);
     if (!ok(lr_sweep<T>(a, nblk, stream), "broyden sweep")) return false;
diff --git a/mir_optim_amd/csrc/solver_loop.hip b/mir_optim_amd/csrc/solver_loop.hip
--- a/mir_optim_amd/csrc/solver_loop.hip
+++ b/mir_optim_amd/csrc/solver_loop.hip
@@ -327,7 +327,7 @@
     if (stats) stats->fused_rounds++;
     LrArgs<T> a{};
     a.J = B.J; a.U = static_cast<T*>(ws->ulr); a.D = B.lrD; a.dx = B.dx; a.dx_dot = &B.rec[0].new_dx_dot; a.y = ytr; a.y_old = y;
-    a.partials = B.lrpart; a.m = m; a.n = (int)n; a.k = lr_k;
+    a.partials = B.lrpart; a.m = m; a.n = (int)n; a.k = lr_k; a.path = (variant & MIR_LSQ_VARIANT_SWEEP_PLAIN) ? 1 : ((variant & MIR_LSQ_VARIANT_SWEEP_RING) ? 2 : 0);
     a.spec_rec = B.rec; a.absTolerance = sd.absTolerance; a.relTolerance = sd.relTolerance;
     const int nblk = lr_blocks(m, ws->num_cu), len = lr_len((int)n);
     spec_enqueue = true;
diff --git a/mir_optim_amd/csrc/unit_entries.hip b/mir_optim_amd/csrc/unit_entries.hip
--- a/mir_optim_amd/csrc/unit_entries.hip
+++ b/mir_optim_amd/csrc/unit_entries.hip
@@ -140,9 +140,72 @@
     (void)hipFree(slabs); (void)hipFree(packed); (void)hipFree(st);
     return rc;
 }
+
+int lr_sweep_entry(size_t m, size_t n, int k, const double* J, double* U, const double* D, const double* dx, const double* y,
+                   const double* y_old, int spec, int path, int reps, double* partials, double* reduced, int* nblk_out, float* kernel_ms)
+{
+    if (!device_available()) return -1;
+    if (m == 0 || n == 0 || n > (size_t)kLrMaxN || k < 0 || k >= kLrMax || spec < 0 || spec > 2 || reps < 1) return -2;
+    const int nblk = lr_blocks(m, query_num_cu()), len = lr_len((int)n);
+    size_t off = 0;
+    auto take = [&](size_t bytes) { size_t o = off; off = align_up(off + bytes, 256); return o; };
+    const size_t oJ = take(8 * m * n), oU = take(8 * (size_t)kLrMax * m), oD = take(8 * (size_t)kLrMax * n), odx = take(8 * n), oy = take(8 * m),
+                 oyo = take(8 * m), op = take(8 * (size_t)nblk * len), or_ = take(8 * (size_t)len), os = take(8), orec = take(sizeof(ChainRec<double>));
+    char* base = nullptr;
+    if (hipMalloc((void**)&base, off) != hipSuccess) return -3;
+    double dd = 0;
+    for (size_t j = 0; j < n; ++j) dd += dx[j] * dx[j];
+    ChainRec<double> rec{};
+    rec.new_dx_dot = dd;
+    rec.trial_xnorm = 1;
+    rec.flags = spec == 2 ? kFlagNullStep : 0;
+    LrArgs<double> a{};
+    a.J = (double*)(base + oJ); a.U = (double*)(base + oU); a.D = (double*)(base + oD); a.dx = (double*)(base + odx);
+    a.y = (double*)(base + oy); a.y_old = (double*)(base + oyo); a.partials = (double*)(base + op); a.dx_dot = (double*)(base + os);
+    a.m = m; a.n = (int)n; a.k = k; a.path = path;
+    a.spec_rec = spec ? (ChainRec<double>*)(base + orec) : nullptr;
+    a.absTolerance = 0; a.relTolerance = 0;
+    bool good = hipMemcpy((void*)a.J, J, 8 * m * n, hipMemcpyHostToDevice) == hipSuccess
+        && hipMemcpy((void*)a.U, U, 8 * (size_t)kLrMax * m, hipMemcpyHostToDevice) == hipSuccess
+        && hipMemcpy((void*)a.D, D, 8 * (size_t)kLrMax * n, hipMemcpyHostToDevice) == hipSuccess
+        && hipMemcpy((void*)a.dx, dx, 8 * n, hipMemcpyHostToDevice) == hipSuccess
+        && hipMemcpy((void*)a.y, y, 8 * m, hipMemcpyHostToDevice) == hipSuccess
+        && hipMemcpy((void*)a.y_old, y_old, 8 * m, hipMemcpyHostToDevice) == hipSuccess
+        && hipMemcpy((void*)a.dx_dot, &dd, 8, hipMemcpyHostToDevice) == hipSuccess
+        && hipMemcpy(base + orec, &rec, sizeof(rec), hipMemcpyHostToDevice) == hipSuccess;
+    int rc = good ? 0 : -3;
+    hipEvent_t e0, e1;
+    (void)hipEventCreate(&e0); (void)hipEventCreate(&e1);
+    if (good) {
+        if (reps > 1 && lr_sweep<double>(a, nblk, nullptr) != hipSuccess) rc = -4;
+        (void)hipEventRecord(e0, nullptr);
+        for (int r = 0; r < reps && rc == 0; ++r)
+            if (lr_sweep<double>(a, nblk, nullptr) != hipSuccess) rc = -4;
+        (void)hipEventRecord(e1, nullptr);
+        if (rc == 0 && lr_reduce<double>(a.partials, nblk, (int)n, (double*)(base + or_), nullptr) != hipSuccess) rc = -4;
+        if (hipDeviceSynchronize() != hipSuccess) rc = -5;
+    }
+    if (rc == 0) {
+        if (kernel_ms) { float ms = 0; (void)hipEventElapsedTime(&ms, e0, e1); *kernel_ms = ms / (float)reps; }
+        good = hipMemcpy(partials, a.partials, 8 * (size_t)nblk * len, hipMemcpyDeviceToHost) == hipSuccess
+            && hipMemcpy(reduced, base + or_, 8 * (size_t)len, hipMemcpyDeviceToHost) == hipSuccess
+            && hipMemcpy(U, a.U, 8 * (size_t)kLrMax * m, hipMemcpyDeviceToHost) == hipSuccess;
+        if (!good) rc = -5;
+        if (nblk_out) *nblk_out = nblk;
+    }
+    (void)hipEventDestroy(e0); (void)hipEventDestroy(e1);
+    (void)hipFree(base);
+    return rc;
+}
 }
 
 extern "C" {
+
+int mir_lsq_lr_sweep_d(size_t m, size_t n, int k, const double* J, double* U, const double* D, const double* dx, const double* y,
+                       const double* y_old, int spec, int path, int reps, double* partials, double* reduced, int* nblk, float* kernel_ms)
+{
+    return lr_sweep_entry(m, n, k, J, U, D, dx, y, y_old, spec, path, reps, partials, reduced, nblk, kernel_ms);
+}
 
 int mir_solve_box_qp_gpu_d(const mir_box_qp_settings_d* settings, size_t n, const double* P, const double* q,
                            const double* l, const double* u, double* x, int unconstrainedSolution, int* iterations)
diff --git a/mir_optim_amd/csrc/workloads.hip b/mir_optim_amd/csrc/workloads.hip
--- a/mir_optim_amd/csrc/workloads.hip
+++ b/mir_optim_amd/csrc/workloads.hip
@@ -7,7 +7,7 @@
 template <> struct Pair<double> { using type = double2; };
 template <> struct Pair<float> { using type = float2; };
 
-template <typename T, int NCP, int MODE, bool VEC>
+template <typename T, int NCP, int MODE, bool VEC, bool PIECES = false>
 __global__ __launch_bounds__(256) void k_tanh_linear(const T* __restrict__ A, const T* __restrict__ b,
                                                      const T* __restrict__ x, T* __restrict__ out, size_t m, int n)
 {
@@ -40,7 +40,7 @@
         const size_t gc = g < ge ? g : (ge > gb ? ge - 1 : gb);
         const size_t row = 4 * gc + q;
         const T* rp = A + (row < m ? row : m - 1) * (size_t)n;
-        if constexpr (MODE == 0) bv[buf] = b[row < m ? row : m - 1];
+        if constexpr (MODE == 0 && !PIECES) bv[buf] = b[row < m ? row : m - 1];
 #pragma unroll
         for (int c = 0; c < NCP; ++c) {
             if constexpr (VEC) {
@@ -77,6 +77,31 @@
     };
     if (gb >= ge) return;
     wl_static_for<kAhead>([&](auto U) { load(gb + decltype(U)::value, U); });
+    if constexpr (PIECES) {
+        static_assert(VEC && MODE == 0 && 16 % kRing == 0, "the ring walks 16-group pieces of b and out");
+        auto piece = [&](size_t c0) { const size_t row = 4 * c0 + lane; return b[row < m ? row : m - 1]; };
+        T bc = piece(gb);
+        for (size_t c0 = gb; c0 < ge; c0 += 16) {
+            const T bx = piece(c0 + 16);
+            T sg = 0;
+            wl_static_for<16>([&](auto E) {
+                constexpr int e = decltype(E)::value, buf = e % kRing;
+                load(c0 + e + kAhead, std::integral_constant<int, (e + kAhead) % kRing>{});
+                if (c0 + e < ge) {
+                    T s = 0;
+#pragma unroll
+                    for (int c = 0; c < NCP; ++c) s += v0[buf][c] * x0[c] + v1[buf][c] * x1[c];
+                    s = sum16(s);
+                    const T g = __shfl(s, 16 * (lane & 3), 64);
+                    if ((lane >> 2) == e) sg = g;
+                }
+            });
+            const size_t row = 4 * c0 + lane;
+            if (c0 + (size_t)(lane >> 2) < ge && row < m) out[row] = dtanh(sg) - bc;
+            bc = bx;
+        }
+        return;
+    }
     for (size_t g0 = gb; g0 < ge; g0 += kRing) {
         wl_static_for<kRing>([&](auto U) {
             constexpr int u0 = decltype(U)::value;
@@ -111,16 +136,25 @@
     }
 }
 
+inline bool wl_pieces(int body, size_t m, unsigned blocks, size_t min_per)
+{
+    const size_t G = (m + 3) / 4, nw = (size_t)blocks * 4;
+    return body == 2 || (body == 0 && (G + nw - 1) / nw >= min_per);
+}
+
 template <typename T, int NCP, int MODE>
-void launch_tanh_linear_ncp(const T* A, const T* b, const T* x, T* out, size_t m, int n, dim3 grid, hipStream_t s)
+void launch_tanh_linear_ncp(const T* A, const T* b, const T* x, T* out, size_t m, int n, dim3 grid, hipStream_t s, int body)
 {
     const bool vec = (n % 2 == 0) && (reinterpret_cast<uintptr_t>(A) % (2 * sizeof(T)) == 0);
+    if constexpr (MODE == 0 && NCP == 4 && sizeof(T) == 8) {
+        if (vec && wl_pieces(body, m, grid.x, 32)) { hipLaunchKernelGGL((k_tanh_linear<T, NCP, MODE, true, true>), grid, dim3(256), 0, s, A, b, x, out, m, n); return; }
+    }
     if (vec) hipLaunchKernelGGL((k_tanh_linear<T, NCP, MODE, true>), grid, dim3(256), 0, s, A, b, x, out, m, n);
     else hipLaunchKernelGGL((k_tanh_linear<T, NCP, MODE, false>), grid, dim3(256), 0, s, A, b, x, out, m, n);
 }
 
 template <typename T, int MODE>
-void launch_tanh_linear(const T* A, const T* b, const T* x, T* out, size_t m, int n, hipStream_t s)
+void launch_tanh_linear(const T* A, const T* b, const T* x, T* out, size_t m, int n, hipStream_t s, int body = 0)
 {
     const size_t G = (m + 3) / 4;
     size_t blocks = (G + 3) / 4;
@@ -132,10 +166,10 @@
         hipLaunchKernelGGL((k_tanh_linear_rows<T, MODE>), grid, dim3(256), 0, s, A, b, x, out, m, n);
         return;
     }
-    if (ncp <= 1) launch_tanh_linear_ncp<T, 1, MODE>(A, b, x, out, m, n, grid, s);
-    else if (ncp <= 2) launch_tanh_linear_ncp<T, 2, MODE>(A, b, x, out, m, n, grid, s);
-    else if (ncp <= 4) launch_tanh_linear_ncp<T, 4, MODE>(A, b, x, out, m, n, grid, s);
-    else launch_tanh_linear_ncp<T, 8, MODE>(A, b, x, out, m, n, grid, s);
+    if (ncp <= 1) launch_tanh_linear_ncp<T, 1, MODE>(A, b, x, out, m, n, grid, s, body);
+    else if (ncp <= 2) launch_tanh_linear_ncp<T, 2, MODE>(A, b, x, out, m, n, grid, s, body);
+    else if (ncp <= 4) launch_tanh_linear_ncp<T, 4, MODE>(A, b, x, out, m, n, grid, s, body);
+    else launch_tanh_linear_ncp<T, 8, MODE>(A, b, x, out, m, n, grid, s, body);
 }
 
 constexpr int kGaussMax = 16;
@@ -213,7 +247,7 @@
 
 
 
-template <int NCP, int NP>
+template <int NCP, int NP, bool PIECES = false>
 __global__ __launch_bounds__(256) void k_tanh_linear_multi(const double* __restrict__ A, const double* __restrict__ b,
                                                            const double* __restrict__ X, double* __restrict__ Y,
                                                            size_t m, int n, int P)
@@ -237,6 +271,56 @@
     const size_t G = (m + 3) / 4;
     const size_t wave_id = ((size_t)blockIdx.x * blockDim.x + threadIdx.x) >> 6;
     const size_t nwaves = ((size_t)gridDim.x * blockDim.x) >> 6;
+    if constexpr (PIECES) {
+        typedef double wl_d2 __attribute__((ext_vector_type(2)));
+        const size_t per = (G + nwaves - 1) / nwaves;
+        const size_t gb = wave_id * per < G ? wave_id * per : G;
+        const size_t ge = gb + per < G ? gb + per : G;
+        if (gb >= ge) return;
+        wl_d2 v[2][NCP];
+        auto load = [&](size_t g, auto B) {
+            constexpr int buf = decltype(B)::value;
+            const size_t gc = g < ge ? g : ge - 1;
+            const size_t row = 4 * gc + q;
+            const double* rp = A + (row < m ? row : m - 1) * (size_t)n;
+#pragma unroll
+            for (int c = 0; c < NCP; ++c) v[buf][c] = __builtin_nontemporal_load(reinterpret_cast<const wl_d2*>(rp + coff[c]));
+        };
+        auto piece = [&](size_t c0) { const size_t row = 4 * c0 + lane; return b[row < m ? row : m - 1]; };
+        load(gb, std::integral_constant<int, 0>{});
+        double bc = piece(gb);
+        for (size_t c0 = gb; c0 < ge; c0 += 16) {
+            const double bx = piece(c0 + 16);
+            double sg[NP];
+#pragma unroll
+            for (int k = 0; k < NP; ++k) sg[k] = 0;
+            wl_static_for<16>([&](auto E) {
+                constexpr int e = decltype(E)::value, buf = e % 2;
+                load(c0 + e + 1, std::integral_constant<int, (e + 1) % 2>{});
+                if (c0 + e < ge) {
+#pragma unroll
+                    for (int k = 0; k < NP; ++k) {
+                        if (k < P) {
+                            double s = 0;
+#pragma unroll
+                            for (int c = 0; c < NCP; ++c) s += v[buf][c].x * x0[k][c] + v[buf][c].y * x1[k][c];
+                            s = sum16(s);
+                            const double g = __shfl(s, 16 * (lane & 3), 64);
+                            if ((lane >> 2) == e) sg[k] = g;
+                        }
+                    }
+                }
+            });
+            const size_t row = 4 * c0 + lane;
+            if (c0 + (size_t)(lane >> 2) < ge && row < m) {
+#pragma unroll
+                for (int k = 0; k < NP; ++k)
+                    if (k < P) Y[(size_t)k * m + row] = dtanh(sg[k]) - bc;
+            }
+            bc = bx;
+        }
+        return;
+    }
     for (size_t g = wave_id; g < G; g += nwaves) {
         const size_t row = 4 * g + q;
         const bool rok = row < m;
@@ -262,7 +346,8 @@
     }
 }
 
-bool launch_tanh_linear_multi(const double* A, const double* b, const double* X, double* Y, size_t m, int n, int P, hipStream_t s)
+bool launch_tanh_linear_multi(const double* A, const double* b, const double* X, double* Y, size_t m, int n, int P, hipStream_t s,
+                              int body = 0)
 {
     if (P > 8 || n > 128 || n % 2 != 0) return false;
     if (reinterpret_cast<uintptr_t>(A) % 16 != 0 || reinterpret_cast<uintptr_t>(X) % 16 != 0) return false;
@@ -274,7 +359,8 @@
     dim3 grid((unsigned)blocks), blk(256);
     if (ncp <= 1) hipLaunchKernelGGL((k_tanh_linear_multi<1, 8>), grid, blk, 0, s, A, b, X, Y, m, n, P);
     else if (ncp <= 2) hipLaunchKernelGGL((k_tanh_linear_multi<2, 8>), grid, blk, 0, s, A, b, X, Y, m, n, P);
-    else hipLaunchKernelGGL((k_tanh_linear_multi<4, 8>), grid, blk, 0, s, A, b, X, Y, m, n, P);
+    else if (!wl_pieces(body, m, grid.x, 12)) hipLaunchKernelGGL((k_tanh_linear_multi<4, 8>), grid, blk, 0, s, A, b, X, Y, m, n, P);
+    else hipLaunchKernelGGL((k_tanh_linear_multi<4, 8, true>), grid, blk, 0, s, A, b, X, Y, m, n, P);
     return true;
 }
 
@@ -313,6 +399,16 @@
     auto* c = static_cast<wl_tanh_linear_ctx*>(vctx);
     launch_tanh_linear<double, 0>((const double*)c->A, (const double*)c->b, x, y, m, (int)n, (hipStream_t)c->stream);
 }
+void wl_tanh_linear_f_plain_d(void* vctx, size_t m, size_t n, const double* x, double* y)
+{
+    auto* c = static_cast<wl_tanh_linear_ctx*>(vctx);
+    launch_tanh_linear<double, 0>((const double*)c->A, (const double*)c->b, x, y, m, (int)n, (hipStream_t)c->stream, 1);
+}
+void wl_tanh_linear_f_pieces_d(void* vctx, size_t m, size_t n, const double* x, double* y)
+{
+    auto* c = static_cast<wl_tanh_linear_ctx*>(vctx);
+    launch_tanh_linear<double, 0>((const double*)c->A, (const double*)c->b, x, y, m, (int)n, (hipStream_t)c->stream, 2);
+}
 void wl_tanh_linear_g_d(void* vctx, size_t m, size_t n, const double* x, double* J)
 {
     auto* c = static_cast<wl_tanh_linear_ctx*>(vctx);
@@ -326,6 +422,16 @@
     for (size_t k = 0; k < p; ++k)
         launch_tanh_linear<double, 0>((const double*)c->A, (const double*)c->b, X + k * n, Y + k * m, m, (int)n, (hipStream_t)c->stream);
 }
+static void wl_tanh_linear_fb_body(void* vctx, size_t m, size_t n, size_t p, const double* X, double* Y, int body)
+{
+    auto* c = static_cast<wl_tanh_linear_ctx*>(vctx);
+    if (p <= 8 && launch_tanh_linear_multi((const double*)c->A, (const double*)c->b, X, Y, m, (int)n, (int)p, (hipStream_t)c->stream, body)) return;
+    if (launch_tanh_linear_batched((const double*)c->A, (const double*)c->b, X, Y, m, (int)n, (int)p, (hipStream_t)c->stream)) return;
+    for (size_t k = 0; k < p; ++k)
+        launch_tanh_linear<double, 0>((const double*)c->A, (const double*)c->b, X + k * n, Y + k * m, m, (int)n, (hipStream_t)c->stream, body);
+}
+void wl_tanh_linear_fb_plain_d(void* vctx, size_t m, size_t n, size_t p, const double* X, double* Y) { wl_tanh_linear_fb_body(vctx, m, n, p, X, Y, 1); }
+void wl_tanh_linear_fb_pieces_d(void* vctx, size_t m, size_t n, size_t p, const double* X, double* Y) { wl_tanh_linear_fb_body(vctx, m, n, p, X, Y, 2); }
 void wl_tanh_linear_fbr_d(void* vctx, size_t m, size_t n, size_t p, const double* X, double* Y)
 {
     auto* c = static_cast<wl_tanh_linear_ctx*>(vctx);
```

Result: no change. 1157 (-0.8%).
